# GoekeLab/m6anet

Measured on AMD Instinct MI355X. Metric: DRACH sites/sec at num_iterations=1000, higher is better.
Workload: dtype f32

## Files before the change

include/m6a.h:

```cpp
#ifndef M6A_H
#define M6A_H
#include <stddef.h>
#include <stdint.h>
#ifdef __cplusplus
extern "C" {
#endif

typedef struct m6a_ctx m6a_ctx;

enum {
    M6A_OK = 0,
    M6A_EINVAL = -1,
    M6A_ENOMEM = -2,
    M6A_EHIP = -3,
    M6A_ESTREAM = -4,
    M6A_ENODEV = -5,
    M6A_EUNSUPPORTED = -6,
    M6A_EFORMAT = -7,
    M6A_EIO = -8,
    M6A_EDECLINED = -9
};

enum { M6A_RNG_NUMPY = 0 };

#define M6A_N_WEIGHTS 7997
#define M6A_N_FEATURES 9
#define M6A_MAX_SAMPLES 64
#define M6A_N_KMERS 66

int m6a_create(m6a_ctx **out, const float *weights, size_t n_floats, int device_id);
void m6a_destroy(m6a_ctx *ctx);
const char *m6a_last_error(const m6a_ctx *ctx);

int m6a_set_stream(m6a_ctx *ctx, void *hip_stream);
int m6a_set_job_offset(m6a_ctx *ctx, int64_t first_site);
int m6a_sync(m6a_ctx *ctx);
int m6a_set_host_offsets(m6a_ctx *ctx, const int64_t *off_host);
int m6a_prepare_host_io(m6a_ctx *ctx);
int m6a_host_alloc(size_t bytes, void **out);
int m6a_host_free(void *p);
int m6a_host_is_pinned(const void *p, size_t bytes);

int m6a_encode_reads(m6a_ctx *ctx, const float *X, const uint8_t *site_kmers, const int64_t *off,
                     int64_t n_sites, float *read_prob);

int m6a_site_pool(m6a_ctx *ctx, const float *read_prob, const int64_t *off, int64_t n_sites,
                  int n_iters, int n_samples, float read_proba_threshold, uint32_t seed,
                  int rng_mode, int64_t batch_size, int64_t save_per_batch,
                  float *site_prob, double *mod_ratio);

int m6a_infer(m6a_ctx *ctx, const float *X, const uint8_t *site_kmers, const int64_t *off,
              int64_t n_sites, int n_iters, int n_samples, float read_proba_threshold,
              uint32_t seed, int rng_mode, int64_t batch_size, int64_t save_per_batch,
              float *read_prob, float *site_prob, double *mod_ratio);

int m6a_job_begin(m6a_ctx *ctx, int n_iters, int n_samples, float read_proba_threshold, uint32_t seed, int rng_mode,
                  int64_t batch_size, int64_t save_per_batch, int64_t expect_sites, int64_t expect_reads);
int m6a_job_feed(m6a_ctx *ctx, const float *X, const uint8_t *site_kmers, const int64_t *off, int64_t n_sites);
int m6a_job_feed_collated(m6a_ctx *ctx, const float *features, const int64_t *kmers, const int64_t *n_reads, int64_t n_sites);
int m6a_job_size(const m6a_ctx *ctx, int64_t *n_sites, int64_t *n_reads);
int m6a_job_end(m6a_ctx *ctx, float *read_prob, float *site_prob, double *mod_ratio);
int m6a_job_abort(m6a_ctx *ctx);

int m6a_bag_forward(m6a_ctx *ctx, const float *X, const uint8_t *site_kmers, int64_t n_bags,
                    int bag, float *site_prob);

int m6a_validate_pool(m6a_ctx *ctx, const float *read_prob, const int64_t *off, int64_t n_sites,
                      int n_iters, int n_samples, uint32_t seed, float *y_pred, float *y_pred_avg);
int m6a_validate(m6a_ctx *ctx, const float *X, const uint8_t *site_kmers, const int64_t *off,
                 int64_t n_sites, int n_iters, int n_samples, uint32_t seed, float *read_prob,
                 float *y_pred, float *y_pred_avg);


int64_t m6a_flush_groups(int64_t n_sites, int64_t batch_size, int64_t save_per_batch,
                         int64_t *group_off, int64_t cap);

int64_t m6a_reference_written_sites(int64_t n_sites, int64_t batch_size, int64_t save_per_batch);

int m6a_shard_plan(const int64_t *off, int64_t n_sites, int64_t batch_size, int64_t save_per_batch,
                   int n_shards, int64_t *shard_site_off);

#define M6A_COMM_ID_BYTES 128
int m6a_comm_unique_id(void *id_out);
int m6a_comm_init(m6a_ctx *ctx, const void *unique_id, int rank, int world_size);
int m6a_gather(m6a_ctx *ctx, const float *site_prob, const double *mod_ratio, const int64_t *shard_site_off,
               int dst, float *site_all, double *mod_all);
int m6a_gather_reads(m6a_ctx *ctx, const float *read_prob, const int64_t *shard_read_off, int dst, float *read_all);
int m6a_comm_destroy(m6a_ctx *ctx);
int m6a_comm_count(m6a_ctx *ctx, int *ranks_seen);
int m6a_comm_info(m6a_ctx *ctx, int *rank, int *device, int *rccl_version);
int m6a_device_link(int dev_a, int dev_b, int *link_type, int *hops, int *peer_access);
int m6a_device_count(void);

int m6a_random_stream(m6a_ctx *ctx, uint32_t seed, int64_t n_words, uint32_t *words);

int m6a_profile_enable(m6a_ctx *ctx, int on);
int m6a_profile_read(m6a_ctx *ctx, int kind, double *total_ms, int64_t *n_launches);
int m6a_profile_clock(m6a_ctx *ctx, int kind, double *ghz_median, double *ghz_min, double *ghz_max, double *span_ms, int *n_waves);
int m6a_set_encoder_variant(m6a_ctx *ctx, int mode);
const char *m6a_last_encoder_variant(const m6a_ctx *ctx);
const char *m6a_last_encoder_kernel(const m6a_ctx *ctx);
int m6a_set_scan_driver(m6a_ctx *ctx, int mode);
int m6a_set_table_variant(m6a_ctx *ctx, int mode);
const char *m6a_last_pool_variant(const m6a_ctx *ctx);

const char *m6a_version(void);

typedef struct m6a_prep m6a_prep;
struct m6a_io_prep_table;
int m6a_prep_eventalign(int device_id, const char *path, int n_neighbors, const char *index_path, m6a_prep **out);
const struct m6a_io_prep_table *m6a_prep_table(const m6a_prep *p);
int m6a_prep_times(const m6a_prep *p, double *ms6);
void m6a_prep_free(m6a_prep *p);
const char *m6a_prep_last_error(void);

typedef struct m6a_prep_sites m6a_prep_sites;
struct m6a_io_rows;
typedef struct m6a_prep_host_half {
    int (*rows)(const char *eventalign_path, int64_t n_runs, const int64_t *start, const int64_t *end, const int64_t *read,
                int n_neighbors, int n_threads, struct m6a_io_rows **out);
    const struct m6a_io_prep_table *(*table)(const struct m6a_io_rows *r);
    void (*free)(struct m6a_io_rows *r);
    const char *(*error)(void);
} m6a_prep_host_half;
typedef struct m6a_prep_sites_info {
    int64_t n_sites, n_reads, n_tx;
    const float *X;
    const uint8_t *site_kmers;
    const int64_t *off;
    float *read_prob, *site_prob;
    double *mod_ratio;
    const int64_t *off_host;
    const uint32_t *site_tx;
    const int64_t *site_pos;
    const char *site_kmer7;
    const char *tx_blob;
    const int64_t *tx_off;
    const double *read_ids;
    double ms[8];
    int64_t d2h_bytes;
    int n_rep;
    const int32_t *read_rep;
    int64_t peak_bytes;
    int64_t n_windows, window_bytes;
    int64_t n_bgzf_blocks, compressed_bytes;
    double ms_inflate;
    int64_t n_declined_sites;
} m6a_prep_sites_info;
int m6a_prep_sites_build(int device_id, const char *path, int readcount_min, int readcount_max, int min_segment_count,
                         const char *norm_kmers, const double *norm_mean, const double *norm_std, int n_norm,
                         const m6a_prep_host_half *host, int n_threads, m6a_prep_sites **out);
int m6a_prep_sites_build_multi(int device_id, const char *const *paths, int n_paths, int readcount_min, int readcount_max,
                               int min_segment_count, const char *norm_kmers, const double *norm_mean, const double *norm_std, int n_norm,
                               const m6a_prep_host_half *host, int n_threads, m6a_prep_sites **out);
int m6a_prep_sites_build_windows(int device_id, const char *const *paths, int n_paths, int readcount_min, int readcount_max,
                                 int min_segment_count, const char *norm_kmers, const double *norm_mean, const double *norm_std, int n_norm,
                                 const m6a_prep_host_half *host, int n_threads, int64_t window_bytes, m6a_prep_sites **out);
int m6a_prep_sites_build_names(int device_id, const char *const *paths, int n_paths, int readcount_min, int readcount_max,
                               int min_segment_count, const char *norm_kmers, const double *norm_mean, const double *norm_std, int n_norm,
                               const m6a_prep_host_half *host, int n_threads, int64_t window_bytes, int read_names, m6a_prep_sites **out);
int m6a_prep_sites_read_names(const m6a_prep_sites *p, const uint8_t **names16, const int64_t **name_off, int *n_rep);
double m6a_prep_sites_intern_ms(const m6a_prep_sites *p);
#define M6A_PREP_STREAM_WINDOW_BYTES ((int64_t)256 << 20)
int64_t m6a_prep_sites_stream_bytes(const m6a_prep_sites *p);
int64_t m6a_prep_sites_n_streams(const m6a_prep_sites *p);
const m6a_prep_sites_info *m6a_prep_sites_get(const m6a_prep_sites *p);
int m6a_prep_sites_fetch(m6a_prep_sites *p, float *read_prob, float *site_prob, double *mod_ratio);
int m6a_prep_sites_inputs(m6a_prep_sites *p, float *X, uint8_t *site_kmers, int64_t *off);
void m6a_prep_sites_free(m6a_prep_sites *p);

struct m6a_io_info;
struct m6a_io_info_table;
typedef struct m6a_json_host_half {
    int (*open)(const char *dir, int min_reads, struct m6a_io_info **out);
    const struct m6a_io_info_table *(*table)(const struct m6a_io_info *info);
    int (*rows)(struct m6a_io_info *info, const int64_t *sites, int64_t n, const char *norm_kmers, const double *norm_mean,
                const double *norm_std, int n_norm, int n_threads, float *X, double *read_ids, uint8_t *site_kmers, char *kmer7);
    void (*free)(struct m6a_io_info *info);
    const char *(*error)(void);
} m6a_json_host_half;
int m6a_json_sites_build(int device_id, const char *const *dirs, int n_dirs, int min_reads, const char *norm_kmers,
// ... 59 lines not shown
```

m6anet_amd/_lib.py:

```python
import ctypes as C
import os

_PKG = os.path.dirname(os.path.abspath(__file__))
LIB_PATH = os.environ.get("M6A_HIP_LIB") or os.path.join(_PKG, "libm6a_hip.so")

M6A_OK = 0
ERRORS = {-1: "M6A_EINVAL", -2: "M6A_ENOMEM", -3: "M6A_EHIP", -4: "M6A_ESTREAM", -5: "M6A_ENODEV",
          -6: "M6A_EUNSUPPORTED", -7: "M6A_EFORMAT", -8: "M6A_EIO", -9: "M6A_EDECLINED"}
M6A_EDECLINED = -9
RNG_NUMPY = 0

SYMBOLS = ["m6a_create", "m6a_destroy", "m6a_last_error", "m6a_set_stream", "m6a_set_job_offset", "m6a_set_scan_driver", "m6a_set_table_variant", "m6a_set_encoder_variant", "m6a_last_encoder_variant", "m6a_last_encoder_kernel", "m6a_sync", "m6a_set_host_offsets", "m6a_prepare_host_io", "m6a_host_alloc", "m6a_host_free", "m6a_host_is_pinned",
           "m6a_encode_reads", "m6a_site_pool", "m6a_infer", "m6a_job_begin", "m6a_job_feed", "m6a_job_feed_collated", "m6a_job_size", "m6a_job_end", "m6a_job_abort", "m6a_bag_forward", "m6a_validate_pool", "m6a_validate", "m6a_flush_groups",
           "m6a_reference_written_sites",
           "m6a_shard_plan", "m6a_comm_unique_id", "m6a_comm_init", "m6a_gather", "m6a_gather_reads", "m6a_device_count", "m6a_random_stream", "m6a_comm_destroy", "m6a_comm_count", "m6a_comm_info", "m6a_device_link", "m6a_profile_enable", "m6a_profile_read", "m6a_profile_clock", "m6a_last_pool_variant",
           "m6a_version", "m6a_prep_eventalign", "m6a_prep_table", "m6a_prep_times", "m6a_prep_free", "m6a_prep_last_error",
           "m6a_prep_sites_build", "m6a_prep_sites_build_multi", "m6a_prep_sites_build_windows", "m6a_prep_sites_build_names", "m6a_prep_sites_read_names", "m6a_prep_sites_intern_ms", "m6a_prep_sites_stream_bytes", "m6a_prep_sites_n_streams", "m6a_prep_sites_get", "m6a_prep_sites_fetch", "m6a_prep_sites_inputs", "m6a_prep_sites_free",
           "m6a_csv_format", "m6a_prep_sites_write_csv", "m6a_bgzf_inflate", "m6a_bgzf_deflate", "m6a_prep_sites_write_csv_bgzf",
           "m6a_bgzf_deflate_level", "m6a_prep_sites_write_csv_bgzf_level", "m6a_json_sites_build"]

_lib = None


class HostHalf(C.Structure):
    _fields_ = [("rows", C.c_void_p), ("table", C.c_void_p), ("free", C.c_void_p), ("error", C.c_void_p)]


class JsonHostHalf(C.Structure):
    _fields_ = [("open", C.c_void_p), ("table", C.c_void_p), ("rows", C.c_void_p), ("free", C.c_void_p), ("error", C.c_void_p)]


class PrepSitesInfo(C.Structure):
    _fields_ = [("n_sites", C.c_int64), ("n_reads", C.c_int64), ("n_tx", C.c_int64), ("X", C.c_void_p), ("site_kmers", C.c_void_p),
                ("off", C.c_void_p), ("read_prob", C.c_void_p), ("site_prob", C.c_void_p), ("mod_ratio", C.c_void_p),
                ("off_host", C.c_void_p), ("site_tx", C.c_void_p), ("site_pos", C.c_void_p), ("site_kmer7", C.c_void_p),
                ("tx_blob", C.c_void_p), ("tx_off", C.c_void_p), ("read_ids", C.c_void_p), ("ms", C.c_double * 8),
                ("d2h_bytes", C.c_int64), ("n_rep", C.c_int), ("read_rep", C.c_void_p), ("peak_bytes", C.c_int64),
                ("n_windows", C.c_int64), ("window_bytes", C.c_int64),
                ("n_bgzf_blocks", C.c_int64), ("compressed_bytes", C.c_int64), ("ms_inflate", C.c_double),
                ("n_declined_sites", C.c_int64)]


class BgzfStats(C.Structure):
    _fields_ = [("n_blocks", C.c_int64), ("compressed_bytes", C.c_int64), ("ms_upload", C.c_double), ("ms_inflate", C.c_double),
                ("ms_crc", C.c_double), ("ms_copy", C.c_double), ("d2h_bytes", C.c_int64)]


class DeflateStats(C.Structure):
    _fields_ = [("n_blocks", C.c_int64), ("n_stored", C.c_int64), ("ms_deflate", C.c_double), ("ms_copy", C.c_double), ("d2h_bytes", C.c_int64)]


class CsvBgzfStats(C.Structure):
    _fields_ = [("ms_format", C.c_double), ("ms_deflate", C.c_double), ("ms_copy", C.c_double), ("ms_write", C.c_double),
                ("site_bytes", C.c_int64), ("indiv_bytes", C.c_int64), ("site_compressed", C.c_int64), ("indiv_compressed", C.c_int64),
                ("n_blocks", C.c_int64), ("n_stored", C.c_int64), ("n_declined", C.c_int64), ("d2h_bytes", C.c_int64), ("n_rounds", C.c_int64)]


class CsvArrays(C.Structure):
    _fields_ = [("n_sites", C.c_int64), ("n_tx", C.c_int64), ("off", C.c_void_p), ("site_tx", C.c_void_p), ("site_pos", C.c_void_p),
                ("kmer5", C.c_void_p), ("tx_blob", C.c_char_p), ("tx_off", C.c_void_p), ("read_ids", C.c_void_p), ("read_rep", C.c_void_p),
                ("n_rep", C.c_int), ("read_prob", C.c_void_p), ("site_prob", C.c_void_p), ("mod_ratio", C.c_void_p)]


class CsvStats(C.Structure):
    _fields_ = [("ms_format", C.c_double), ("ms_copy", C.c_double), ("ms_write", C.c_double), ("site_bytes", C.c_int64),
                ("indiv_bytes", C.c_int64), ("n_declined", C.c_int64), ("d2h_bytes", C.c_int64), ("n_rounds", C.c_int64)]


class M6AError(RuntimeError):
    def __init__(self, code, msg):
        super().__init__("%s (%d): %s" % (ERRORS.get(code, "M6A_E?"), code, msg))
        self.code = code


def _preload_hip_runtime():
    import importlib.util
    try:
        spec = importlib.util.find_spec("torch")
    except (ImportError, ValueError):
        spec = None
    if spec and spec.submodule_search_locations:
        libdir = os.path.join(list(spec.submodule_search_locations)[0], "lib")
        rt = os.path.join(libdir, "libamdhip64.so")
        if os.path.exists(rt):
            C.CDLL(rt, mode=C.RTLD_GLOBAL)
        rccl = os.path.join(libdir, "librccl.so")
        if os.path.exists(rccl):
            os.environ.setdefault("M6A_RCCL_LIB", rccl)


def load():
    global _lib
    if _lib is not None:
        return _lib
    if not os.path.exists(LIB_PATH):
        raise ImportError("libm6a_hip.so is not built: run `python -m m6anet_amd.build` "
                          "(or __graft_entry__.build()); there is no CPU fallback")
    _preload_hip_runtime()
    L = C.CDLL(LIB_PATH)
    vp, i64, i32, u32, f32, sz = C.c_void_p, C.c_int64, C.c_int, C.c_uint32, C.c_float, C.c_size_t
    L.m6a_create.argtypes = [C.POINTER(vp), vp, sz, i32]
    L.m6a_destroy.argtypes = [vp]
    L.m6a_destroy.restype = None
    L.m6a_last_error.argtypes = [vp]
    L.m6a_last_error.restype = C.c_char_p
    L.m6a_set_stream.argtypes = [vp, vp]
    L.m6a_sync.argtypes = [vp]
    L.m6a_set_host_offsets.argtypes = [vp, vp]
    L.m6a_prepare_host_io.argtypes = [vp]
    L.m6a_set_job_offset.argtypes = [vp, i64]
    L.m6a_set_scan_driver.argtypes = [vp, i32]
    L.m6a_set_table_variant.argtypes = [vp, i32]
    L.m6a_set_encoder_variant.argtypes = [vp, i32]
    L.m6a_last_encoder_variant.argtypes = [vp]
    L.m6a_last_encoder_variant.restype = C.c_char_p
    L.m6a_host_alloc.argtypes = [C.c_size_t, C.POINTER(vp)]
    L.m6a_host_free.argtypes = [vp]
    L.m6a_host_is_pinned.argtypes = [vp, C.c_size_t]
    L.m6a_last_encoder_kernel.argtypes = [vp]
    L.m6a_last_encoder_kernel.restype = C.c_char_p
    L.m6a_encode_reads.argtypes = [vp, vp, vp, vp, i64, vp]
    L.m6a_site_pool.argtypes = [vp, vp, vp, i64, i32, i32, f32, u32, i32, i64, i64, vp, vp]
    L.m6a_infer.argtypes = [vp, vp, vp, vp, i64, i32, i32, f32, u32, i32, i64, i64, vp, vp, vp]
    L.m6a_job_begin.argtypes = [vp, i32, i32, f32, u32, i32, i64, i64, i64, i64]
    L.m6a_job_feed.argtypes = [vp, vp, vp, vp, i64]
    L.m6a_job_feed_collated.argtypes = [vp, vp, vp, vp, i64]
    L.m6a_job_size.argtypes = [vp, C.POINTER(i64), C.POINTER(i64)]
    L.m6a_job_end.argtypes = [vp, vp, vp, vp]
    L.m6a_job_abort.argtypes = [vp]
    L.m6a_bag_forward.argtypes = [vp, vp, vp, i64, i32, vp]
    L.m6a_validate_pool.argtypes = [vp, vp, vp, i64, i32, i32, C.c_uint32, vp, vp]
    L.m6a_validate.argtypes = [vp, vp, vp, vp, i64, i32, i32, C.c_uint32, vp, vp, vp]
    L.m6a_flush_groups.argtypes = [i64, i64, i64, vp, i64]
    L.m6a_flush_groups.restype = i64
    L.m6a_reference_written_sites.argtypes = [i64, i64, i64]
    L.m6a_reference_written_sites.restype = i64
    L.m6a_shard_plan.argtypes = [vp, i64, i64, i64, i32, vp]
    L.m6a_comm_unique_id.argtypes = [vp]
    L.m6a_comm_init.argtypes = [vp, vp, i32, i32]
    L.m6a_gather.argtypes = [vp, vp, vp, vp, i32, vp, vp]
    L.m6a_gather_reads.argtypes = [vp, vp, vp, i32, vp]
    L.m6a_device_count.argtypes = []
    L.m6a_random_stream.argtypes = [vp, u32, i64, vp]
    L.m6a_comm_destroy.argtypes = [vp]
    pi = C.POINTER(i32)
    L.m6a_comm_count.argtypes = [vp, pi]
    L.m6a_comm_info.argtypes = [vp, pi, pi, pi]
    L.m6a_device_link.argtypes = [i32, i32, pi, pi, pi]
    L.m6a_profile_enable.argtypes = [vp, i32]
    L.m6a_profile_read.argtypes = [vp, i32, C.POINTER(C.c_double), C.POINTER(i64)]
    L.m6a_profile_clock.argtypes = [vp, i32] + [C.POINTER(C.c_double)] * 4 + [C.POINTER(i32)]
    L.m6a_last_pool_variant.argtypes = [vp]
    L.m6a_last_pool_variant.restype = C.c_char_p
    L.m6a_version.restype = C.c_char_p
    L.m6a_prep_eventalign.argtypes = [i32, C.c_char_p, i32, C.c_char_p, C.POINTER(vp)]
    L.m6a_prep_table.argtypes = [vp]
    L.m6a_prep_table.restype = vp
    L.m6a_prep_times.argtypes = [vp, C.POINTER(C.c_double)]
    L.m6a_prep_free.argtypes = [vp]
    L.m6a_prep_free.restype = None
    L.m6a_prep_sites_build.argtypes = [i32, C.c_char_p, i32, i32, i32, C.c_char_p, vp, vp, i32, C.POINTER(HostHalf), i32, C.POINTER(vp)]
    L.m6a_prep_sites_build_multi.argtypes = [i32, C.POINTER(C.c_char_p), i32, i32, i32, i32, C.c_char_p, vp, vp, i32, C.POINTER(HostHalf), i32,
                                             C.POINTER(vp)]
    L.m6a_prep_sites_build_windows.argtypes = [i32, C.POINTER(C.c_char_p), i32, i32, i32, i32, C.c_char_p, vp, vp, i32, C.POINTER(HostHalf), i32,
                                               i64, C.POINTER(vp)]
    L.m6a_prep_sites_build_names.argtypes = [i32, C.POINTER(C.c_char_p), i32, i32, i32, i32, C.c_char_p, vp, vp, i32, C.POINTER(HostHalf), i32,
                                             i64, i32, C.POINTER(vp)]
    L.m6a_prep_sites_read_names.argtypes = [vp, C.POINTER(vp), C.POINTER(vp), C.POINTER(i32)]
    L.m6a_prep_sites_intern_ms.argtypes = [vp]
    L.m6a_prep_sites_intern_ms.restype = C.c_double
    for f in (L.m6a_prep_sites_stream_bytes, L.m6a_prep_sites_n_streams):
        f.argtypes = [vp]
        f.restype = C.c_int64
    L.m6a_json_sites_build.argtypes = [i32, C.POINTER(C.c_char_p), i32, i32, C.c_char_p, vp, vp, i32, C.POINTER(JsonHostHalf), i32, C.POINTER(vp)]
    L.m6a_prep_sites_get.argtypes = [vp]
    L.m6a_prep_sites_get.restype = C.POINTER(PrepSitesInfo)
    L.m6a_prep_sites_fetch.argtypes = [vp, vp, vp, vp]
    L.m6a_prep_sites_inputs.argtypes = [vp, vp, vp, vp]
    L.m6a_prep_sites_free.argtypes = [vp]
    L.m6a_prep_sites_free.restype = None
    pl = C.POINTER(i64)
    L.m6a_csv_format.argtypes = [i32, C.POINTER(CsvArrays), i64, i64, vp, i64, vp, i64, pl, pl, pl]
    L.m6a_prep_sites_write_csv.argtypes = [vp, C.c_char_p, i32, i64, i32, C.POINTER(CsvStats)]
    L.m6a_bgzf_inflate.argtypes = [i32, C.c_char_p, vp, i64, pl, C.POINTER(BgzfStats)]
    L.m6a_bgzf_deflate.argtypes = [i32, C.c_char_p, i64, vp, i64, pl, C.POINTER(DeflateStats)]
    L.m6a_prep_sites_write_csv_bgzf.argtypes = [vp, C.c_char_p, i32, i64, i32, C.POINTER(CsvBgzfStats)]
    L.m6a_bgzf_deflate_level.argtypes = [i32, C.c_char_p, i64, i32, vp, i64, pl, C.POINTER(DeflateStats), pl]
    L.m6a_prep_sites_write_csv_bgzf_level.argtypes = [vp, C.c_char_p, i32, i64, i32, i32, C.POINTER(CsvBgzfStats), pl]
    L.m6a_prep_last_error.argtypes = []
    L.m6a_prep_last_error.restype = C.c_char_p
    for name in SYMBOLS:
        fn = getattr(L, name)
        if fn.restype is C.c_int and name not in ("m6a_flush_groups", "m6a_reference_written_sites"):
            fn.restype = C.c_int
    _lib = L
    return L
```

m6anet_amd/csrc/m6a_api.hip:

```cpp
#include "m6a_ctx.h"

#if !defined(__HIP_DEVICE_COMPILE__)
#ifndef M6A_MT_JUMP_PATH
#error "build with -DM6A_MT_JUMP_PATH=\"<repo>/m6anet_amd/assets/mt19937_jump.bin\" (m6anet_amd/build.py does)"
#endif
asm(".section .rodata\n"
    ".global m6a_mt_jump_blob\n.global m6a_mt_jump_blob_end\n.hidden m6a_mt_jump_blob\n.hidden m6a_mt_jump_blob_end\n.balign 64\n"
    "m6a_mt_jump_blob:\n.incbin \"" M6A_MT_JUMP_PATH "\"\n"
    "m6a_mt_jump_blob_end:\n.byte 0\n.previous\n");
#endif

namespace {

thread_local std::string g_create_error;

std::mutex g_live_mu;
std::vector<m6a_ctx *> g_live;
void join_background_setups()
{
    std::lock_guard<std::mutex> g(g_live_mu);
    for (m6a_ctx *c : g_live)
        if (c->warm.joinable()) c->warm.join();
    g_live.clear();
}
// ... 50 lines not shown
    for (float &v : alpha) v *= bn_scale;
    for (float &v : beta) v *= bn_scale;
    for (float &v : w2) v *= 0x1p+64f;
    const float w3_scale = 0.5f;
    auto unit_of_row = [](int m, int i) { return 32 * m + 2 * ((i & 3) + 4 * (i >> 3)) + ((i >> 2) & 1); };
    auto out_unit = [](int q, int half) {
        if (half == 0) return q < 8 ? 2 * q + 1 : 2 * (q - 8) + 17;
        return q < 8 ? 2 * q + 2 : (q < 15 ? 2 * (q - 8) + 18 : 0);
    };
    auto out_unit_of_row = [&](int i) { return out_unit((i & 3) + 4 * (i >> 3), (i >> 2) & 1); };
    frag.assign(M6A_WFRAG_FLOATS, 0.f);
    for (int lane = 0; lane < 64; lane++) {
        const int col = lane & 31, half = lane >> 5;
        for (int m = 0; m < 5; m++) {
            for (int st = 0; st < 8; st++)
                frag[(m * 8 + st) * 64 + lane] = w1[unit_of_row(m, col) * 16 + 2 * st + half];
            for (int q = 0; q < 16; q++)
                frag[(40 + m * 16 + q) * 64 + lane] = w2[out_unit_of_row(col) * 160 + 32 * m + 2 * q + half];
        }
        for (int q = 0; q < 16; q++)
            frag[(120 + q) * 64 + lane] = w3_scale * w[O_W3 + out_unit(q, half)];
    }
    frag2.assign(M6A_WFRAG2_FLOATS, 0.f);
    w1e.assign(M6A_W1E_FLOATS + M6A_BN_FLOATS, 0.f);
    for (int lane = 0; lane < 64; lane++) {
        const int col = lane & 31, half = lane >> 5;
        for (int m = 0; m < 5; m++) {
            for (int st = 0; st < 4; st++) frag2[(m * 4 + st) * 64 + lane] = w1[unit_of_row(m, col) * 16 + 2 * st + half];
            frag2[(20 + m) * 64 + lane] = w1[unit_of_row(m, col) * 16 + 8];
        }
    }
    for (int m = 0; m < 5; m++)
        for (int col = 0; col < 32; col++) {
            for (int e = 0; e < 6; e++) w1e[(m * 7 + e) * 32 + col] = w1[unit_of_row(m, col) * 16 + 9 + e];
            w1e[(m * 7 + 6) * 32 + col] = w1[unit_of_row(m, col) * 16 + 15];
        }
    for (int m = 0; m < 5; m++)
        for (int half = 0; half < 2; half++)
            for (int q = 0; q < 16; q++) {
                const int u = 32 * m + 2 * q + half;
                w1e[M6A_W1E_FLOATS + ((m * 2 + half) * 16 + q) * 2] = alpha[u];
                w1e[M6A_W1E_FLOATS + ((m * 2 + half) * 16 + q) * 2 + 1] = beta[u];
            }
}

int64_t flush_groups(int64_t S, int64_t bs, int64_t spb, int64_t base, std::vector<int64_t> &goff)
{
    goff.clear();
    goff.push_back(0);
    if (S <= 0) return 0;
    const int64_t it0 = base / bs;
    const int64_t nb = (S + bs - 1) / bs;
    int64_t start_b = 0;
    for (int64_t b = 0; b < nb; b++) {
        if ((it0 + b + 1) % spb) {
            goff.push_back(std::min((b + 1) * bs, S));
            start_b = b + 1;
        }
    }
    if (start_b < nb) goff.push_back(S);
    return (int64_t)goff.size() - 1;
}

bool base_is_group_start(int64_t base, int64_t bs, int64_t spb)
{
    if (base < 0 || base % bs) return false;
    const int64_t it0 = base / bs;
    return it0 == 0 || (it0 % spb) != 0;
}

int ensure_groups(m6a_ctx *c, int64_t S, int64_t bs, int64_t spb)
{
    const int64_t base = c->job_offset;
    if (c->goff_key.valid && c->goff_key.S == S && c->goff_key.bs == bs && c->goff_key.spb == spb &&
        c->goff_key.base == base) return M6A_OK;
    if (!base_is_group_start(base, bs, spb))
        return fail(c, M6A_EINVAL, "job offset %lld does not start a flush group for batch_size=%lld save_per_batch=%lld",
                    (long long)base, (long long)bs, (long long)spb);
    std::vector<int64_t> g;
    const int64_t G = flush_groups(S, bs, spb, base, g);
    int64_t gmax = 0;
    for (int64_t i = 0; i < G; i++) gmax = std::max(gmax, g[i + 1] - g[i]);
    HIPCHK(c, c->goff.ensure(g.size() * sizeof(int64_t)));
    HIPCHK(c, hipMemcpyAsync(c->goff.p, g.data(), g.size() * sizeof(int64_t), hipMemcpyHostToDevice, c->stream));
    HIPCHK(c, hipStreamSynchronize(c->stream));
    c->goff_key = {S, bs, spb, base, G, gmax, true};
    return M6A_OK;
}

constexpr int kJumpPerRegime = 31, kJumpPolyWords = 312;
constexpr int64_t kXheadWords = 22016;

extern "C" const unsigned char m6a_mt_jump_blob[];
extern "C" const unsigned char m6a_mt_jump_blob_end[];

struct JumpRegime { int64_t G; const uint64_t *polys; };

const JumpRegime *jump_regimes(int *n_out)
{
    static JumpRegime reg[8];
    static int n = 0;
    static std::once_flag once;
    std::call_once(once, [] {
        const unsigned char *b = m6a_mt_jump_blob;
        const size_t len = (size_t)(m6a_mt_jump_blob_end - m6a_mt_jump_blob);
        uint32_t hdr[4];
        if (len >= 24 && std::memcmp(b, "M6AMTJP1", 8) == 0) {
            std::memcpy(hdr, b + 8, 16);
            const size_t per = 8 + (size_t)hdr[1] * hdr[2] * 8;
            if (hdr[0] <= 8 && hdr[1] == (uint32_t)kJumpPerRegime && hdr[2] == (uint32_t)kJumpPolyWords && hdr[3] == 512 &&
                len == 24 + hdr[0] * per)
                for (uint32_t r = 0; r < hdr[0]; r++) {
                    const unsigned char *q = b + 24 + r * per;
                    int64_t G;
                    std::memcpy(&G, q, 8);
                    reg[n++] = {G, (const uint64_t *)(q + 8)};
                }
        }
    });
    *n_out = n;
    return reg;
}

int launch_stream(m6a_ctx *c, uint32_t seed, int64_t len, uint32_t *raw)
{
    int n_reg = 0;
    const JumpRegime *reg = jump_regimes(&n_reg);
    const JumpRegime *use = nullptr;
    static const bool allowed = !(getenv("M6A_MT_SEGMENTS") && getenv("M6A_MT_SEGMENTS")[0] == '0');
    if (allowed && n_reg > 0 && len > reg[0].G + kXheadWords) {
        use = &reg[n_reg - 1];
        for (int r = 0; r < n_reg; r++) if (len <= (int64_t)(kJumpPerRegime + 1) * reg[r].G) { use = &reg[r]; break; }
    }
    if (!use) {
        hipLaunchKernelGGL(mt19937_kernel, dim3(1), dim3(640), 0, c->stream, seed, len, raw, (const uint32_t *)nullptr, len,
                           (uint32_t *)nullptr, (int64_t)0);
        HIPCHK(c, hipGetLastError());
        return M6A_OK;
    }
    const int n_seg = (int)std::min<int64_t>((len + use->G - 1) / use->G, kJumpPerRegime + 1);
    const size_t poly_bytes = (size_t)kJumpPerRegime * kJumpPolyWords * 8;
    HIPCHK(c, c->mt_scratch.ensure((size_t)kXheadWords * 4 + (size_t)kJumpPerRegime * 1078 * 4 + poly_bytes));
    uint32_t *xhead = (uint32_t *)c->mt_scratch.p, *hist = xhead + kXheadWords;
    uint64_t *d_polys = (uint64_t *)(hist + (size_t)kJumpPerRegime * 1078);
    if (c->mt_polys_G != use->G) {
        HIPCHK(c, hipMemcpyAsync(d_polys, use->polys, poly_bytes, hipMemcpyHostToDevice, c->stream));
        c->mt_polys_G = use->G;
    }
    hipLaunchKernelGGL(mt19937_kernel, dim3(1), dim3(640), 0, c->stream, seed, kXheadWords - 624, raw, (const uint32_t *)nullptr,
                       kXheadWords, xhead, kXheadWords);
    hipLaunchKernelGGL(mt_jump_kernel, dim3(17, (unsigned)(n_seg - 1)), dim3(256), 0, c->stream, (const uint32_t *)xhead,
                       (const uint64_t *)d_polys, hist);
    hipLaunchKernelGGL(mt19937_kernel, dim3((unsigned)n_seg), dim3(640), 0, c->stream, seed, len, raw, (const uint32_t *)hist, use->G,
                       (uint32_t *)nullptr, (int64_t)0);
    HIPCHK(c, hipGetLastError());
    return M6A_OK;
}

int ensure_raw(m6a_ctx *c, uint32_t seed, int64_t len)
{
    if (c->raw_len >= len && c->raw_seed == seed) return M6A_OK;
    if (len > ((int64_t)1 << 31) - 512)
        return fail(c, M6A_ESTREAM, "a flush group would need %lld MT19937 words (cap 2^31); "
                    "reduce batch_size*save_per_batch or num_iterations", (long long)len);
    len = (len + 1023) / 1024 * 1024;
    c->raw_len = 0;
    c->rt.valid = false;
    HIPCHK(c, c->raw.ensure((size_t)len * 4));
    int rc = launch_stream(c, seed, len, (uint32_t *)c->raw.p);
    if (rc) return rc;
    c->raw_seed = seed; c->raw_len = len;
    return M6A_OK;
}

void pairwise_rec(int lo, int n, MeanPlan &p)
{
    if (n <= 128) {
        p.leaf_start.push_back(lo);
        p.merge_after.push_back(0);
        return;
    }
    int n2 = n / 2;
    n2 -= n2 % 8;
    pairwise_rec(lo, n2, p);
    pairwise_rec(lo + n2, n - n2, p);
    p.merge_after.back()++;
}

int plan_iteration(const MeanPlan &p, int row, int lane)
{
    const int L = (int)p.merge_after.size();
    const int ps = p.row_pass[row], i = p.row_round[row];
    if (ps < 0) return lane < p.n_rem ? p.T - p.n_rem + lane : -1;
    const int b = 8 * ps + (lane >> 3);
    if (b >= L) return -1;
    const int len = p.leaf_start[b + 1] - p.leaf_start[b];
    return i < len / 8 ? p.leaf_start[b] + 8 * i + (lane & 7) : -1;
}

void build_mean_plan(int T, MeanPlan &p)
{
    p = MeanPlan();
    p.T = T;
    pairwise_rec(0, T, p);
    p.leaf_start.push_back(T);
    const int L = (int)p.merge_after.size();
    const int last_len = p.leaf_start[L] - p.leaf_start[L - 1];
    p.n_rem = last_len % 8;
    if (p.n_rem) { p.row_pass.push_back(-1); p.row_round.push_back(0); }
    const int P = (L + 7) / 8;
    for (int ps = 0; ps < P; ps++) {
        int rounds = 0;
        for (int b = 8 * ps; b < std::min(L, 8 * ps + 8); b++)
            rounds = std::max(rounds, (p.leaf_start[b + 1] - p.leaf_start[b]) / 8);
        rounds = std::max(rounds, 1);
        for (int i = 0; i < rounds; i++) { p.row_pass.push_back(ps); p.row_round.push_back(i); }
    }
    int d = 0;
    for (int b = 0; b < L; b++) {
        d++; p.depth = std::max(p.depth, d); d -= p.merge_after[b];
        p.max_merge = std::max<int>(p.max_merge, p.merge_after[b]);
    }
    p.reg_ctl.assign((size_t)std::max(1, (T - p.n_rem) / 8), 0u);
    for (int b = 0; b + 1 < L; b++) p.reg_ctl[(size_t)p.leaf_start[b + 1] / 8 - 1] = 1u | ((uint32_t)p.merge_after[b] << 8);
    const int rows = (int)p.row_pass.size();
    p.row_meta.assign((size_t)rows * 4, 0u);
    for (int r = 0; r < rows; r++) {
        uint32_t *m = &p.row_meta[(size_t)r * 4];
        uint64_t live = 0;
        for (int l = 0; l < 64; l++) live |= (uint64_t)(plan_iteration(p, r, l) >= 0) << l;
        m[1] = (uint32_t)live; m[2] = (uint32_t)(live >> 32);
        const int ps = p.row_pass[r];
        if (ps < 0) { m[0] = 1u << 25; continue; }
        if (r + 1 == rows || p.row_pass[r + 1] != ps) {
            const int nl = std::min(8, L - 8 * ps);
            m[0] = (1u << 24) | ((uint32_t)nl << 26) | (ps == P - 1 ? 1u << 30 : 0u);
            for (int bl = 0; bl < nl; bl++) m[3] |= (uint32_t)(p.merge_after[8 * ps + bl] & 15) << (4 * bl);
        }
    }
}

int ensure_mean_plan(m6a_ctx *c, int T)
{
    if (c->plan.T == T && c->plan_dev.p) return M6A_OK;
    build_mean_plan(T, c->plan);
    const MeanPlan &p = c->plan;
    if (p.depth > M6A_MEAN_STACK) return fail(c, M6A_EUNSUPPORTED, "n_iters %d: pairwise-sum tree deeper than %d", T, M6A_MEAN_STACK);
    const size_t b0 = p.leaf_start.size() * 4, b1 = (p.merge_after.size() + 3) / 4 * 4, b2 = std::max<size_t>(p.row_meta.size(), 1) * 4;
    const size_t b3 = p.reg_ctl.size() * 4;
    HIPCHK(c, c->plan_dev.ensure(b0 + b1 + b2 + b3));
    char *d = (char *)c->plan_dev.p;
    HIPCHK(c, hipMemcpyAsync(d, p.leaf_start.data(), b0, hipMemcpyHostToDevice, c->stream));
    HIPCHK(c, hipMemcpyAsync(d + b0, p.merge_after.data(), p.merge_after.size(), hipMemcpyHostToDevice, c->stream));
    if (!p.row_meta.empty())
        HIPCHK(c, hipMemcpyAsync(d + b0 + b1, p.row_meta.data(), p.row_meta.size() * 4, hipMemcpyHostToDevice, c->stream));
    HIPCHK(c, hipMemcpyAsync(d + b0 + b1 + b2, p.reg_ctl.data(), b3, hipMemcpyHostToDevice, c->stream));
    HIPCHK(c, hipStreamSynchronize(c->stream));
    c->plan_off[0] = 0; c->plan_off[1] = b0; c->plan_off[2] = b0 + b1; c->plan_off[3] = b0 + b1 + b2;
    c->tab_key.valid = false;
    return M6A_OK;
}

void plan_args(m6a_ctx *c, PoolArgs &a)
{
    const char *d = (const char *)c->plan_dev.p;
    a.leaf_start = (const int *)(d + c->plan_off[0]);
    a.merge_after = (const uint8_t *)(d + c->plan_off[1]);
    a.row_meta = (const uint32_t *)(d + c->plan_off[2]);
    a.n_leaves = (int)c->plan.merge_after.size();
    a.n_rows = (int)c->plan.row_pass.size();
    a.n_rem = c->plan.n_rem;
    a.stack_depth = c->plan.depth;
    a.reg_ctl = (const uint32_t *)(d + c->plan_off[3]);
    a.reg_rounds = (a.T - c->plan.n_rem) / 8;
    a.reg_final_merges = c->plan.merge_after.back();
}

int64_t stream_need(int64_t gmax, int T, int K)
{
    const int64_t A = (int64_t)T * K;
    return gmax * (2 * A + A / 16) + 8192;
}

uint32_t *ctl_cursor(m6a_ctx *c) { return c->h_ctl; }
int32_t *ctl_slot(m6a_ctx *c) { return (int32_t *)(c->h_ctl + M6A_HIST_BINS); }
int32_t *ctl_build_n(m6a_ctx *c) { return ctl_slot(c) + M6A_RTAB_MAX_N + 1; }
int32_t *ctl_build_slot(m6a_ctx *c) { return ctl_build_n(c) + M6A_RTAB_MAX_N; }
constexpr size_t kCtlWords = M6A_HIST_BINS + (M6A_RTAB_MAX_N + 1) + 2 * M6A_RTAB_MAX_N;

int rtab_missing(const m6a_ctx *c, uint32_t seed, int T, int K, int64_t need, const uint32_t *hist, int *n_distinct)
{
    const bool valid = c->rt.valid && c->rt.seed == seed && c->rt.A == (int64_t)T * K && c->raw_seed == seed &&
                       c->rt.n_blk * 64 >= need && c->rt.n_blk == c->raw_len / 64;
    int missing = 0, distinct = 0;
    for (int n = 2; n <= M6A_RTAB_MAX_N; n++)
        if (hist[n]) { distinct++; if (!valid || c->rt.slot_of_n[n] < 0) missing++; }
    if (n_distinct) *n_distinct = distinct;
    return missing;
}

int ensure_rtab(m6a_ctx *c, uint32_t seed, int T, int K, int64_t gmax, const uint32_t *hist, bool *usable)
{
    *usable = false;
    const int64_t need = stream_need(gmax, T, K);
    int rc = ensure_raw(c, seed, need);
    if (rc) return rc;
    auto &rt = c->rt;
    const int64_t n_blk = c->raw_len / 64;
    if (!(rt.valid && rt.seed == seed && rt.A == (int64_t)T * K && rt.n_blk == n_blk)) {
        rt.valid = false; rt.used = 0;
        for (int n = 0; n <= M6A_RTAB_MAX_N; n++) rt.slot_of_n[n] = -1;
    }
    std::vector<int> todo;
    for (int n = 2; n <= M6A_RTAB_MAX_N; n++)
        if (hist[n] && rt.slot_of_n[n] < 0) todo.push_back(n);
    const int64_t c_stride = n_blk * 64;
    const size_t slot_bytes = (size_t)c_stride * 2 + (size_t)(n_blk + 1) * 4;
    const bool fresh = !rt.valid || rt.n_blk != n_blk;
    const int want = (fresh ? 1 : rt.used) + (int)todo.size();
    if (fresh || want > rt.cap) {
        int new_cap = std::max(want, fresh ? 0 : rt.cap * 2);
        new_cap = std::min(std::max(new_cap, std::max(32, c->rt_presize)), M6A_RTAB_MAX_N + 1);
        size_t free_b = 0, total_b = 0;
        HIPCHK(c, hipMemGetInfo(&free_b, &total_b));
        const size_t held = fresh ? 0 : (size_t)rt.cap * slot_bytes;
        const size_t budget = std::min<size_t>((size_t)16 << 30, (free_b + held) / 2);
        if ((size_t)new_cap * slot_bytes > budget) new_cap = want;
        if ((size_t)new_cap * slot_bytes > budget) return M6A_OK;
        uint16_t *nC = nullptr; uint32_t *nRS = nullptr;
        if (fresh) {
            if (rt.C) (void)hipFree(rt.C);
            if (rt.RS) (void)hipFree(rt.RS);
            rt.C = nullptr; rt.RS = nullptr; rt.cap = 0;
        }
        if (hipMalloc((void **)&nC, (size_t)new_cap * c_stride * 2 + 64) != hipSuccess) { (void)hipGetLastError(); return M6A_OK; }
        if (hipMalloc((void **)&nRS, (size_t)new_cap * (n_blk + 1) * 4) != hipSuccess) { (void)hipGetLastError(); (void)hipFree(nC); return M6A_OK; }
        if (!fresh && rt.used) {
            HIPCHK(c, hipMemcpyAsync(nC, rt.C, (size_t)rt.used * c_stride * 2, hipMemcpyDeviceToDevice, c->stream));
            HIPCHK(c, hipMemcpyAsync(nRS, rt.RS, (size_t)rt.used * (n_blk + 1) * 4, hipMemcpyDeviceToDevice, c->stream));
            HIPCHK(c, hipStreamSynchronize(c->stream));
            c->graveyard.push_back(rt.C); c->graveyard.push_back(rt.RS);
        }
        rt.C = nC; rt.RS = nRS; rt.cap = new_cap;
        if (fresh) {
            HIPCHK(c, hipMemsetAsync(rt.C, 0, (size_t)c_stride * 2, c->stream));
            HIPCHK(c, hipMemsetAsync(rt.RS, 0, (size_t)(n_blk + 1) * 4, c->stream));
            rt.used = 1;
        }
        rt.valid = true; rt.seed = seed; rt.A = (int64_t)T * K; rt.n_blk = n_blk;
    }
    if (!todo.empty()) {
        int32_t *bn = ctl_build_n(c), *bs = ctl_build_slot(c);
        for (size_t i = 0; i < todo.size(); i++) { bn[i] = todo[i]; bs[i] = rt.used; rt.slot_of_n[todo[i]] = rt.used++; }
        HIPCHK(c, c->ctl_dev.ensure(kCtlWords * 4));
        int32_t *d_bn = (int32_t *)c->ctl_dev.p + (ctl_build_n(c) - (int32_t *)c->h_ctl);
        HIPCHK(c, hipMemcpyAsync(d_bn, bn, (size_t)2 * M6A_RTAB_MAX_N * 4, hipMemcpyHostToDevice, c->stream));
        RtabBuild b;
        b.raw = (const uint32_t *)c->raw.p; b.n_blk = (uint32_t)n_blk; b.build_n = d_bn; b.build_slot = d_bn + M6A_RTAB_MAX_N;
        b.C = rt.C; b.RS = rt.RS; b.c_stride = c_stride; b.n_build = (int)todo.size();
        const unsigned gx = (unsigned)std::min<int64_t>((n_blk + 63) / 64, 65535);
        const unsigned gn = (unsigned)((todo.size() + 7) / 8);
        hipLaunchKernelGGL(rtab_count_kernel, dim3(gn, gx), dim3(256), 0, c->stream, b);
        hipLaunchKernelGGL(rtab_scan_kernel, dim3((unsigned)todo.size()), dim3(256), 0, c->stream, b);
        hipLaunchKernelGGL(rtab_fill_kernel, dim3(gn, gx), dim3(256), 0, c->stream, b);
        HIPCHK(c, hipGetLastError());
        HIPCHK(c, hipStreamSynchronize(c->stream));
    }
    *usable = true;
    return M6A_OK;
}

int uniform_slice(m6a_ctx *c, uint32_t seed, int n, int T, int K, int jmax, const uint16_t **C)
{
    *C = nullptr;
    if (n < 2) return M6A_OK;
    std::vector<uint32_t> hist(M6A_HIST_BINS, 0u);
    hist[n] = 1;
    bool usable = false;
    int rc = ensure_rtab(c, seed, T, K, jmax, hist.data(), &usable);
    if (rc) return rc;
    if (!usable) return fail(c, M6A_ENOMEM, "no device memory for the index table of bag size %d", n);
    const int64_t slot = c->rt.slot_of_n[n], A = (int64_t)T * K;
    uint32_t total = 0;
    HIPCHK(c, hipMemcpyAsync(&total, c->rt.RS + slot * (c->rt.n_blk + 1) + c->rt.n_blk, 4, hipMemcpyDeviceToHost, c->stream));
    HIPCHK(c, hipStreamSynchronize(c->stream));
    if ((int64_t)total < A * jmax) return fail(c, M6A_ESTREAM, "MT19937 stream too short for a flush group");
    *C = c->rt.C + slot * c->rt.n_blk * 64;
    return M6A_OK;
}

int ensure_table_reg(m6a_ctx *c, uint32_t seed, int n, int T, int K, int jmax)
{
    auto &k = c->tab_reg_key;
    if (k.valid && k.seed == seed && k.n == n && k.T == T && k.K == K && k.jmax >= jmax) return M6A_OK;
    k.valid = false;
    const size_t per_j = (size_t)(T + 8) * K;
    const size_t bytes = (size_t)jmax * per_j * 2 + 4096;
    HIPCHK(c, c->tab_reg.ensure(bytes));
    HIPCHK(c, hipMemsetAsync(c->tab_reg.p, 0, bytes, c->stream));
    const uint16_t *C = nullptr;
    int rc = uniform_slice(c, seed, n, T, K, jmax, &C);
    if (rc) return rc;
    if (C) {
        const int64_t A = (int64_t)T * K;
        hipLaunchKernelGGL(rtab_to_reg_table_kernel, dim3((unsigned)((A * jmax + 255) / 256)), dim3(256), 0, c->stream,
                           C, A, (int64_t)per_j, jmax, (uint16_t *)c->tab_reg.p);
        HIPCHK(c, hipGetLastError());
    }
    k = {seed, n, T, K, jmax, true};
    return M6A_OK;
}

int ensure_table(m6a_ctx *c, uint32_t seed, int n, int T, int K, int jmax)
{
    int rc = ensure_mean_plan(c, T);
    if (rc) return rc;
    auto &k = c->tab_key;
    if (k.valid && k.seed == seed && k.n == n && k.T == T && k.K == K && k.jmax >= jmax) return M6A_OK;
    k.valid = false;
    const MeanPlan &p = c->plan;
    const int rows = (int)p.row_pass.size();
    c->iter_of.resize((size_t)rows * 64);
    for (int r = 0; r < rows; r++)
        for (int l = 0; l < 64; l++) c->iter_of[(size_t)r * 64 + l] = plan_iteration(p, r, l);
    const size_t words = (size_t)jmax * rows * 5 * 64;
    HIPCHK(c, c->tab.ensure(words * 4 + c->iter_of.size() * 4));
    int *d_iter = (int *)((uint32_t *)c->tab.p + words);
    HIPCHK(c, hipMemcpyAsync(d_iter, c->iter_of.data(), c->iter_of.size() * 4, hipMemcpyHostToDevice, c->stream));
    const uint16_t *C = nullptr;
    rc = uniform_slice(c, seed, n, T, K, jmax, &C);
    if (rc) return rc;
    if (C) {
        hipLaunchKernelGGL(rtab_to_lds_table_kernel, dim3((unsigned)((words + 255) / 256)), dim3(256), 0, c->stream,
                           C, (int64_t)T * K, K, rows, jmax, (const int *)d_iter, (uint32_t *)c->tab.p);
        HIPCHK(c, hipGetLastError());
    } else {
        HIPCHK(c, hipMemsetAsync(c->tab.p, 0, words * 4, c->stream));
    }
    k = {seed, n, T, K, jmax, true};
    return M6A_OK;
}

void prof_begin(m6a_ctx *c, int kind)
{
    Profiler &p = c->prof;
    if (!p.on || !(p.mask >> kind & 1)) return;
    if (p.used[kind] >= kMaxProfiled) { p.dropped[kind]++; return; }
    if ((int)p.start[kind].size() <= p.used[kind]) {
        hipEvent_t a, b;
        (void)hipEventCreate(&a); (void)hipEventCreate(&b);
        p.start[kind].push_back(a); p.stop[kind].push_back(b);
    }
    (void)hipEventRecord(p.start[kind][p.used[kind]], c->stream);
}
void prof_end(m6a_ctx *c, int kind)
{
    Profiler &p = c->prof;
    if (!p.on || !(p.mask >> kind & 1) || p.used[kind] >= kMaxProfiled) return;
    (void)hipEventRecord(p.stop[kind][p.used[kind]], c->stream);
    p.used[kind]++;
}

void host_bag_range(m6a_ctx *c, const int64_t *off, int64_t S);
int sync_and_check(m6a_ctx *c);

int query_bags(m6a_ctx *c, const int64_t *d_off, int64_t S)
{
    if (c->side_work) { HIPCHK(c, hipStreamSynchronize(c->s_prep)); c->side_work = false; }
    c->h_minmax[0] = ~0ull; c->h_minmax[1] = 0ull; c->h_minmax[2] = 0ull;
    HIPCHK(c, hipMemcpyAsync(c->d_minmax, c->h_minmax, 24, hipMemcpyHostToDevice, c->stream));
    HIPCHK(c, hipMemsetAsync(c->d_hist, 0, M6A_HIST_BINS * 4, c->stream));
    hipLaunchKernelGGL(bag_minmax_kernel, dim3((unsigned)std::min<int64_t>((S + 255) / 256, 512)), dim3(256), 0,
                       c->stream, d_off, S, c->d_minmax, c->d_hist);
    HIPCHK(c, hipGetLastError());
    HIPCHK(c, hipMemcpyAsync(c->h_minmax, c->d_minmax, 24, hipMemcpyDeviceToHost, c->stream));
    HIPCHK(c, hipMemcpyAsync(c->h_hist, c->d_hist, M6A_HIST_BINS * 4, hipMemcpyDeviceToHost, c->stream));
    HIPCHK(c, hipStreamSynchronize(c->stream));
    c->bag_min = (int64_t)c->h_minmax[0];
    c->bag_max = (int64_t)c->h_minmax[1];
    c->n_reads = (int64_t)c->h_minmax[2];
    return M6A_OK;
}

int bag_stats(m6a_ctx *c, const int64_t *d_off, int64_t S)
{
    const int64_t *h = c->hint_off;
    c->hint_off = nullptr;
    if (!h) return query_bags(c, d_off, S);
    if (h[0] != 0) return fail(c, M6A_EINVAL, "off[0] must be 0");
    host_bag_range(c, h, S);
    if (c->bag_min < 0) return fail(c, M6A_EINVAL, "off[] must be non-decreasing");
    unsigned long long hash = 0;
    for (int i = 0; i < M6A_HIST_BINS; i++) hash += (unsigned long long)c->h_hist[i] * m6a_bin_weight(i);
    hipStream_t st = c->s_prep ? c->s_prep : c->stream;
    if (st != c->stream) {
        HIPCHK(c, hipEventRecord(c->ev_main, c->stream));
        HIPCHK(c, hipStreamWaitEvent(st, c->ev_main, 0));
    }
    HIPCHK(c, hipMemsetAsync(c->d_minmax, 0xff, 8, st));
    HIPCHK(c, hipMemsetAsync(c->d_minmax + 1, 0, 16, st));
    HIPCHK(c, hipMemsetAsync(c->d_hist, 0, M6A_HIST_BINS * 4, st));
    hipLaunchKernelGGL(bag_minmax_kernel, dim3((unsigned)std::min<int64_t>((S + 255) / 256, 512)), dim3(256), 0,
                       st, d_off, S, c->d_minmax, c->d_hist);
    hipLaunchKernelGGL(bag_verify_kernel, dim3(1), dim3(256), 0, st, c->d_minmax, c->d_hist, (unsigned long long)c->bag_min,
                       (unsigned long long)c->bag_max, (unsigned long long)c->n_reads, hash, c->d_err);
    HIPCHK(c, hipGetLastError());
    c->side_work = true;
    return M6A_OK;
}

int launch_encode(m6a_ctx *c, const float *X, const uint8_t *km, const int64_t *off, int64_t S,
                  int64_t R, float *rp)
{
    if (R <= 0 || S <= 0) return M6A_OK;
    EncArgs a;
    a.X = X; a.site_kmers = km; a.off = off; a.wfrag = c->d_wfrag; a.emb = c->d_emb; a.read_prob = rp;
    a.wfrag2 = c->d_wfrag2; a.w1e_tab = c->d_w1e; a.bn = c->d_w1e + M6A_W1E_FLOATS; a.err = c->d_err;
    a.n_sites = S; a.n_reads = R; a.n_tiles = (R + 31) / 32; a.b3 = c->b3;
    a.clk = c->prof.clk_for(0);
#ifdef M6A_AB_W3
    const int64_t max_waves = (int64_t)c->n_cu * 12;
#else
    const int64_t max_waves = (int64_t)c->n_cu * 8;
#endif
    a.tiles_per_wave = (a.n_tiles + max_waves - 1) / max_waves;
    const int64_t waves = (a.n_tiles + a.tiles_per_wave - 1) / a.tiles_per_wave;
    const unsigned blocks = (unsigned)((waves + 3) / 4);
    const bool fits32 = S < 0x7ffffff0LL && a.n_tiles < 0x7ffffff0LL;
    if (c->enc_variant == 2 && !fits32) return fail(c, M6A_EUNSUPPORTED, "12-slot encoder: more than 2^31 sites or tiles");
    const bool scalar_chain = c->bag_min >= M6A_CSITE_MIN_BAG && fits32;
    const bool csite = c->enc_variant == 2 || (c->enc_variant == 4 && scalar_chain);
    const bool site16 = !csite && c->enc_variant != 3 && scalar_chain;
    c->enc_variant_used = csite ? "csite12" : "general16";
    c->enc_kernel_used = csite ? "enc_csite_kernel" : site16 ? "enc_site16_kernel" : "enc_kernel";
    prof_begin(c, 0);
    if (csite) hipLaunchKernelGGL(enc_csite_kernel, dim3(blocks), dim3(256), 0, c->stream, a);
    else if (site16) hipLaunchKernelGGL(enc_site16_kernel, dim3(blocks), dim3(256), 0, c->stream, a);
    else hipLaunchKernelGGL(enc_kernel, dim3(blocks), dim3(256), 0, c->stream, a);
    prof_end(c, 0);
    HIPCHK(c, hipGetLastError());
    return M6A_OK;
}

RtabUse rtab_use(m6a_ctx *c, int64_t nmax, uint32_t si_base = 0, uint32_t si_count = 0)
{
    RtabUse u;
    u.C = c->rt.C; u.RS = c->rt.RS; u.slot_of_n = (const int32_t *)c->ctl_dev.p + M6A_HIST_BINS;
    u.rank = (uint32_t *)c->rt_rank.p; u.order = (const uint32_t *)c->rt_order.p;
    u.c_stride = c->rt.n_blk * 64; u.n_blk = (uint32_t)c->rt.n_blk;
    u.bag_cap = (int)std::max<int64_t>(64, (nmax + 63) / 64 * 64);
    u.si_base = si_base; u.si_count = si_count;
    return u;
}

int rtab_prepare(m6a_ctx *c, PoolArgs a, int64_t nmax, int64_t gmax, uint32_t seed, bool *use)
{
    *use = false;
    const int T = a.T, K = a.K;
    const int64_t S = a.n_sites;
    const int64_t need = stream_need(gmax, T, K);
    if (nmax > M6A_RTAB_MAX_N || c->scan_driver == 1 || c->scan_driver == 2) {
        if (c->scan_driver == 3)
            return fail(c, M6A_EUNSUPPORTED, "index-table pooling needs every bag <= %d reads (largest: %lld)", M6A_RTAB_MAX_N, (long long)nmax);
        return M6A_OK;
    }
    int distinct = 0;
    const int missing = rtab_missing(c, seed, T, K, need, c->h_hist, &distinct);
    if (c->rt_credit_seed != seed || c->rt_credit_A != (int64_t)T * K) { c->rt_credit_seed = seed; c->rt_credit_A = (int64_t)T * K; c->rt_credit = 0; }
    bool use_rtab = c->scan_driver == 3 || missing == 0 || c->rt_credit + S >= (int64_t)16 * missing;
    if (use_rtab) c->rt_credit = 0; else c->rt_credit += S;
    if (!use_rtab) return M6A_OK;
    int rc = ensure_rtab(c, seed, T, K, gmax, c->h_hist, &use_rtab);
    if (rc) return rc;
    if (!use_rtab) return M6A_OK;
    a.raw = (const uint32_t *)c->raw.p; a.raw_len = c->raw_len;
    HIPCHK(c, c->rt_rank.ensure((size_t)S * 4));
    HIPCHK(c, c->rt_order.ensure((size_t)S * 4));
    HIPCHK(c, c->ctl_dev.ensure(kCtlWords * 4));
    HIPCHK(c, hipEventSynchronize(c->ev_ctl));
    uint32_t *cur = ctl_cursor(c);
    uint32_t run = 0;
    for (int n = M6A_HIST_BINS - 1; n > M6A_RTAB_SMALL_N; n--) { cur[n] = run; run += c->h_hist[n]; }
    for (int x = 0; x < 8; x++)
        for (int n = M6A_RTAB_SMALL_N - ((M6A_RTAB_SMALL_N - x) & 7); n >= 0; n -= 8) { cur[n] = run; run += c->h_hist[n]; }
    std::memcpy(ctl_slot(c), c->rt.slot_of_n, sizeof c->rt.slot_of_n);
    HIPCHK(c, hipMemcpyAsync(c->ctl_dev.p, c->h_ctl, (size_t)(M6A_HIST_BINS + M6A_RTAB_MAX_N + 1) * 4, hipMemcpyHostToDevice, c->stream));
    HIPCHK(c, hipEventRecord(c->ev_ctl, c->stream));
    const RtabUse u = rtab_use(c, nmax);
    const unsigned n_order_blocks = (unsigned)((S + 255) / 256);
    const unsigned n_chain_blocks = (unsigned)std::min<int64_t>((a.n_groups + 3) / 4, (int64_t)c->n_cu * 16);
    hipLaunchKernelGGL(rtab_prep_kernel, dim3(n_order_blocks + n_chain_blocks), dim3(256), 0, c->stream, a, u,
                       (uint32_t *)c->ctl_dev.p, (uint32_t *)c->rt_order.p, n_order_blocks);
    HIPCHK(c, hipGetLastError());
    *use = true;
    return M6A_OK;
}

int launch_pool(m6a_ctx *c, const float *rp, const int64_t *off, int64_t S, int T, int K, float thr,
                uint32_t seed, int64_t bs, int64_t spb, float *site, double *mod, bool dry)
{
    const bool prepared = c->prep.ready && c->prep.off == off && c->prep.S == S && c->prep.T == T && c->prep.K == K &&
                          c->prep.seed == seed && c->prep.bs == bs && c->prep.spb == spb;
    c->prep.ready = false;
    if (S <= 0) return M6A_OK;
    int rc = ensure_groups(c, S, bs, spb);
    if (rc) return rc;
    const int64_t nmin = c->bag_min, nmax = c->bag_max;
    if (nmin < 0 || nmax > 0x7fffffff) return fail(c, M6A_EINVAL, "off[] is not a non-decreasing CSR array");

    PoolArgs a;
    memset(&a, 0, sizeof a);
    a.read_prob = rp; a.off = off; a.goff = (const int64_t *)c->goff.p; a.site_prob = site; a.mod_ratio = mod;
    a.err = c->d_err; a.n_groups = c->goff_key.G; a.n_sites = S; a.T = T; a.K = K; a.thr = thr;
    a.clk = dry ? nullptr : c->prof.clk_for(1);
    const int64_t gmax = c->goff_key.gmax;

    rc = ensure_mean_plan(c, T);
    if (rc) return rc;
    const bool uniform = nmin == nmax && nmin >= 1 && nmin <= M6A_TABLE_MAX_N && K == 20 && gmax <= 4096;
    const bool reg_ok = uniform && c->plan.depth <= M6A_REG_STACK && c->n_reads < (int64_t)1 << 30 &&
                        (int64_t)gmax * (T + 8) * K * 2 <= (int64_t)256 << 20;
    if (uniform && reg_ok && c->table_variant != 1) {
        rc = ensure_table_reg(c, seed, (int)nmin, T, K, (int)gmax);
        if (rc) return rc;
        plan_args(c, a);
        a.tab = (const uint32_t *)c->tab_reg.p; a.uniform_n = (int)nmin; a.jmax = (int)gmax;
        if (dry) return M6A_OK;
        c->pool_variant = "table-reg";
        prof_begin(c, 1);
        const int64_t wpj = (a.n_groups + 255) / 256;
        a.reg_items = wpj * a.jmax;
        hipLaunchKernelGGL(pool_reg_kernel, dim3((unsigned)((a.reg_items + 7) / 8 * 8)), dim3(64), 0, c->stream, a);
        prof_end(c, 1);
    } else if (uniform && c->plan.max_merge <= 15) {
        rc = ensure_table(c, seed, (int)nmin, T, K, (int)gmax);
        if (rc) return rc;
        if (dry) return M6A_OK;
        plan_args(c, a);
        a.tab = (const uint32_t *)c->tab.p; a.uniform_n = (int)nmin; a.jmax = (int)gmax;
        const int64_t gblocks = (a.n_groups + 7) / 8;
        int64_t nbj = std::max<int64_t>(1, ((int64_t)c->n_cu * 5 + a.jmax - 1) / a.jmax);
        nbj = std::min<int64_t>(nbj, (gblocks + 3) / 4);
        const unsigned blocks = (unsigned)(nbj * a.jmax);
        c->pool_variant = "table";
        prof_begin(c, 1);
        const size_t mean_lds = (size_t)4 * (128 + 8 * a.stack_depth) * sizeof(float);
        hipLaunchKernelGGL(pool_table_kernel, dim3(blocks), dim3(256), mean_lds, c->stream, a);
        prof_end(c, 1);
    } else {
        const int64_t need = stream_need(gmax, T, K);
        bool use_rtab = false;
        if (prepared && !dry) {
            use_rtab = c->prep.use;
        } else {
            rc = rtab_prepare(c, a, nmax, gmax, seed, &use_rtab);
            if (rc) return rc;
        }
        if (dry) {
            c->prep.ready = true; c->prep.use = use_rtab;
            c->prep.off = off; c->prep.S = S; c->prep.bs = bs; c->prep.spb = spb; c->prep.T = T; c->prep.K = K; c->prep.seed = seed;
            if (!use_rtab) {
                rc = ensure_raw(c, seed, need);
                if (rc) return rc;
                HIPCHK(c, c->start_pos.ensure((size_t)S * sizeof(uint32_t)));
            }
            return M6A_OK;
        }
        if (use_rtab) {
            plan_args(c, a);
            a.raw = (const uint32_t *)c->raw.p; a.raw_len = c->raw_len;
            c->pool_variant = "ragged-table";
            int64_t n_big = 0;
            for (int n = M6A_RTAB_SMALL_N + 1; n < M6A_HIST_BINS; n++) n_big += c->h_hist[n];
            prof_begin(c, 1);
            auto launch = [&](int64_t base, int64_t count, int64_t cap_n) {
                if (count <= 0) return;
                const RtabUse u = rtab_use(c, cap_n, (uint32_t)base, (uint32_t)count);
                const size_t lds = (size_t)(u.bag_cap + 16 + M6A_MEAN_STACK) * sizeof(float);
                const unsigned blocks = (unsigned)((count + 7) / 8 * 8);
                if (K == 20) hipLaunchKernelGGL(pool_rtab_kernel<20>, dim3(blocks), dim3(64), lds, c->stream, a, u);
                else hipLaunchKernelGGL(pool_rtab_kernel<0>, dim3(blocks), dim3(64), lds, c->stream, a, u);
            };
            launch(0, n_big, nmax);
            launch(n_big, S - n_big, std::min<int64_t>(nmax, M6A_RTAB_SMALL_N));
            prof_end(c, 1);
            HIPCHK(c, hipGetLastError());
            return M6A_OK;
        }
        rc = ensure_raw(c, seed, need);
        if (rc) return rc;
        plan_args(c, a);
        a.raw = (const uint32_t *)c->raw.p; a.raw_len = c->raw_len;
        HIPCHK(c, c->start_pos.ensure((size_t)S * sizeof(uint32_t)));
        a.start_pos = (uint32_t *)c->start_pos.p;
        int64_t cap = 64;
        while (cap < nmax && cap < M6A_BAG_LDS) cap *= 2;
        a.bag_cap = (int)cap;
        const size_t lds = (size_t)4 * (a.bag_cap + (32 * K + 256) * 5 / 4 + 32 + M6A_MEAN_STACK) * sizeof(float);
        const int64_t wg_per_cu = std::max<int64_t>(1, std::min<int64_t>(a.bag_cap >= 256 ? 5 : 8, (160 * 1024) / (int64_t)lds));
        const int64_t wave_slots = (int64_t)c->n_cu * wg_per_cu * 4;
        const bool by_group = c->scan_driver ? c->scan_driver == 1 : a.n_groups * 5 >= wave_slots * 3;
        c->pool_variant = by_group ? "scan-group" : "scan-site";
        prof_begin(c, 1);
        if (by_group) {
            const unsigned blocks = (unsigned)std::min<int64_t>((a.n_groups + 3) / 4, wave_slots / 4);
            if (K == 20) hipLaunchKernelGGL(pool_scan_group_kernel<20>, dim3(blocks), dim3(256), lds, c->stream, a);
            else hipLaunchKernelGGL(pool_scan_group_kernel<0>, dim3(blocks), dim3(256), lds, c->stream, a);
        } else {
            hipLaunchKernelGGL(pool_scan_start_kernel, dim3((unsigned)std::min<int64_t>((a.n_groups + 3) / 4, (int64_t)c->n_cu * 8)),
                               dim3(256), 0, c->stream, a);
            const unsigned blocks = (unsigned)std::min<int64_t>((S + 3) / 4, wave_slots / 4);
            if (K == 20) hipLaunchKernelGGL(pool_scan_site_kernel<20>, dim3(blocks), dim3(256), lds, c->stream, a);
            else hipLaunchKernelGGL(pool_scan_site_kernel<0>, dim3(blocks), dim3(256), lds, c->stream, a);
        }
        prof_end(c, 1);
    }
    HIPCHK(c, hipGetLastError());
    return M6A_OK;
}

int pool_setup_aside(m6a_ctx *c, const int64_t *off, int64_t S, int T, int K, uint32_t seed, int64_t bs, int64_t spb)
{
    c->prep.ready = false;
    if (S <= 0 || !c->s_prep) return M6A_OK;
    HIPCHK(c, hipStreamWaitEvent(c->s_prep, c->ev_main, 0));
    hipStream_t main_stream = c->stream;
    c->stream = c->s_prep;
    const int rc = launch_pool(c, nullptr, off, S, T, K, 0.0f, seed, bs, spb, nullptr, nullptr, true);
    c->stream = main_stream;
    if (rc) { c->prep.ready = false; return rc; }
    HIPCHK(c, hipEventRecord(c->ev_prep, c->s_prep));
    HIPCHK(c, hipStreamWaitEvent(c->stream, c->ev_prep, 0));
    return M6A_OK;
}

template <int>
static inline void bag_range_loop(const int64_t *off, int64_t S, int64_t *mn_out, int64_t *mx_out)
{
    int64_t mn = INT64_MAX, mx = 0;
    for (int64_t s = 0; s < S; s++) {
        const int64_t n = off[s + 1] - off[s];
        mn = n < mn ? n : mn;
        mx = n > mx ? n : mx;
    }
    *mn_out = mn; *mx_out = mx;
}
__attribute__((target("avx2"))) static void bag_range_avx2(const int64_t *off, int64_t S, int64_t *mn, int64_t *mx) { bag_range_loop<1>(off, S, mn, mx); }
static void bag_range_base(const int64_t *off, int64_t S, int64_t *mn, int64_t *mx) { bag_range_loop<0>(off, S, mn, mx); }

void host_bag_range(m6a_ctx *c, const int64_t *off, int64_t S)
{
    int64_t mn = INT64_MAX, mx = 0;
    static const bool avx2 = __builtin_cpu_supports("avx2");
    (avx2 ? bag_range_avx2 : bag_range_base)(off, S, &mn, &mx);
    auto bin = [](int64_t n) { return n < 0 ? 0 : n > M6A_RTAB_MAX_N ? M6A_RTAB_MAX_N + 1 : n; };
    std::memset(c->h_hist, 0, M6A_HIST_BINS * 4);
    if (mn == mx || S == 0) {
        if (S > 0) c->h_hist[bin(mn)] = (uint32_t)S;
    } else {
        c->hist_part.assign((size_t)8 * M6A_HIST_BINS, 0u);
        uint32_t (*part)[M6A_HIST_BINS] = (uint32_t (*)[M6A_HIST_BINS])c->hist_part.data();
        int64_t s = 0;
        for (; s + 8 <= S; s += 8)
            for (int k = 0; k < 8; k++) part[k][bin(off[s + k + 1] - off[s + k])]++;
        for (; s < S; s++) part[0][bin(off[s + 1] - off[s])]++;
        for (int i = 0; i < M6A_HIST_BINS; i++) {
            uint32_t t = 0;
            for (int k = 0; k < 8; k++) t += part[k][i];
            c->h_hist[i] = t;
        }
    }
    c->bag_min = S > 0 ? mn : 0; c->bag_max = mx; c->n_reads = off[S];
}

int job_busy(m6a_ctx *c)
{
    if (c->job.open) return fail(c, M6A_EINVAL, "a streaming job is open on this context (m6a_job_end or m6a_job_abort first)");
    return M6A_OK;
}

int check_pool_args(m6a_ctx *c, int64_t S, int T, int K, int rng_mode, int64_t bs, int64_t spb)
{
    if (!c) return M6A_EINVAL;
    if (S < 0) return fail(c, M6A_EINVAL, "n_sites < 0");
    if (T < 1) return fail(c, M6A_EINVAL, "n_iters must be >= 1");
    if (K < 1 || K > M6A_MAX_SAMPLES) return fail(c, M6A_EINVAL, "n_samples must be in 1..%d", M6A_MAX_SAMPLES);
    if ((int64_t)T * K > 0x3fffffff) return fail(c, M6A_EINVAL, "n_iters*n_samples too large");
    if (rng_mode != M6A_RNG_NUMPY) return fail(c, M6A_EINVAL, "rng_mode %d: M6A_RNG_NUMPY (0) is the only value (include/m6a.h)", rng_mode);
    if (bs < 1 || spb < 1) return fail(c, M6A_EINVAL, "batch_size and save_per_batch must be >= 1");
    return M6A_OK;
}

int deferred_error(m6a_ctx *c)
{
    if (*c->h_err) {
        const int e = *c->h_err;
        *c->h_err = 0;
        if (e == 2) return fail(c, M6A_EINVAL, "encoder: a 32-read tile spans more than 3 sites (bag < 16 reads) in the 12-slot kernel");
        if (e == 4) return fail(c, M6A_EHIP, "pool_rtab_kernel: the dynamic LDS block does not start at offset 0");
        if (e == 3) return fail(c, M6A_EINVAL, "the host offsets given to m6a_set_host_offsets differ from the device off[] of the call");
        return fail(c, M6A_ESTREAM, "MT19937 stream too short for a flush group");
    }
    return M6A_OK;
}

int sync_and_check(m6a_ctx *c)
{
    if (c->side_work) { HIPCHK(c, hipStreamSynchronize(c->s_prep)); c->side_work = false; }
    HIPCHK(c, hipMemcpyAsync(c->h_err, c->d_err, sizeof(int), hipMemcpyDeviceToHost, c->stream));
    HIPCHK(c, hipStreamSynchronize(c->stream));
    for (void *p : c->graveyard) (void)hipFree(p);
    c->graveyard.clear();
    if (*c->h_err) {
        HIPCHK(c, hipMemsetAsync(c->d_err, 0, sizeof(int), c->stream));
        return deferred_error(c);
// ... 35 lines not shown
}


extern "C" {

const char *m6a_version(void) { return "m6a_hip 0.1 (gfx950)"; }

const char *m6a_last_error(const m6a_ctx *ctx)
{
    settle(const_cast<m6a_ctx *>(ctx));
    return ctx ? ctx->err.c_str() : g_create_error.c_str();
}

int m6a_create(m6a_ctx **out, const float *weights, size_t n_floats, int device_id)
{
    if (!out) return M6A_EINVAL;
    *out = nullptr;
    if (!weights || n_floats != M6A_N_WEIGHTS)
        return fail(nullptr, M6A_EINVAL, "weights must be %d floats (got %zu)", M6A_N_WEIGHTS, n_floats);
    for (int i = O_W2; i < O_W3; i++)
        if (std::isfinite(weights[i]) && std::fabs(weights[i]) >= 0x1p+63f)
            return fail(nullptr, M6A_EUNSUPPORTED, "layer-2 weight %d is %g: beyond 2^63 in magnitude", i - O_W2, (double)weights[i]);
    int env_enc = 0;
    if (const char *ev = getenv("M6A_ENCODER")) {
        if (!*ev || !strcmp(ev, "auto") || !strcmp(ev, "reference")) env_enc = 0;
        else if (!strcmp(ev, "general16")) env_enc = 1;
        else if (!strcmp(ev, "csite12")) env_enc = 2;
        else if (!strcmp(ev, "walk16")) env_enc = 3;
        else if (!strcmp(ev, "fast")) env_enc = 4;
        else return fail(nullptr, M6A_EINVAL, "M6A_ENCODER=%s: must be auto, reference, general16, csite12, walk16 or fast", ev);
    }
    int ndev = 0;
    if (hipGetDeviceCount(&ndev) != hipSuccess || ndev <= 0) {
        (void)hipGetLastError();
        return fail(nullptr, M6A_ENODEV, "no HIP device visible");
    }
    if (device_id < 0 || device_id >= ndev) return fail(nullptr, M6A_EINVAL, "device_id %d out of range (%d devices)", device_id, ndev);
    m6a_ctx *c = new (std::nothrow) m6a_ctx;
    if (!c) return fail(nullptr, M6A_ENOMEM, "out of host memory");
    c->device = device_id;
#define CRCHK(expr)                                                                                  \
    do {                                                                                             \
        hipError_t e_ = (expr);                                                                      \
        if (e_ != hipSuccess) {                                                                      \
            (void)hipGetLastError();                                                                 \
            fail(nullptr, M6A_EHIP, "%s: %s", #expr, hipGetErrorString(e_));                         \
            m6a_destroy(c);                                                                          \
            return M6A_EHIP;                                                                         \
        }                                                                                            \
    } while (0)
    CRCHK(hipSetDevice(device_id));
    hipDeviceProp_t prop;
    CRCHK(hipGetDeviceProperties(&prop, device_id));
    if (std::strncmp(prop.gcnArchName, "gfx950", 6) != 0) {
        fail(nullptr, M6A_ENODEV, "device %d is %s; this library is built for gfx950 only", device_id, prop.gcnArchName);
        m6a_destroy(c);
        return M6A_ENODEV;
    }
    c->n_cu = prop.multiProcessorCount > 0 ? prop.multiProcessorCount : 256;
    CRCHK(hipStreamCreate(&c->own_stream));
    CRCHK(hipStreamCreateWithFlags(&c->s_prep, hipStreamNonBlocking));
    CRCHK(hipEventCreateWithFlags(&c->ev_main, hipEventDisableTiming));
    CRCHK(hipEventCreateWithFlags(&c->ev_prep, hipEventDisableTiming));
    CRCHK(hipEventCreateWithFlags(&c->ev_ctl, hipEventDisableTiming));
    c->stream = c->own_stream;
    std::vector<float> frag, frag2, w1e;
    build_fragments(weights, frag, frag2, w1e);
    CRCHK(hipMalloc((void **)&c->d_wfrag, frag.size() * sizeof(float)));
    CRCHK(hipMalloc((void **)&c->d_wfrag2, frag2.size() * sizeof(float)));
    CRCHK(hipMalloc((void **)&c->d_w1e, w1e.size() * sizeof(float)));
    CRCHK(hipMemcpy(c->d_wfrag2, frag2.data(), frag2.size() * sizeof(float), hipMemcpyHostToDevice));
    CRCHK(hipMemcpy(c->d_w1e, w1e.data(), w1e.size() * sizeof(float), hipMemcpyHostToDevice));
    CRCHK(hipMalloc((void **)&c->d_emb, 132 * sizeof(float)));
    CRCHK(hipMemcpy(c->d_wfrag, frag.data(), frag.size() * sizeof(float), hipMemcpyHostToDevice));
    CRCHK(hipMemcpy(c->d_emb, weights + O_E, 132 * sizeof(float), hipMemcpyHostToDevice));
    c->b3 = weights[O_B3];
    CRCHK(hipMalloc((void **)&c->d_err, sizeof(int)));
    CRCHK(hipMemset(c->d_err, 0, sizeof(int)));
    CRCHK(hipMalloc((void **)&c->d_minmax, 24));
    CRCHK(hipHostMalloc((void **)&c->h_minmax, 24, hipHostMallocDefault));
    CRCHK(hipHostMalloc((void **)&c->h_err, sizeof(int), hipHostMallocDefault));
    *c->h_err = 0;
    CRCHK(hipMalloc((void **)&c->d_hist, M6A_HIST_BINS * 4));
    CRCHK(hipHostMalloc((void **)&c->h_hist, M6A_HIST_BINS * 4, hipHostMallocDefault));
    CRCHK(hipHostMalloc((void **)&c->h_ctl, kCtlWords * 4, hipHostMallocDefault));
    for (int n = 0; n <= M6A_RTAB_MAX_N; n++) c->rt.slot_of_n[n] = -1;
#undef CRCHK
    c->enc_variant = env_enc;
    const char *w = getenv("M6A_WARMUP");
    if (!(w && w[0] == '0')) {
        try { c->warm = std::thread(warm_default, c); } catch (...) {  }
        if (c->warm.joinable()) {
            static std::once_flag once;
            std::call_once(once, [] { atexit(join_background_setups); });
            std::lock_guard<std::mutex> g(g_live_mu);
            g_live.push_back(c);
        }
    }
    *out = c;
    return M6A_OK;
}

void m6a_destroy(m6a_ctx *c)
{
    if (!c) return;
    settle(c);
    {
        std::lock_guard<std::mutex> g(g_live_mu);
        g_live.erase(std::remove(g_live.begin(), g_live.end(), c), g_live.end());
    }
    (void)hipSetDevice(c->device);
    if (c->stream) (void)hipStreamSynchronize(c->stream);
    for (int k = 0; k < 2; k++) {
        for (auto e : c->prof.start[k]) (void)hipEventDestroy(e);
        for (auto e : c->prof.stop[k]) (void)hipEventDestroy(e);
    }
    for (DevBuf *b : {&c->raw, &c->tab, &c->goff, &c->rp_scratch, &c->off_scratch, &c->start_pos, &c->plan_dev, &c->tab_reg, &c->val_idx, &c->val_y, &c->val_avg, &c->sX, &c->sK, &c->sOff,
                      &c->sP, &c->sSite, &c->sMod}) b->release();
    if (c->prof.d_clk) (void)hipFree(c->prof.d_clk);
    if (c->d_wfrag) (void)hipFree(c->d_wfrag);
    if (c->d_wfrag2) (void)hipFree(c->d_wfrag2);
    if (c->d_w1e) (void)hipFree(c->d_w1e);
    if (c->d_emb) (void)hipFree(c->d_emb);
    if (c->d_err) (void)hipFree(c->d_err);
    if (c->d_minmax) (void)hipFree(c->d_minmax);
    if (c->h_minmax) (void)hipHostFree(c->h_minmax);
    if (c->h_err) (void)hipHostFree(c->h_err);
    if (c->d_hist) (void)hipFree(c->d_hist);
    if (c->h_hist) (void)hipHostFree(c->h_hist);
    if (c->h_ctl) (void)hipHostFree(c->h_ctl);
    for (void *p : c->graveyard) (void)hipFree(p);
    if (c->rt.C) (void)hipFree(c->rt.C);
    if (c->rt.RS) (void)hipFree(c->rt.RS);
    for (DevBuf *b : {&c->ctl_dev, &c->rt_rank, &c->rt_order, &c->sOffChunk, &c->jX, &c->jP, &c->jOff, &c->gSite, &c->gMod, &c->gP, &c->mt_scratch}) b->release();
    for (auto e : c->job.ev_h2d) (void)hipEventDestroy(e);
    for (auto e : c->job.ev_enc) (void)hipEventDestroy(e);
    release_staging(c);
    comm_release(c);
    if (c->s_prep) (void)hipStreamDestroy(c->s_prep);
    if (c->ev_main) (void)hipEventDestroy(c->ev_main);
    if (c->ev_prep) (void)hipEventDestroy(c->ev_prep);
    if (c->ev_ctl) (void)hipEventDestroy(c->ev_ctl);
    if (c->own_stream) (void)hipStreamDestroy(c->own_stream);
    delete c;
}

int m6a_set_stream(m6a_ctx *c, void *hip_stream)
{
    settle(c);
    if (!c) return M6A_EINVAL;
    if (c->job.open) return job_busy(c);
    c->stream = hip_stream ? (hipStream_t)hip_stream : c->own_stream;
    return M6A_OK;
}

int m6a_set_host_offsets(m6a_ctx *c, const int64_t *off_host)
{
    if (!c) return M6A_EINVAL;
    if (off_host && is_device_ptr(off_host)) return fail(c, M6A_EINVAL, "m6a_set_host_offsets takes a host pointer");
    c->hint_off = off_host;
    return M6A_OK;
}

int m6a_set_job_offset(m6a_ctx *c, int64_t first_site)
{
    if (!c) return M6A_EINVAL;
    if (c->job.open) return job_busy(c);
    if (first_site < 0) return fail(c, M6A_EINVAL, "job offset must be >= 0");
    c->job_offset = first_site;
    return M6A_OK;
}

int m6a_set_encoder_variant(m6a_ctx *c, int mode)
{
    if (!c) return M6A_EINVAL;
    if (mode < 0 || mode > 4)
        return fail(c, M6A_EINVAL, "encoder variant must be 0 (auto: 16-slot), 1 (16-slot), 2 (12-slot), 3 (16-slot, per-lane walk) or 4 (fast: 12-slot where every bag has >= 16 reads)");
    c->enc_variant = mode;
    return M6A_OK;
}

const char *m6a_last_encoder_variant(const m6a_ctx *c) { return c ? c->enc_variant_used : "none"; }
const char *m6a_last_encoder_kernel(const m6a_ctx *c) { return c ? c->enc_kernel_used : "none"; }

int m6a_set_scan_driver(m6a_ctx *c, int mode)
{
    if (!c) return M6A_EINVAL;
    if (mode < 0 || mode > 3) return fail(c, M6A_EINVAL, "scan driver must be 0 (auto), 1 (group), 2 (site) or 3 (index tables)");
    c->scan_driver = mode;
    return M6A_OK;
}

int m6a_set_table_variant(m6a_ctx *c, int mode)
{
    if (!c) return M6A_EINVAL;
    if (mode < 0 || mode > 2) return fail(c, M6A_EINVAL, "table variant must be 0 (auto), 1 (LDS) or 2 (registers)");
    c->table_variant = mode;
    return M6A_OK;
}

int m6a_sync(m6a_ctx *c)
{
    settle(c);
    if (!c) return M6A_EINVAL;
    HIPCHK(c, hipSetDevice(c->device));
    return sync_and_check(c);
}

int m6a_prepare_host_io(m6a_ctx *c)
{
    settle(c);
    if (!c) return M6A_EINVAL;
    HIPCHK(c, hipSetDevice(c->device));
    return ensure_staging(c);
}

int m6a_host_alloc(size_t bytes, void **out)
{
    if (!out) return M6A_EINVAL;
    *out = nullptr;
    if (bytes == 0) return M6A_OK;
    const hipError_t e = hipHostMalloc(out, bytes, hipHostMallocDefault);
    if (e != hipSuccess) { (void)hipGetLastError(); *out = nullptr; return e == hipErrorOutOfMemory ? M6A_ENOMEM : M6A_EHIP; }
    return M6A_OK;
}

int m6a_host_free(void *p)
{
    if (!p) return M6A_OK;
    if (hipHostFree(p) != hipSuccess) { (void)hipGetLastError(); return M6A_EHIP; }
    return M6A_OK;
}

int m6a_encode_reads(m6a_ctx *c, const float *X, const uint8_t *km, const int64_t *off, int64_t S, float *rp)
{
    settle(c);
    HintScope hint_scope(c);
    if (c && c->job.open) return job_busy(c);
    if (!c) return M6A_EINVAL;
    if (S < 0) return fail(c, M6A_EINVAL, "n_sites < 0");
    if (S == 0) return M6A_OK;
    if (!X || !km || !off || !rp) return fail(c, M6A_EINVAL, "null pointer argument");
    HIPCHK(c, hipSetDevice(c->device));
    const bool dev = is_device_ptr(X);
    if (dev != is_device_ptr(km) || dev != is_device_ptr(off) || dev != is_device_ptr(rp))
        return fail(c, M6A_EINVAL, "X, site_kmers, off, read_prob must be all host or all device pointers");
    if (!dev) {
        if (off[0] != 0) return fail(c, M6A_EINVAL, "off[0] must be 0");
        for (int64_t s = 0; s < S; s++) if (off[s + 1] < off[s]) return fail(c, M6A_EINVAL, "off[] must be non-decreasing");
        const int64_t R = off[S];
        if (R == 0) return M6A_OK;
        host_bag_range(c, off, S);
        Prefault pf_rp;
        pf_rp.start(rp, (size_t)R * 4, 2);
        int rc = staged_encode(c, X, km, off, S, R, rp);
        if (rc) return rc;
        return sync_and_check(c);
    }
    int rc = bag_stats(c, off, S);
    if (rc) return rc;
    return launch_encode(c, X, km, off, S, c->n_reads, rp);
}

int m6a_site_pool(m6a_ctx *c, const float *rp, const int64_t *off, int64_t S, int T, int K, float thr,
                  uint32_t seed, int rng_mode, int64_t bs, int64_t spb, float *site, double *mod)
{
    settle(c);
    HintScope hint_scope(c);
    if (c && c->job.open) return job_busy(c);
    int rc = check_pool_args(c, S, T, K, rng_mode, bs, spb);
    if (rc) return rc;
    if (S == 0) return M6A_OK;
    if (!rp || !off || !site || !mod) return fail(c, M6A_EINVAL, "null pointer argument");
    HIPCHK(c, hipSetDevice(c->device));
    const bool dev = is_device_ptr(rp);
    if (dev != is_device_ptr(off) || dev != is_device_ptr(site) || dev != is_device_ptr(mod))
        return fail(c, M6A_EINVAL, "read_prob, off, site_prob, mod_ratio must be all host or all device pointers");
    if (dev) {
        rc = bag_stats(c, off, S);
        if (rc) return rc;
        return launch_pool(c, rp, off, S, T, K, thr, seed, bs, spb, site, mod);
    }
    if (off[0] != 0) return fail(c, M6A_EINVAL, "off[0] must be 0");
    for (int64_t s = 0; s < S; s++) if (off[s + 1] < off[s]) return fail(c, M6A_EINVAL, "off[] must be non-decreasing");
    const int64_t R = off[S];
    HIPCHK(c, c->sP.ensure((size_t)std::max<int64_t>(R, 1) * 4));
    HIPCHK(c, c->sOff.ensure((size_t)(S + 1) * 8));
    HIPCHK(c, c->sSite.ensure((size_t)S * 4));
    HIPCHK(c, c->sMod.ensure((size_t)S * 8));
    HIPCHK(c, hipMemcpyAsync(c->sP.p, rp, (size_t)R * 4, hipMemcpyHostToDevice, c->stream));
    HIPCHK(c, hipMemcpyAsync(c->sOff.p, off, (size_t)(S + 1) * 8, hipMemcpyHostToDevice, c->stream));
    host_bag_range(c, off, S);
    rc = launch_pool(c, (const float *)c->sP.p, (const int64_t *)c->sOff.p, S, T, K, thr, seed, bs, spb,
                     (float *)c->sSite.p, (double *)c->sMod.p);
    if (rc) return rc;
    HIPCHK(c, hipMemcpyAsync(site, c->sSite.p, (size_t)S * 4, hipMemcpyDeviceToHost, c->stream));
    HIPCHK(c, hipMemcpyAsync(mod, c->sMod.p, (size_t)S * 8, hipMemcpyDeviceToHost, c->stream));
    return sync_and_check(c);
}

int m6a_infer(m6a_ctx *c, const float *X, const uint8_t *km, const int64_t *off, int64_t S, int T, int K,
              float thr, uint32_t seed, int rng_mode, int64_t bs, int64_t spb, float *rp, float *site, double *mod)
{
    settle(c);
    HintScope hint_scope(c);
    if (c && c->job.open) return job_busy(c);
    int rc = check_pool_args(c, S, T, K, rng_mode, bs, spb);
    if (rc) return rc;
    if (S == 0) return M6A_OK;
    if (!X || !km || !off || !site || !mod) return fail(c, M6A_EINVAL, "null pointer argument");
    HIPCHK(c, hipSetDevice(c->device));
    const bool dev = is_device_ptr(X);
    if (dev != is_device_ptr(km) || dev != is_device_ptr(off) || dev != is_device_ptr(site) ||
        dev != is_device_ptr(mod) || (rp && dev != is_device_ptr(rp)))
        return fail(c, M6A_EINVAL, "all data pointers must be host pointers or all device pointers");
    if (dev) {
        rc = bag_stats(c, off, S);
        if (rc) return rc;
        const int64_t R = c->n_reads;
        float *p = rp;
        if (!p) { HIPCHK(c, c->rp_scratch.ensure((size_t)std::max<int64_t>(R, 1) * 4)); p = (float *)c->rp_scratch.p; }
        HIPCHK(c, hipEventRecord(c->ev_main, c->stream));
        rc = launch_encode(c, X, km, off, S, R, p);
        if (rc) return rc;
        rc = pool_setup_aside(c, off, S, T, K, seed, bs, spb);
        if (rc) return rc;
        return launch_pool(c, p, off, S, T, K, thr, seed, bs, spb, site, mod);
    }
    if (off[0] != 0) return fail(c, M6A_EINVAL, "off[0] must be 0");
    for (int64_t s = 0; s < S; s++) if (off[s + 1] < off[s]) return fail(c, M6A_EINVAL, "off[] must be non-decreasing");
    const int64_t R = off[S];
    HIPCHK(c, c->sSite.ensure((size_t)S * 4));
    HIPCHK(c, c->sMod.ensure((size_t)S * 8));
    host_bag_range(c, off, S);
    Prefault pf_rp, pf_out;
    if (rp) pf_rp.start(rp, (size_t)R * 4, 2);
    pf_out.start(mod, (size_t)S * 8, 1);
    rc = staged_encode(c, X, km, off, S, R, rp);
    if (rc) return rc;
    rc = launch_pool(c, (const float *)c->sP.p, (const int64_t *)c->sOff.p, S, T, K, thr, seed, bs, spb,
                     (float *)c->sSite.p, (double *)c->sMod.p);
    if (rc) return rc;
    return staged_outputs(c, S, site, mod);
}

int m6a_bag_forward(m6a_ctx *c, const float *X, const uint8_t *km, int64_t B, int bag, float *site)
{
    settle(c);
    HintScope hint_scope(c);
    if (c && c->job.open) return job_busy(c);
    if (!c) return M6A_EINVAL;
    if (B < 0 || bag < 1) return fail(c, M6A_EINVAL, "n_bags must be >= 0 and bag >= 1");
    if (B == 0) return M6A_OK;
    if (!X || !km || !site) return fail(c, M6A_EINVAL, "null pointer argument");
    HIPCHK(c, hipSetDevice(c->device));
    const bool dev = is_device_ptr(X);
    if (dev != is_device_ptr(km) || dev != is_device_ptr(site))
        return fail(c, M6A_EINVAL, "X, site_kmers, site_prob must be all host or all device pointers");
    const int64_t R = B * bag;
    HIPCHK(c, c->off_scratch.ensure((size_t)(B + 1) * 8));
    HIPCHK(c, c->rp_scratch.ensure((size_t)R * 4));
    int64_t *d_off = (int64_t *)c->off_scratch.p;
    float *d_p = (float *)c->rp_scratch.p;
    hipLaunchKernelGGL(iota_off_kernel, dim3((unsigned)((B + 1 + 255) / 256)), dim3(256), 0, c->stream, d_off, B + 1, (int64_t)bag);
    HIPCHK(c, hipGetLastError());
    const float *dX = X; const uint8_t *dK = km; float *dS = site;
    if (!dev) {
        HIPCHK(c, c->sX.ensure((size_t)R * 9 * 4));
        HIPCHK(c, c->sK.ensure((size_t)B * 3));
        HIPCHK(c, c->sSite.ensure((size_t)B * 4));
        HIPCHK(c, hipMemcpyAsync(c->sX.p, X, (size_t)R * 9 * 4, hipMemcpyHostToDevice, c->stream));
        HIPCHK(c, hipMemcpyAsync(c->sK.p, km, (size_t)B * 3, hipMemcpyHostToDevice, c->stream));
        dX = (const float *)c->sX.p; dK = (const uint8_t *)c->sK.p; dS = (float *)c->sSite.p;
    }
    c->bag_min = c->bag_max = bag; c->n_reads = R;
    int rc = launch_encode(c, dX, dK, d_off, B, R, d_p);
    if (rc) return rc;
    hipLaunchKernelGGL(bag_noisy_or_kernel, dim3((unsigned)((B + 255) / 256)), dim3(256), 0, c->stream, d_p, B, bag, dS);
    HIPCHK(c, hipGetLastError());
    if (!dev) {
        HIPCHK(c, hipMemcpyAsync(site, dS, (size_t)B * 4, hipMemcpyDeviceToHost, c->stream));
        HIPCHK(c, hipStreamSynchronize(c->stream));
    }
    return M6A_OK;
}

int64_t m6a_flush_groups(int64_t S, int64_t bs, int64_t spb, int64_t *group_off, int64_t cap)
{
    if (S < 0 || bs < 1 || spb < 1 || !group_off) return M6A_EINVAL;
    std::vector<int64_t> g;
    const int64_t G = flush_groups(S, bs, spb, 0, g);
    if (cap < G + 1) return M6A_EINVAL;
    std::copy(g.begin(), g.end(), group_off);
    return G;
}

int64_t m6a_reference_written_sites(int64_t S, int64_t bs, int64_t spb)
{
    if (S < 0 || bs < 1 || spb < 1) return M6A_EINVAL;
    const int64_t nb = (S + bs - 1) / bs;
    for (int64_t b = nb - 1; b >= 0; b--)
        if ((b + 1) % spb) return std::min((b + 1) * bs, S);
    return 0;
}

int m6a_shard_plan(const int64_t *off, int64_t S, int64_t bs, int64_t spb, int n_shards, int64_t *shard_off)
{
    if (!off || !shard_off || S < 0 || n_shards < 1 || bs < 1 || spb < 1) return M6A_EINVAL;
    std::vector<int64_t> g;
    const int64_t G = flush_groups(S, bs, spb, 0, g);
    const int64_t R = S > 0 ? off[S] : 0;
    shard_off[0] = 0;
    int64_t gi = 0;
    for (int k = 1; k <= n_shards; k++) {
        if (k == n_shards) { shard_off[k] = S; break; }
        const double target = (double)R * k / n_shards;
        while (gi < G && (double)off[g[gi]] < target) gi++;
        if (gi > 0 && gi <= G) {
            const double hi = (double)off[g[std::min(gi, G)]], lo = (double)off[g[gi - 1]];
            if (target - lo < hi - target && g[gi - 1] >= shard_off[k - 1]) gi--;
        }
        shard_off[k] = std::max(g[std::min(gi, G)], shard_off[k - 1]);
    }
    return M6A_OK;
}

int m6a_random_stream(m6a_ctx *c, uint32_t seed, int64_t n_words, uint32_t *words)
{
    settle(c);
    if (!c) return M6A_EINVAL;
    if (n_words < 0 || n_words > ((int64_t)1 << 31) - 2048) return fail(c, M6A_EINVAL, "n_words out of range");
    if (n_words == 0) return M6A_OK;
    if (!words) return fail(c, M6A_EINVAL, "null pointer argument");
    HIPCHK(c, hipSetDevice(c->device));
    if (is_device_ptr(words)) return launch_stream(c, seed, n_words, words);
    HIPCHK(c, c->val_idx.ensure((size_t)n_words * 4));
    int rc = launch_stream(c, seed, n_words, (uint32_t *)c->val_idx.p);
    if (rc) return rc;
    rc = d2h_through_ring(c, words, c->val_idx.p, (size_t)n_words * 4);
    if (rc) return rc;
    return sync_and_check(c);
}

int m6a_device_count(void)
{
    int n = 0;
    if (hipGetDeviceCount(&n) != hipSuccess) { (void)hipGetLastError(); return 0; }
    return n;
}

int m6a_profile_enable(m6a_ctx *c, int on)
{
    if (!c) return M6A_EINVAL;
    if (on && !c->prof.d_clk) {
        HIPCHK(c, hipSetDevice(c->device));
        HIPCHK(c, hipMalloc((void **)&c->prof.d_clk, (size_t)2 * M6A_CLK_SLOTS * 4 * sizeof(unsigned long long)));
    }
    if (on) HIPCHK(c, hipMemsetAsync(c->prof.d_clk, 0, (size_t)2 * M6A_CLK_SLOTS * 4 * sizeof(unsigned long long), c->stream));
    c->prof.on = on != 0;
    c->prof.mask = on == 2 ? 1 : on == 3 ? 2 : 3;
    c->prof.used[0] = c->prof.used[1] = 0;
    c->prof.dropped[0] = c->prof.dropped[1] = 0;
    return M6A_OK;
}

int m6a_profile_read(m6a_ctx *c, int kind, double *total_ms, int64_t *n_launches)
{
    settle(c);
    if (!c || kind < 0 || kind > 1 || !total_ms || !n_launches) return M6A_EINVAL;
    HIPCHK(c, hipSetDevice(c->device));
    HIPCHK(c, hipStreamSynchronize(c->stream));
    double tot = 0;
    for (int i = 0; i < c->prof.used[kind]; i++) {
        float ms = 0;
        HIPCHK(c, hipEventElapsedTime(&ms, c->prof.start[kind][i], c->prof.stop[kind][i]));
        tot += ms;
    }
    *total_ms = tot;
    *n_launches = c->prof.used[kind];
    return M6A_OK;
}

int m6a_profile_clock(m6a_ctx *c, int kind, double *ghz_median, double *ghz_min, double *ghz_max, double *span_ms, int *n_waves)
{
    settle(c);
    if (!c || kind < 0 || kind > 1) return M6A_EINVAL;
    if (!c->prof.d_clk) return fail(c, M6A_EINVAL, "m6a_profile_clock: profiling was never enabled on this context");
    HIPCHK(c, hipSetDevice(c->device));
    HIPCHK(c, hipStreamSynchronize(c->stream));
    unsigned long long h[M6A_CLK_SLOTS * 4];
    HIPCHK(c, hipMemcpy(h, c->prof.d_clk + (size_t)kind * M6A_CLK_SLOTS * 4, sizeof h, hipMemcpyDeviceToHost));
    std::vector<double> ghz;
    unsigned long long r_first = ~0ull, r_last = 0;
    for (int i = 0; i < M6A_CLK_SLOTS; i++) {
        const unsigned long long c0 = h[4 * i], r0 = h[4 * i + 1], c1 = h[4 * i + 2], r1 = h[4 * i + 3];
        if (!r0 || r1 <= r0 || c1 <= c0) continue;
        ghz.push_back((double)(c1 - c0) / (double)(r1 - r0) * 0.1);
        r_first = std::min(r_first, r0);
        r_last = std::max(r_last, r1);
    }
    std::sort(ghz.begin(), ghz.end());
    const bool any = !ghz.empty();
    if (ghz_median) *ghz_median = any ? ghz[ghz.size() / 2] : 0.0;
    if (ghz_min) *ghz_min = any ? ghz.front() : 0.0;
    if (ghz_max) *ghz_max = any ? ghz.back() : 0.0;
    if (span_ms) *span_ms = any ? (double)(r_last - r_first) * 1e-5 : 0.0;
    if (n_waves) *n_waves = (int)ghz.size();
    return M6A_OK;
}

const char *m6a_last_pool_variant(const m6a_ctx *c) { return c ? c->pool_variant : "none"; }

}
```

m6anet_amd/csrc/m6a_ctx.h:

```cpp
#pragma once
#include <hip/hip_runtime.h>
#include <dlfcn.h>
#include <sys/mman.h>

#include <algorithm>
#include <atomic>
#include <cmath>
#include <cstdarg>
#include <cstdio>
#include <cstdlib>
#include <cstring>
#include <condition_variable>
#include <functional>
#include <memory>
#include <mutex>
#include <new>
#include <string>
#include <thread>
#include <vector>

#include "m6a.h"
#include "m6a_kernels.h"
#include "m6a_host_cpus.h"




struct DevBuf {
    void *p = nullptr;
    size_t cap = 0;
    hipError_t ensure(size_t bytes)
    {
        if (bytes <= cap) return hipSuccess;
        if (p) (void)hipFree(p);
        p = nullptr; cap = 0;
        size_t want = bytes + bytes / 8 + 256;
        hipError_t e = hipMalloc(&p, want);
        if (e == hipSuccess) cap = want;
        return e;
    }
    void release() { if (p) (void)hipFree(p); p = nullptr; cap = 0; }
};

constexpr int kMaxProfiled = 8192;

struct Profiler {
    unsigned long long *d_clk = nullptr;
    unsigned long long *clk_for(int kind) const { return on && (mask >> kind & 1) ? d_clk + (size_t)kind * M6A_CLK_SLOTS * 4 : nullptr; }
    bool on = false;
    int mask = 3;
    std::vector<hipEvent_t> start[2], stop[2];
    int used[2] = {0, 0};
    int64_t dropped[2] = {0, 0};
};


class CopyPool {
public:
    explicit CopyPool(int n_threads)
    {
        for (int i = 0; i < n_threads; i++) workers_.emplace_back([this] { loop(); });
    }
    ~CopyPool()
    {
        { std::lock_guard<std::mutex> g(mu_); stop_ = true; }
        cv_job_.notify_all();
        for (auto &t : workers_) t.join();
    }
    void copy(void *dst, const void *src, size_t n)
    {
        const size_t parts = std::max<size_t>(1, std::min<size_t>(workers_.size() + 1, n / ((size_t)256 << 10)));
        if (parts == 1) { std::memcpy(dst, src, n); return; }
        const size_t slice = ((n + parts - 1) / parts + 4095) & ~(size_t)4095;
        {
            std::lock_guard<std::mutex> g(mu_);
            dst_ = (char *)dst; src_ = (const char *)src; n_ = n; slice_ = slice; next_ = 0; pending_ = (n + slice - 1) / slice;
        }
        cv_job_.notify_all();
        work();
        std::unique_lock<std::mutex> g(mu_);
        cv_done_.wait(g, [this] { return pending_ == 0; });
    }

private:
    bool work()
    {
        bool any = false;
        for (;;) {
            size_t off;
            {
                std::lock_guard<std::mutex> g(mu_);
                if (next_ * slice_ >= n_) return any;
                off = next_++ * slice_;
            }
            std::memcpy(dst_ + off, src_ + off, std::min(slice_, n_ - off));
            any = true;
            std::lock_guard<std::mutex> g(mu_);
            if (--pending_ == 0) cv_done_.notify_all();
        }
    }
    void loop()
    {
        for (;;) {
            {
                std::unique_lock<std::mutex> g(mu_);
                cv_job_.wait(g, [this] { return stop_ || next_ * slice_ < n_; });
                if (stop_) return;
            }
            work();
        }
    }
    std::vector<std::thread> workers_;
    std::mutex mu_;
    std::condition_variable cv_job_, cv_done_;
    char *dst_ = nullptr; const char *src_ = nullptr;
    size_t n_ = 0, slice_ = 1, next_ = 0, pending_ = 0;
    bool stop_ = false;
};

class Prefault {
public:
    Prefault() = default;
    void start(void *p, size_t bytes, int n_threads)
    {
        if (!p || bytes < ((size_t)4 << 20)) return;
        char *b = (char *)p;
        const size_t page = 4096;
        const size_t first = (page - ((uintptr_t)b & (page - 1))) & (page - 1);
        if (first >= bytes) return;
        const size_t n_pages = (bytes - first) / page;
        for (int t = 0; t < n_threads; t++)
            th_.emplace_back([=] {
                const size_t p0 = n_pages * (size_t)t / (size_t)n_threads, p1 = n_pages * (size_t)(t + 1) / (size_t)n_threads;
                char *lo = b + first + p0 * page, *hi = b + first + p1 * page;
                bool populate = true;
                for (char *q = lo; q < hi;) {
                    const size_t len = std::min<size_t>((size_t)2 << 20, (size_t)(hi - q));
                    if (populate && madvise(q, len, 23 ) != 0) populate = false;
                    if (!populate)
                        for (size_t o = 0; o < len; o += page) __atomic_fetch_add(q + o, (char)0, __ATOMIC_RELAXED);
                    q += len;
                }
            });
    }
    void join() { for (auto &t : th_) t.join(); th_.clear(); }
    ~Prefault() { join(); }
private:
    std::vector<std::thread> th_;
};

constexpr int kStageSlots = 3;
struct Staging {
    hipStream_t s_h2d = nullptr, s_d2h = nullptr;
    char *pin_in[kStageSlots] = {nullptr, nullptr, nullptr};
    char *pin_out[kStageSlots] = {nullptr, nullptr, nullptr};
    hipEvent_t ev_h2d[kStageSlots] = {nullptr, nullptr, nullptr}, ev_enc[kStageSlots] = {nullptr, nullptr, nullptr},
               ev_d2h[kStageSlots] = {nullptr, nullptr, nullptr};
    int64_t chunk_reads = 0;
    std::unique_ptr<CopyPool> pool;
    bool ready = false;
};

struct MeanPlan {
    int T = 0;
    std::vector<int> leaf_start;
    std::vector<uint8_t> merge_after;
    std::vector<uint32_t> row_meta;
    std::vector<int> row_pass, row_round;
    std::vector<uint32_t> reg_ctl;
    int n_rem = 0;
    int depth = 1;
    int max_merge = 0;
};

struct m6a_ctx {
    int device = 0;
    int n_cu = 256;
    hipStream_t own_stream = nullptr;
    hipStream_t stream = nullptr;
    std::string err;
    float *d_wfrag = nullptr, *d_wfrag2 = nullptr, *d_w1e = nullptr, *d_emb = nullptr;
    float b3 = 0.f;
    DevBuf raw, tab, tab_reg, goff, rp_scratch, off_scratch, start_pos, plan_dev;
    MeanPlan plan; size_t plan_off[4] = {0, 0, 0, 0};
    uint32_t raw_seed = 0; int64_t raw_len = 0;
    struct { uint32_t seed; int n, T, K, jmax; bool valid; } tab_key = {0, 0, 0, 0, 0, false}, tab_reg_key = {0, 0, 0, 0, 0, false};
    int table_variant = 0;
    struct { int64_t S, bs, spb, base, G, gmax; bool valid; } goff_key = {0, 0, 0, 0, 0, 0, false};
    int64_t job_offset = 0;
    int64_t bag_min = 0, bag_max = 0, n_reads = 0;
    int enc_variant = 0;
    const char *enc_variant_used = "none";
    const char *enc_kernel_used = "none";
    int scan_driver = 0;
    int *d_err = nullptr;
    unsigned long long *d_minmax = nullptr;
    unsigned long long *h_minmax = nullptr;
    int *h_err = nullptr;
    uint32_t *h_hist = nullptr, *d_hist = nullptr;
    std::vector<uint32_t> hist_part;
    uint32_t *h_ctl = nullptr;
    DevBuf ctl_dev, rt_rank, rt_order;
    bool side_work = false;
    const int64_t *hint_off = nullptr;
    hipEvent_t ev_ctl = nullptr;
    hipStream_t s_prep = nullptr;
    hipEvent_t ev_main = nullptr, ev_prep = nullptr;
    struct { bool ready = false, use = false; const int64_t *off = nullptr; int64_t S = 0, bs = 0, spb = 0; int T = 0, K = 0; uint32_t seed = 0; } prep;
    struct {
        bool valid = false; uint32_t seed = 0; int64_t A = 0, n_blk = 0;
        int cap = 0, used = 0;
        uint16_t *C = nullptr; uint32_t *RS = nullptr;
        int32_t slot_of_n[M6A_RTAB_MAX_N + 1];
    } rt;
    DevBuf sX, sK, sOff, sP, sSite, sMod, val_idx, val_y, val_avg, sOffChunk;
    Staging stg;
    std::vector<void *> graveyard;
    int rt_presize = 0;
    uint32_t rt_credit_seed = 0; int64_t rt_credit_A = 0, rt_credit = 0;
    struct Job {
        bool open = false;
        int failed = 0;
        std::string failed_msg;
        int T = 0, K = 0; float thr = 0.f; uint32_t seed = 0; int64_t bs = 1, spb = 1;
        std::vector<int64_t> off;
        int64_t S = 0, R = 0;
        int n_sub = 0; size_t sub_bytes = 0, o_goff = 0, o_km = 0, o_x = 0;
        int64_t cap_sites = 0, cap_reads = 0;
        std::vector<char *> pin;
        std::vector<hipEvent_t> ev_h2d, ev_enc;
        std::vector<char> used;
        int64_t item = 0;
        int64_t fill_sites = 0, fill_reads = 0, fill_min = INT64_MAX;
        bool cur_ready = false;
        int64_t chunks = 0;
    } job;
    DevBuf gSite, gMod, gP;
    DevBuf jX, jP, jOff;
    DevBuf mt_scratch; int64_t mt_polys_G = 0;
    std::vector<int> iter_of;
    std::thread warm;
    void *comm = nullptr;
    int comm_rank = 0, comm_world = 0;
    Profiler prof;
    const char *pool_variant = "none";
};

namespace m6a_detail {

int fail(m6a_ctx *c, int code, const char *fmt, ...);

#define HIPCHK(c, expr)                                                                    \
    do {                                                                                   \
        hipError_t e_ = (expr);                                                            \
        if (e_ != hipSuccess) {                                                            \
            (void)hipGetLastError();                                                       \
            return fail((c), e_ == hipErrorOutOfMemory ? M6A_ENOMEM : M6A_EHIP, "%s: %s (%s:%d)", \
                        #expr, hipGetErrorString(e_), __FILE__, __LINE__);                 \
        }                                                                                  \
    } while (0)

bool is_device_ptr(const void *p);
inline void settle(m6a_ctx *c) { if (c && c->warm.joinable()) c->warm.join(); }
int job_busy(m6a_ctx *c);
int check_pool_args(m6a_ctx *c, int64_t S, int T, int K, int rng_mode, int64_t bs, int64_t spb);
int deferred_error(m6a_ctx *c);
int sync_and_check(m6a_ctx *c);
struct HintScope {
    m6a_ctx *c;
    explicit HintScope(m6a_ctx *ctx) : c(ctx) {}
    ~HintScope() { if (c) c->hint_off = nullptr; }
};
int ensure_raw(m6a_ctx *c, uint32_t seed, int64_t len);
int launch_stream(m6a_ctx *c, uint32_t seed, int64_t len, uint32_t *raw);
int launch_encode(m6a_ctx *c, const float *X, const uint8_t *km, const int64_t *off, int64_t S, int64_t R, float *rp);
int launch_pool(m6a_ctx *c, const float *rp, const int64_t *off, int64_t S, int T, int K, float thr, uint32_t seed, int64_t bs, int64_t spb,
                float *site, double *mod, bool dry = false);
int bag_stats(m6a_ctx *c, const int64_t *d_off, int64_t S);
void host_bag_range(m6a_ctx *c, const int64_t *off, int64_t S);
void prof_begin(m6a_ctx *c, int kind);
void prof_end(m6a_ctx *c, int kind);
int ensure_staging(m6a_ctx *c);
void release_staging(m6a_ctx *c);
int staged_encode(m6a_ctx *c, const float *X, const uint8_t *km, const int64_t *off, int64_t S, int64_t R, float *rp_host);
int staged_outputs(m6a_ctx *c, int64_t S, float *site, double *mod);
int d2h_through_ring(m6a_ctx *c, void *host, const void *dev, size_t bytes);
bool base_is_group_start(int64_t base, int64_t bs, int64_t spb);
void comm_release(m6a_ctx *c);

}
```

m6anet_amd/csrc/m6a_kernels.h:

```cpp
#ifndef M6A_KERNELS_H
#define M6A_KERNELS_H
#include <hip/hip_runtime.h>
#include <stdint.h>

#define M6A_BAG_LDS 1024
#define M6A_WFRAG_FLOATS (136 * 64)
#define M6A_WFRAG2_FLOATS (25 * 64)
#define M6A_W1E_FLOATS (35 * 32)
#define M6A_BN_FLOATS (5 * 2 * 16 * 2)
#define M6A_MEAN_STACK 32
#define M6A_CSITE_MIN_BAG 16
#define M6A_TABLE_MAX_N 32
#define M6A_REG_STACK 8
#define M6A_RTAB_MAX_N 4096
#define M6A_RTAB_SMALL_N 1024
#define M6A_RTAB_U8_MAX_N 256
#define M6A_HIST_BINS (M6A_RTAB_MAX_N + 2)

__host__ __device__ inline unsigned long long m6a_bin_weight(int i)
{
    unsigned long long z = (unsigned long long)(i + 1) * 0x9E3779B97F4A7C15ull;
    z = (z ^ (z >> 30)) * 0xBF58476D1CE4E5B9ull;
    z = (z ^ (z >> 27)) * 0x94D049BB133111EBull;
    return z ^ (z >> 31);
}

#define M6A_CLK_SLOTS 64
__device__ __forceinline__ void m6a_clk_stamp(unsigned long long *clk, int which)
{
    if (!clk) return;
    const unsigned stride = (gridDim.x >> 6) | 1u, b = blockIdx.x;
    if (threadIdx.x == 0 && b % stride == 0 && b / stride < M6A_CLK_SLOTS) {
        unsigned long long *p = clk + (size_t)(b / stride) * 4 + which * 2;
        p[0] = __builtin_amdgcn_s_memtime();
        p[1] = __builtin_amdgcn_s_memrealtime();
    }
}

struct EncArgs {
    const float *X;
    const uint8_t *site_kmers;
    const int64_t *off;
    const float *wfrag;
    const float *wfrag2;
    const float *w1e_tab;
    const float *bn;
    const float *emb;
    float *read_prob;
    int *err;
    int64_t n_sites, n_reads, n_tiles, tiles_per_wave;
    float b3;
    unsigned long long *clk;
};

struct PoolArgs {
    const float *read_prob;
    const int64_t *off;
    const int64_t *goff;
    const uint32_t *raw;
    const uint32_t *tab;
    float *site_prob;
    double *mod_ratio;
    uint32_t *start_pos;
    const int *leaf_start;
    const uint8_t *merge_after;
    const uint32_t *row_meta;
    int n_leaves, n_rows, n_rem;
    int stack_depth;
    const uint32_t *reg_ctl;
    int reg_rounds, reg_final_merges;
    int64_t reg_items;
    int *err;
    int64_t n_groups, n_sites, raw_len;
    int T, K, uniform_n, jmax, bag_cap;
    float thr;
    unsigned long long *clk;
};

struct RtabBuild {
    const uint32_t *raw;
    uint32_t n_blk;
    const int32_t *build_n;
    const int32_t *build_slot;
    int n_build;
    uint16_t *C;
    uint32_t *RS;
    int64_t c_stride;
};
struct RtabUse {
    const uint16_t *C;
    const uint32_t *RS;
    const int32_t *slot_of_n;
    uint32_t *rank;
    const uint32_t *order;
    int64_t c_stride;
    uint32_t n_blk;
    int bag_cap;
    uint32_t si_base, si_count;
};

__global__ void enc_kernel(EncArgs a);
__global__ void enc_site16_kernel(EncArgs a);
__global__ void enc_csite_kernel(EncArgs a);
__global__ void pool_scan_start_kernel(PoolArgs a);
template <int KT> __global__ void pool_scan_group_kernel(PoolArgs a);
template <int KT> __global__ void pool_scan_site_kernel(PoolArgs a);
__global__ void pool_table_kernel(PoolArgs a);
__global__ void pool_reg_kernel(PoolArgs a);
__global__ void bag_noisy_or_kernel(const float *read_prob, int64_t n_bags, int bag, float *site_prob);
__global__ void iota_off_kernel(int64_t *off, int64_t n_plus_1, int64_t step);
__global__ void rebase_off_kernel(const int64_t *off, int64_t count, int64_t *out);
__global__ void sampled_noisy_or_kernel(const float *read_prob, const int32_t *gidx, int64_t n_bags, int k, float *y);
__global__ void mean_over_passes_kernel(const float *y, int n_iters, int64_t n_sites, float *avg);
__global__ void pairwise_mean_kernel(const float *y, int n_iters, float *avg);
__global__ void bag_minmax_kernel(const int64_t *off, int64_t n_sites, unsigned long long *out, uint32_t *hist);
__global__ void bag_verify_kernel(const unsigned long long *got, const uint32_t *hist, unsigned long long mn, unsigned long long mx,
                                  unsigned long long reads, unsigned long long hash, int *err);
__global__ void mt19937_kernel(uint32_t seed, int64_t n_words, uint32_t *raw, const uint32_t *hist, int64_t seg_words, uint32_t *xhead, int64_t xhead_n);
__global__ void mt_jump_kernel(const uint32_t *xhead, const uint64_t *polys, uint32_t *hist);
__global__ void rtab_count_kernel(RtabBuild a);
__global__ void rtab_scan_kernel(RtabBuild a);
__global__ void rtab_fill_kernel(RtabBuild a);
__global__ void rtab_to_reg_table_kernel(const uint16_t *C, int64_t A, int64_t row_words, int jmax, uint16_t *tab);
__global__ void rtab_to_lds_table_kernel(const uint16_t *C, int64_t A, int K, int rows, int jmax, const int *iter_of, uint32_t *tab);
__global__ void rtab_prep_kernel(PoolArgs a, RtabUse u, uint32_t *cursor, uint32_t *order, unsigned n_order_blocks);
template <int KT> __global__ void pool_rtab_kernel(PoolArgs a, RtabUse u);

__global__ void m6a_touch_kernels();
__global__ void m6a_touch_pool_reg();
__global__ void m6a_touch_pool_rtab();

#endif
```

m6anet_amd/csrc/m6a_kernels.hip:

```cpp
#include <hip/hip_runtime.h>
#include <stdint.h>

#include "m6a_kernels.h"

typedef float f32x16 __attribute__((ext_vector_type(16)));
typedef float f32x2 __attribute__((ext_vector_type(2)));

__device__ __forceinline__ float chain8_sum(float r)
{
    r += __builtin_bit_cast(float, __builtin_amdgcn_update_dpp(0, __builtin_bit_cast(int, r), 0xB1, 0xf, 0xf, false));
    r += __builtin_bit_cast(float, __builtin_amdgcn_update_dpp(0, __builtin_bit_cast(int, r), 0x4E, 0xf, 0xf, false));
    r += __builtin_bit_cast(float, __builtin_amdgcn_update_dpp(0, __builtin_bit_cast(int, r), 0x141, 0xf, 0xf, false));
    return r;
}

__device__ __forceinline__ int wave_sum_i32(int v)
{
#pragma unroll
    for (int m = 1; m < 64; m <<= 1) v += __shfl_xor(v, m, 64);
    return v;
}

#define L2_REGS(m) ((m) == 4 ? 12 : 16)

// ... 141 lines not shown
    const int q = (int)qf;
    float s = __builtin_fmaf(qf, -0.693145751953125f, d);
    s = __builtin_fmaf(qf, -1.428606765330187045e-06f, s);
    float u = 0.000198527617612853646278381f;
    u = __builtin_fmaf(u, s, 0.00139304355252534151077271f);
    u = __builtin_fmaf(u, s, 0.00833336077630519866943359f);
    u = __builtin_fmaf(u, s, 0.0416664853692054748535156f);
    u = __builtin_fmaf(u, s, 0.166666671633720397949219f);
    u = __builtin_fmaf(u, s, 0.5f);
    u = 1.0f + __builtin_fmaf(s * s, u, s);
    const int q1 = q >> 1;
    u = u * ldexpf(1.0f, q1) * ldexpf(1.0f, q - q1);
    u = d < -104.0f ? 0.0f : u;
    return d > 104.0f ? __builtin_inff() : u;
}

__device__ __forceinline__ float gemv32_as_mkl(const f32x16 &acc2, const float (&w)[16], int half)
{
    float r[16];
#pragma unroll
    for (int q = 0; q < 16; q++) r[q] = relu2(acc2[q]);
    const float k0 = r[15] * w[15];
    float k0_other = __shfl_xor(k0, 32, 64);
    asm volatile("" : "+v"(k0_other));
    const float s0 = half ? 0.0f : k0_other;
    float v[8];
    v[0] = __builtin_fmaf(r[0], w[0], s0);
#pragma unroll
    for (int q = 1; q < 8; q++) v[q] = r[q] * w[q];
    float c = ((v[0] + v[4]) + (v[2] + v[6])) + ((v[1] + v[5]) + (v[3] + v[7]));
    float c_other = __shfl_xor(c, 32, 64);
    asm volatile("" : "+v"(c_other));
    const float t1 = c + c_other;
    v[0] = __builtin_fmaf(r[8], w[8], half ? 0.0f : t1);
#pragma unroll
    for (int q = 1; q < 7; q++) v[q] = r[8 + q] * w[8 + q];
    v[7] = half ? 0.0f : k0;
    c = ((v[0] + v[4]) + (v[2] + v[6])) + ((v[1] + v[5]) + (v[3] + v[7]));
    c_other = __shfl_xor(c, 32, 64);
    asm volatile("" : "+v"(c_other));
    return c + c_other;
}

__device__ __forceinline__ int64_t uniform_i64(int64_t v)
{
    return ((int64_t)__builtin_amdgcn_readfirstlane((int)(v >> 32)) << 32) |
           (uint32_t)__builtin_amdgcn_readfirstlane((int)v);
}

__device__ __forceinline__ void wave_lds_fence()
{
    __builtin_amdgcn_fence(__ATOMIC_ACQ_REL, "wavefront");
    __builtin_amdgcn_wave_barrier();
}

struct EncTile {
    float f[8];
    int64_t s_last;
};

__global__ __launch_bounds__(256, 2) void enc_kernel(EncArgs a)
{
    clamp_keeps_nan();
    m6a_clk_stamp(a.clk, 0);
    __shared__ float s_emb[132];
    __shared__ __attribute__((aligned(16))) float s_bn[M6A_BN_FLOATS];
    for (int i = threadIdx.x; i < 132; i += 256) s_emb[i] = a.emb[i];
#ifdef M6A_AB_BN_PK
    for (int i = threadIdx.x; i < M6A_BN_FLOATS; i += 256) s_bn[i] = a.bn[(i & ~3) | ((i & 1) << 1) | ((i & 2) >> 1)];
#else
    for (int i = threadIdx.x; i < M6A_BN_FLOATS; i += 256) s_bn[i] = a.bn[i];
#endif
    __syncthreads();

    const int lane = threadIdx.x & 63;
    const int col = lane & 31;
    const int half = lane >> 5;
    const float *bn_half = s_bn + half * 32;
    const int64_t wave = (int64_t)blockIdx.x * 4 + __builtin_amdgcn_readfirstlane((int)(threadIdx.x >> 6));
    const int64_t tile0 = wave * a.tiles_per_wave;
    if (tile0 >= a.n_tiles) return;
    const int64_t tile1 = (tile0 + a.tiles_per_wave < a.n_tiles) ? tile0 + a.tiles_per_wave : a.n_tiles;

    float w1[40], w2[80], w3[16];
#pragma unroll
    for (int i = 0; i < 40; i++) w1[i] = a.wfrag[i * 64 + lane];
#pragma unroll
    for (int i = 0; i < 80; i++) w2[i] = a.wfrag[(40 + i) * 64 + lane];
#pragma unroll
    for (int i = 0; i < 16; i++) w3[i] = a.wfrag[(120 + i) * 64 + lane];

    int64_t s_base;
    {
        const int64_t r = tile0 * 32;
        int64_t lo = 0, hi = a.n_sites;
        while (hi - lo > 1) {
            int64_t mid = (lo + hi) >> 1;
            if (a.off[mid] <= r) lo = mid; else hi = mid;
        }
        s_base = lo;
    }
    const int64_t last_site = a.n_sites - 1;

    auto link0 = [&](int64_t base, int64_t (&o)[3]) {
#pragma unroll
        for (int i = 0; i < 3; i++) {
            const int64_t si = base + 1 + i;
            o[i] = a.off[si <= a.n_sites ? si : a.n_sites];
        }
    };
    auto link1 = [&](int64_t tile, int64_t base, const int64_t (&o)[3], int64_t &s, int (&km)[3], float (&x)[8]) {
        const int64_t r = tile * 32 + col;
        const int64_t rc = r < a.n_reads ? r : a.n_reads - 1;
        s = base + (rc >= o[0] ? 1 : 0) + (rc >= o[1] ? 1 : 0);
        if (__any(rc >= o[2])) {
            s = base;
            while (a.off[s + 1] <= rc) ++s;
        }
        s = s < last_site ? s : last_site;
        const uint8_t *kp = a.site_kmers + s * 3;
        km[0] = kp[0]; km[1] = kp[1]; km[2] = kp[2];
        const float *xp = a.X + rc * 9 + half;
#pragma unroll
        for (int i = 0; i < 4; i++) x[i] = xp[2 * i];
        x[4] = xp[half ? 6 : 8];
    };
    auto link2 = [&](const int (&km)[3], float (&x)[8]) {
        const float e0 = s_emb[2 * km[0] + 1 - half], e1 = s_emb[2 * km[1] + 1 - half], e2 = s_emb[2 * km[2] + 1 - half];
        x[4] = half ? e0 : x[4];
        x[5] = half ? e1 : e0;
        x[6] = half ? e2 : e1;
        x[7] = half ? 1.0f : e2;
    };

    float f[8];
    s_base = uniform_i64(s_base);
    {
        int64_t o[3], s;
        int km[3];
        link0(s_base, o);
        link1(tile0, s_base, o, s, km, f);
        link2(km, f);
        s_base = uniform_i64(__shfl(s, 31, 64));
    }

    BnPairs bnq;
    bn_pairs_load(bnq, bn_half);
    for (int64_t tile = tile0; tile < tile1; ++tile) {
        const int64_t tn = tile + 1 < tile1 ? tile + 1 : tile;
        float fn[8];
        int64_t o[3], sn;
        int km[3];
        link0(s_base, o);
        tile_body_priority();

        f32x16 acc2, h1a, h1b;
#pragma unroll
        for (int q = 0; q < 16; q++) { acc2[q] = 0.0f; h1a[q] = 0.0f; }
#pragma unroll
        for (int st = 0; st < 8; st++)
            h1a = __builtin_amdgcn_mfma_f32_32x32x2f32(w1[st], f[st], h1a, 0, 0, 0);
#pragma unroll
        for (int m = 0; m < 5; m++) {
            f32x16 &cur = (m & 1) ? h1b : h1a;
            f32x16 &nxt = (m & 1) ? h1a : h1b;
            if (m < 4) {
#pragma unroll
                for (int q = 0; q < 16; q++) nxt[q] = 0.0f;
#pragma unroll
                for (int st = 0; st < 8; st++)
                    nxt = __builtin_amdgcn_mfma_f32_32x32x2f32(w1[(m + 1) * 8 + st], f[st], nxt, 0, 0, 0);
            }
            __builtin_amdgcn_sched_barrier(0);
            if (m == 0) link1(tn, s_base, o, sn, km, fn);
            if (m == 2) link2(km, fn);
            if (m == 0) layer2_with_bn<0>(acc2, cur, w2, bnq, bn_half);
            if (m == 1) layer2_with_bn<1>(acc2, cur, w2, bnq, bn_half);
            if (m == 2) layer2_with_bn<2>(acc2, cur, w2, bnq, bn_half);
            if (m == 3) layer2_with_bn<3>(acc2, cur, w2, bnq, bn_half);
            if (m == 4) layer2_with_bn<4>(acc2, cur, w2, bnq, bn_half);
        }
        tile_epilogue_priority();
        const float z = gemv32_as_mkl(acc2, w3, half) + a.b3;
        const float p = 1.0f / (1.0f + sleef_expf_u10(-z));
        const int64_t r = tile * 32 + col;
        if (half == 0 && r < a.n_reads) a.read_prob[r] = p;
        if (tn != tile) s_base = uniform_i64(__shfl(sn, 31, 64));
#pragma unroll
        for (int i = 0; i < 8; i++) f[i] = fn[i];
    }
    m6a_clk_stamp(a.clk, 1);
}

#ifdef M6A_AB_STAMPS
#define M6A_AB_STAMP_TILES 16
#define M6A_AB_STAMP_FIRST 100
#define M6A_AB_STAMP_POINTS 10
__device__ unsigned long long m6a_ab_stamp_buf[4096][M6A_AB_STAMP_TILES][M6A_AB_STAMP_POINTS];
__device__ unsigned m6a_ab_stamp_hw[4096][2];
extern "C" int m6a_ab_read_stamps(unsigned long long *stamps, unsigned *hw)
{
    if (hipMemcpyFromSymbol(stamps, HIP_SYMBOL(m6a_ab_stamp_buf), sizeof(m6a_ab_stamp_buf)) != hipSuccess) return -1;
    if (hipMemcpyFromSymbol(hw, HIP_SYMBOL(m6a_ab_stamp_hw), sizeof(m6a_ab_stamp_hw)) != hipSuccess) return -1;
    return 0;
}
#define M6A_STAMP(k) do { __builtin_amdgcn_sched_barrier(0); ts[k] = __builtin_amdgcn_s_memtime(); __builtin_amdgcn_sched_barrier(0); } while (0)
#else
#define M6A_STAMP(k) do { } while (0)
#endif
__global__ __launch_bounds__(256, M6A_SITE16_WAVES_PER_SIMD) void enc_site16_kernel(EncArgs a)
{
    clamp_keeps_nan();
    m6a_clk_stamp(a.clk, 0);
    __shared__ float s_emb[132];
    __shared__ __attribute__((aligned(16))) float s_bn[M6A_BN_FLOATS];
    for (int i = threadIdx.x; i < 132; i += 256) s_emb[i] = a.emb[i];
#ifdef M6A_AB_BN_PK
    for (int i = threadIdx.x; i < M6A_BN_FLOATS; i += 256) s_bn[i] = a.bn[(i & ~3) | ((i & 1) << 1) | ((i & 2) >> 1)];
#else
    for (int i = threadIdx.x; i < M6A_BN_FLOATS; i += 256) s_bn[i] = a.bn[i];
#endif
#ifdef M6A_AB_W3
    __shared__ float4 s_w2q[19 * 64];
    for (int idx = threadIdx.x; idx < 19 * 64; idx += 256) {
        const int g = idx >> 6, ln = idx & 63, u = (g >> 2) * 16 + (g & 3) * 4;
        s_w2q[idx] = make_float4(a.wfrag[(40 + u) * 64 + ln], a.wfrag[(41 + u) * 64 + ln], a.wfrag[(42 + u) * 64 + ln], a.wfrag[(43 + u) * 64 + ln]);
    }
#endif
    __syncthreads();

    const int lane = threadIdx.x & 63;
    const int col = lane & 31;
    const int half = lane >> 5;
    const float *bn_half = s_bn + half * 32;
    const int wave = (int)blockIdx.x * 4 + __builtin_amdgcn_readfirstlane((int)(threadIdx.x >> 6));
    const int n_tiles = (int)a.n_tiles, tpw = (int)a.tiles_per_wave;
    const int tile0 = wave * tpw;
    if (tile0 >= n_tiles) return;
    const int tile1 = (tile0 + tpw < n_tiles) ? tile0 + tpw : n_tiles;
    const int n_sites = (int)a.n_sites;
    const int last_lim = (int)(a.n_reads - 1 - (int64_t)(n_tiles - 1) * 32);

#ifdef M6A_AB_W3
    float w1[40], w3[16];
    float4 wq[2];
    const float4 *w2lane = s_w2q + lane;
    wq[0] = w2lane[0];
#pragma unroll
    for (int i = 0; i < 40; i++) w1[i] = a.wfrag[i * 64 + lane];
#else
    float w1[40], w2[80], w3[16];
#pragma unroll
    for (int i = 0; i < 40; i++) w1[i] = a.wfrag[i * 64 + lane];
#pragma unroll
    for (int i = 0; i < 80; i++) w2[i] = a.wfrag[(40 + i) * 64 + lane];
#endif
#pragma unroll
    for (int i = 0; i < 16; i++) w3[i] = a.wfrag[(120 + i) * 64 + lane];

    int s_base;
    {
        const int64_t r = (int64_t)tile0 * 32;
        int lo = 0, hi = n_sites;
        while (hi - lo > 1) {
            const int mid = (int)(((int64_t)lo + hi) >> 1);
            if (a.off[mid] <= r) lo = mid; else hi = mid;
        }
        s_base = lo;
    }
    const int last_site = n_sites - 1;

    const __attribute__((address_space(4))) int64_t *off_c = (const __attribute__((address_space(4))) int64_t *)a.off;
    auto link0 = [&](int base, int64_t (&o)[3]) {
#pragma unroll
        for (int i = 0; i < 3; i++) {
            const int si = base + 1 + i;
            o[i] = off_c[si <= n_sites ? si : n_sites];
        }
    };
    const int kq = lane < 18 ? lane : 17;
    const int kq_site = kq / 6, kq_byte = (kq % 6) / 2;
    int too_small = 0;
    auto link1 = [&](int tile, int base, const int64_t (&o)[3], int &rel, int &kid, float (&x)[8]) {
        const int64_t rbase = (int64_t)tile * 32;
        const int lim = tile == n_tiles - 1 ? last_lim : 31;
        const int crel = col < lim ? col : lim;
        const int d0 = (int)o[0] - (int)rbase, d1 = (int)o[1] - (int)rbase, d2 = (int)o[2] - (int)rbase;
        rel = (crel >= d0 ? 1 : 0) + (crel >= d1 ? 1 : 0);
        too_small |= lim >= d2 ? 1 : 0;
        const int room = last_site - base;
        const int ksr = kq_site < room ? kq_site : room;
#ifdef M6A_AB_ADDR64
        kid = (int)(a.site_kmers + (int64_t)base * 3)[ksr * 3 + kq_byte];
#else
        kid = (int)(a.site_kmers + (int64_t)base * 3)[__umul24((unsigned)ksr, 3u) + (unsigned)kq_byte];
#endif
#ifdef M6A_AB_ADDR64
        const float *xp = a.X + rbase * 9 + (crel * 9 + half);
#pragma unroll
        for (int i = 0; i < 4; i++) x[i] = xp[2 * i];
        x[4] = xp[half ? 6 : 8];
#else
        const float *xt = a.X + rbase * 9;
        const float *xp = (const float *)((const char *)xt + (unsigned)(4 * (crel * 9 + half)));
#pragma unroll
        for (int i = 0; i < 4; i++) x[i] = xp[2 * i];
        x[4] = *(const float *)((const char *)xt + (unsigned)(4 * (crel * 9 + (half ? 7 : 8))));
#endif
    };
    auto link2 = [&](int kid, float &ev) { ev = s_emb[2 * kid + (lane & 1)]; };
    auto link3 = [&](float ev, int rel, float (&x)[8]) {
        const int ebits = __builtin_bit_cast(int, ev);
        const int addr = 4 * (rel * 6 + 1 - half);
        const float e0 = __builtin_bit_cast(float, __builtin_amdgcn_ds_bpermute(addr, ebits));
        const float e1 = __builtin_bit_cast(float, __builtin_amdgcn_ds_bpermute(addr + 8, ebits));
        const float e2 = __builtin_bit_cast(float, __builtin_amdgcn_ds_bpermute(addr + 16, ebits));
        x[4] = half ? e0 : x[4];
        x[5] = half ? e1 : e0;
        x[6] = half ? e2 : e1;
        x[7] = half ? 1.0f : e2;
    };

    float f[8];
    s_base = __builtin_amdgcn_readfirstlane(s_base);
    {
        int64_t o[3];
        int rel, kid;
        float ev;
        link0(s_base, o);
        link1(tile0, s_base, o, rel, kid, f);
        link2(kid, ev);
        link3(ev, rel, f);
        s_base += __builtin_amdgcn_readfirstlane(__shfl(rel, 31, 64));
    }

    phase_shift_second_workgroup();
    BnPairs bnq;
    bn_pairs_load(bnq, bn_half);
    for (int tile = tile0; tile < tile1; ++tile) {
        const int tn = tile + 1 < tile1 ? tile + 1 : tile;
        float fn[8], evn;
        int64_t o[3];
        int reln, kidn;
#ifdef M6A_AB_STAMPS
        unsigned long long ts[M6A_AB_STAMP_POINTS];
#endif
        M6A_STAMP(0);
        link0(s_base, o);
        tile_body_priority();

        f32x16 acc2, h1a, h1b;
#pragma unroll
        for (int q = 0; q < 16; q++) { acc2[q] = 0.0f; h1a[q] = 0.0f; }
#pragma unroll
        for (int st = 0; st < 8; st++)
            h1a = __builtin_amdgcn_mfma_f32_32x32x2f32(w1[st], f[st], h1a, 0, 0, 0);
        M6A_STAMP(1);
#pragma unroll
        for (int m = 0; m < 5; m++) {
            f32x16 &cur = (m & 1) ? h1b : h1a;
            f32x16 &nxt = (m & 1) ? h1a : h1b;
#ifndef M6A_AB_L2_FIRST
            if (m < 4) {
#pragma unroll
                for (int q = 0; q < 16; q++) nxt[q] = 0.0f;
#pragma unroll
                for (int st = 0; st < 8; st++)
                    nxt = __builtin_amdgcn_mfma_f32_32x32x2f32(w1[(m + 1) * 8 + st], f[st], nxt, 0, 0, 0);
            }
            __builtin_amdgcn_sched_barrier(0);
#endif
#ifndef M6A_AB_LINK1_AT
#define M6A_AB_LINK1_AT 1
#define M6A_AB_LINK2_AT 2
#define M6A_AB_LINK3_AT 3
#endif
#ifdef M6A_AB_NO_LINKS
            if (m == 0) {
#pragma unroll
                for (int i = 0; i < 8; i++) fn[i] = f[i];
                reln = 0; kidn = 0; evn = 0.0f;
            }
#else
            if (m == M6A_AB_LINK1_AT) link1(tn, s_base, o, reln, kidn, fn);
            if (m == M6A_AB_LINK2_AT) link2(kidn, evn);
            if (m == M6A_AB_LINK3_AT) link3(evn, reln, fn);
#endif
#ifdef M6A_AB_W3
            if (m == 0) layer2_with_bn_lds<0>(acc2, cur, wq, w2lane, bnq, bn_half);
            if (m == 1) layer2_with_bn_lds<1>(acc2, cur, wq, w2lane, bnq, bn_half);
            if (m == 2) layer2_with_bn_lds<2>(acc2, cur, wq, w2lane, bnq, bn_half);
            if (m == 3) layer2_with_bn_lds<3>(acc2, cur, wq, w2lane, bnq, bn_half);
            if (m == 4) layer2_with_bn_lds<4>(acc2, cur, wq, w2lane, bnq, bn_half);
#else
            if (m == 0) layer2_with_bn<0>(acc2, cur, w2, bnq, bn_half);
            if (m == 1) layer2_with_bn<1>(acc2, cur, w2, bnq, bn_half);
            if (m == 2) layer2_with_bn<2>(acc2, cur, w2, bnq, bn_half);
            if (m == 3) layer2_with_bn<3>(acc2, cur, w2, bnq, bn_half);
            if (m == 4) layer2_with_bn<4>(acc2, cur, w2, bnq, bn_half);
#endif
#ifdef M6A_AB_L2_FIRST
            if (m < 4) {
#pragma unroll
                for (int q = 0; q < 16; q++) nxt[q] = 0.0f;
#pragma unroll
                for (int st = 0; st < 8; st++)
                    nxt = __builtin_amdgcn_mfma_f32_32x32x2f32(w1[(m + 1) * 8 + st], f[st], nxt, 0, 0, 0);
            }
            __builtin_amdgcn_sched_barrier(0);
#endif
            M6A_STAMP(2 + m);
        }
        tile_epilogue_priority();
#ifdef M6A_AB_NO_EPILOGUE
        const float p = (acc2[0] + acc2[5]) + w3[0];
#else
        const float z = gemv32_as_mkl(acc2, w3, half) + a.b3;
        M6A_STAMP(7);
        const float p = 1.0f / (1.0f + sleef_expf_u10(-z));
#endif
        if (half == 0 && col <= (tile == n_tiles - 1 ? last_lim : 31)) (a.read_prob + (int64_t)tile * 32)[col] = p;
        M6A_STAMP(8);
        if (tn != tile) s_base += __builtin_amdgcn_readfirstlane(__shfl(reln, 31, 64));
#pragma unroll
        for (int i = 0; i < 8; i++) f[i] = fn[i];
#ifdef M6A_AB_STAMPS
        M6A_STAMP(9);
        {
            const int k = tile - tile0 - M6A_AB_STAMP_FIRST;
            if (k >= 0 && k < M6A_AB_STAMP_TILES && wave < 4096 && lane == 0) {
#pragma unroll
                for (int i = 0; i < M6A_AB_STAMP_POINTS; i++) m6a_ab_stamp_buf[wave][k][i] = ts[i];
                if (k == 0) {
                    m6a_ab_stamp_hw[wave][0] = __builtin_amdgcn_s_getreg(4 | (0 << 6) | (31 << 11));
                    m6a_ab_stamp_hw[wave][1] = __builtin_amdgcn_s_getreg(20 | (0 << 6) | (31 << 11));
                }
            }
        }
#endif
    }
    if (too_small && lane == 0) atomicExch(a.err, 2);
    m6a_clk_stamp(a.clk, 1);
}

__global__ __launch_bounds__(256, 2) void enc_csite_kernel(EncArgs a)
{
    clamp_keeps_nan();
    m6a_clk_stamp(a.clk, 0);
    __shared__ float s_emb[132];
    __shared__ float s_w1e[35 * 32];
    for (int i = threadIdx.x; i < 132; i += 256) s_emb[i] = a.emb[i];
    for (int i = threadIdx.x; i < 35 * 32; i += 256) s_w1e[i] = a.w1e_tab[i];
    __shared__ __attribute__((aligned(16))) float s_bn[M6A_BN_FLOATS];
#ifdef M6A_AB_BN_PK
    for (int i = threadIdx.x; i < M6A_BN_FLOATS; i += 256) s_bn[i] = a.bn[(i & ~3) | ((i & 1) << 1) | ((i & 2) >> 1)];
#else
    for (int i = threadIdx.x; i < M6A_BN_FLOATS; i += 256) s_bn[i] = a.bn[i];
#endif
    __shared__ float s_w3[32];
    if (threadIdx.x < 64) s_w3[(threadIdx.x >> 5) * 16 + (threadIdx.x & 15)] = a.wfrag[(120 + (threadIdx.x & 15)) * 64 + (threadIdx.x & 32)];
    __syncthreads();

    const int lane = threadIdx.x & 63;
    const int col = lane & 31;
    const int half = lane >> 5;
    const float *bn_half = s_bn + half * 32;
    const int wave = (int)blockIdx.x * 4 + __builtin_amdgcn_readfirstlane((int)(threadIdx.x >> 6));
    const int n_tiles = (int)a.n_tiles, tpw = (int)a.tiles_per_wave;
    const int tile0 = wave * tpw;
    if (tile0 >= n_tiles) return;
    const int tile1 = (tile0 + tpw < n_tiles) ? tile0 + tpw : n_tiles;
    const int n_sites = (int)a.n_sites;
    const int last_lim = (int)(a.n_reads - 1 - (int64_t)(n_tiles - 1) * 32);

    float w1x[20], w8[5], w2[80];
#pragma unroll
    for (int i = 0; i < 20; i++) w1x[i] = a.wfrag2[i * 64 + lane];
#pragma unroll
    for (int i = 0; i < 5; i++) w8[i] = a.wfrag2[(20 + i) * 64 + lane];
#pragma unroll
    for (int i = 0; i < 80; i++) w2[i] = a.wfrag[(40 + i) * 64 + lane];

    int s_base;
    {
        const int64_t r = (int64_t)tile0 * 32;
        int lo = 0, hi = n_sites;
        while (hi - lo > 1) {
            const int mid = (int)(((int64_t)lo + hi) >> 1);
            if (a.off[mid] <= r) lo = mid; else hi = mid;
        }
        s_base = lo;
    }
    const int last_site = n_sites - 1;

    const __attribute__((address_space(4))) int64_t *off_c = (const __attribute__((address_space(4))) int64_t *)a.off;
    auto link0 = [&](int base, int64_t (&o)[3]) {
#pragma unroll
        for (int i = 0; i < 3; i++) {
            const int si = base + 1 + i;
            o[i] = off_c[si <= n_sites ? si : n_sites];
        }
    };
    const int kq = lane < 18 ? lane : 17;
    const int kq_site = kq / 6, kq_byte = (kq % 6) / 2;
    int too_small = 0;
    auto link1 = [&](int tile, int base, const int64_t (&o)[3], int &rel, int &kid, float (&x)[5]) {
        const int64_t rbase = (int64_t)tile * 32;
        const int lim = tile == n_tiles - 1 ? last_lim : 31;
        const int crel = col < lim ? col : lim;
        const int d0 = (int)o[0] - (int)rbase, d1 = (int)o[1] - (int)rbase, d2 = (int)o[2] - (int)rbase;
        rel = (crel >= d0 ? 1 : 0) + (crel >= d1 ? 1 : 0);
        too_small |= lim >= d2 ? 1 : 0;
        const int room = last_site - base;
        const int ksr = kq_site < room ? kq_site : room;
#ifdef M6A_AB_ADDR64
        kid = (int)(a.site_kmers + (int64_t)base * 3)[ksr * 3 + kq_byte];
#else
        kid = (int)(a.site_kmers + (int64_t)base * 3)[__umul24((unsigned)ksr, 3u) + (unsigned)kq_byte];
#endif
#ifdef M6A_AB_ADDR64
        const float *xp = a.X + rbase * 9 + (crel * 9 + half);
#pragma unroll
        for (int i = 0; i < 4; i++) x[i] = xp[2 * i];
        x[4] = xp[half ? 6 : 8];
#else
        const float *xt = a.X + rbase * 9;
        const float *xp = (const float *)((const char *)xt + (unsigned)(4 * (crel * 9 + half)));
#pragma unroll
        for (int i = 0; i < 4; i++) x[i] = xp[2 * i];
        x[4] = *(const float *)((const char *)xt + (unsigned)(4 * (crel * 9 + (half ? 7 : 8))));
#endif
    };
    auto link2 = [&](int kid, float &ev) { ev = s_emb[2 * kid + (lane & 1)]; };
    auto link3 = [&](float ev, int rel, float x8, float (&x)[6], float (&a4)[5], float (&a5)[5]) {
        const int ebits = __builtin_bit_cast(int, ev);
        const int lane_b = half ? 48 : 24;
        int lane_a;
        asm("v_mov_b32 %0, 0" : "=v"(lane_a));
        f32x2 e2[6];
#pragma unroll
        for (int q = 0; q < 6; q++) {
            e2[q].x = __builtin_bit_cast(float, __builtin_amdgcn_ds_bpermute(lane_a + 4 * q, ebits));
            e2[q].y = __builtin_bit_cast(float, __builtin_amdgcn_ds_bpermute(lane_b + 4 * q, ebits));
        }
#pragma unroll
        for (int m = 0; m < 5; m++) {
            const float *wr = s_w1e + (m * 7) * 32 + col;
#ifdef M6A_AB_CSITE_SCALAR_FMA
            float cx = wr[6 * 32], cy = cx;
#pragma unroll
            for (int q = 0; q < 6; q++) {
                const float wq = wr[q * 32];
                asm("v_fma_f32 %0, %1, %2, %0" : "+v"(cx) : "v"(wq), "v"(e2[q].x));
                asm("v_fma_f32 %0, %1, %2, %0" : "+v"(cy) : "v"(wq), "v"(e2[q].y));
            }
            const f32x2 c = {cx, cy};
#else
            f32x2 c = {wr[6 * 32], wr[6 * 32]};
#pragma unroll
            for (int q = 0; q < 6; q++) {
                const float wq = wr[q * 32];
                const f32x2 w2v = {wq, wq};
                c = __builtin_elementwise_fma(w2v, e2[q], c);
            }
#endif
            a4[m] = half ? c.x : w8[m];
            a5[m] = c.y;
#ifdef M6A_AB_CSITE_PIN
            asm volatile("" : "+v"(a4[m]), "+v"(a5[m]));
#endif
        }
        x[4] = half ? (rel == 0 ? 1.0f : 0.0f) : x8;
        x[5] = (rel == (half ? 2 : 1)) ? 1.0f : 0.0f;
    };

    float f[6], a4[5], a5[5];
    s_base = __builtin_amdgcn_readfirstlane(s_base);
    {
        int64_t o[3];
        int rel, kid;
        float ev, x5[5];
        link0(s_base, o);
        link1(tile0, s_base, o, rel, kid, x5);
#pragma unroll
        for (int i = 0; i < 4; i++) f[i] = x5[i];
        link2(kid, ev);
        link3(ev, rel, x5[4], f, a4, a5);
        s_base += __builtin_amdgcn_readfirstlane(__shfl(rel, 31, 64));
    }

    BnPairs bnq;
    bn_pairs_load(bnq, bn_half);
    for (int tile = tile0; tile < tile1; ++tile) {
        const int tn = tile + 1 < tile1 ? tile + 1 : tile;
        float fn[5], evn;
        int64_t o[3];
        int reln, kidn;
        link0(s_base, o);
        tile_body_priority();

        auto layer1 = [&](int m, f32x16 &acc) {
#pragma unroll
            for (int q = 0; q < 16; q++) acc[q] = 0.0f;
#pragma unroll
            for (int st = 0; st < 4; st++)
                acc = __builtin_amdgcn_mfma_f32_32x32x2f32(w1x[m * 4 + st], f[st], acc, 0, 0, 0);
            acc = __builtin_amdgcn_mfma_f32_32x32x2f32(a4[m], f[4], acc, 0, 0, 0);
            acc = __builtin_amdgcn_mfma_f32_32x32x2f32(a5[m], f[5], acc, 0, 0, 0);
        };

        f32x16 acc2, h1a, h1b;
#pragma unroll
        for (int q = 0; q < 16; q++) acc2[q] = 0.0f;
        layer1(0, h1a);
#pragma unroll
        for (int m = 0; m < 5; m++) {
            f32x16 &cur = (m & 1) ? h1b : h1a;
            f32x16 &nxt = (m & 1) ? h1a : h1b;
            if (m < 4) layer1(m + 1, nxt);
            __builtin_amdgcn_sched_barrier(0);
            if (m == 0) link1(tn, s_base, o, reln, kidn, fn);
            if (m == 1) link2(kidn, evn);
            if (m == 3) link3(evn, reln, fn[4], f, a4, a5);
            if (m == 0) layer2_with_bn<0>(acc2, cur, w2, bnq, bn_half);
            if (m == 1) layer2_with_bn<1>(acc2, cur, w2, bnq, bn_half);
            if (m == 2) layer2_with_bn<2>(acc2, cur, w2, bnq, bn_half);
            if (m == 3) layer2_with_bn<3>(acc2, cur, w2, bnq, bn_half);
            if (m == 4) layer2_with_bn<4>(acc2, cur, w2, bnq, bn_half);
        }
        tile_epilogue_priority();
        float z = 0.0f;
#pragma unroll
        for (int q = 0; q < 16; q++) z = fmaf(relu2(acc2[q]), s_w3[half * 16 + q], z);
        z += __shfl_xor(z, 32, 64);
        z += a.b3;
        const float p = 1.0f / (1.0f + expf(-z));
        if (half == 0 && col <= (tile == n_tiles - 1 ? last_lim : 31)) (a.read_prob + (int64_t)tile * 32)[col] = p;
        if (tn != tile) s_base += __builtin_amdgcn_readfirstlane(__shfl(reln, 31, 64));
#pragma unroll
        for (int i = 0; i < 4; i++) f[i] = fn[i];
    }
    if (too_small && lane == 0) atomicExch(a.err, 2);
    m6a_clk_stamp(a.clk, 1);
}

__device__ __forceinline__ uint32_t pow2_mask(uint32_t rng)
{
    uint32_t mask = rng;
    mask |= mask >> 1; mask |= mask >> 2; mask |= mask >> 4; mask |= mask >> 8; mask |= mask >> 16;
    return mask;
}

__device__ __forceinline__ int ring_addr(int s) { return s + (s >> 2); }

template <int KT>
__device__ __forceinline__ float window_product(const float *ring, int wbase, int lane, int K)
{
    float prod = 1.0f;
    if (KT && (KT % 4 == 0)) {
        const float *row = ring + (wbase + lane * KT) * 5 / 4;
#pragma unroll
        for (int k = 0; k < KT; k++) prod *= row[k + (k >> 2)];
    } else {
        const int base = wbase + lane * K;
        for (int k = 0; k < K; k++) prod *= ring[ring_addr(base + k)];
    }
    return prod;
}

template <int KT>
__device__ __forceinline__ bool scan_site(const PoolArgs &a, int64_t s, uint32_t &pos, float *bag, float *ring,
                                          int lane, int K)
{
    float *stack = ring + (32 * K + 256) * 5 / 4 + 32;
    pos = (uint32_t)__builtin_amdgcn_readfirstlane((int)pos);
// ... 531 lines not shown
    int64_t i = 8;
    for (; i < n - (n % 8); i += 8)
        for (int k = 0; k < 8; k++) r[k] += a[i + k];
    float res = ((r[0] + r[1]) + (r[2] + r[3])) + ((r[4] + r[5]) + (r[6] + r[7]));
    for (; i < n; i++) res += a[i];
    return res;
}

__global__ void pairwise_mean_kernel(const float *y, int n_iters, float *avg)
{
    if (blockIdx.x != 0 || threadIdx.x != 0) return;
    struct Frame { int64_t off, n; float left; bool right; };
    Frame st[32];
    int sp = 0;
    st[0] = {0, n_iters, 0.0f, false};
    float sum;
    for (;;) {
        Frame &f = st[sp];
        if (f.n > 128) {
            const int64_t n2 = (f.n / 2) - (f.n / 2) % 8;
            st[++sp] = {f.off, n2, 0.0f, false};
            continue;
        }
        sum = pairwise_leaf(y + f.off, f.n);
        for (;;) {
            if (sp == 0) { avg[0] = sum / (float)n_iters; return; }
            Frame &p = st[--sp];
            const int64_t n2 = (p.n / 2) - (p.n / 2) % 8;
            if (!p.right) {
                p.left = sum;
                p.right = true;
                st[++sp] = {p.off + n2, p.n - n2, 0.0f, false};
                break;
            }
            sum = p.left + sum;
        }
    }
}

__global__ void rebase_off_kernel(const int64_t *off, int64_t count, int64_t *out)
{
    const int64_t i = (int64_t)blockIdx.x * blockDim.x + threadIdx.x;
    if (i < count) out[i] = off[i] - off[0];
}

__global__ void iota_off_kernel(int64_t *off, int64_t n_plus_1, int64_t step)
{
    const int64_t i = (int64_t)blockIdx.x * blockDim.x + threadIdx.x;
    if (i < n_plus_1) off[i] = i * step;
}

__global__ __launch_bounds__(256) void bag_minmax_kernel(const int64_t *off, int64_t n_sites, unsigned long long *out, uint32_t *hist)
{
    __shared__ int64_t s_mn[4], s_mx[4];
    __shared__ uint32_t s_hist[M6A_HIST_BINS];
    for (int i = threadIdx.x; i < M6A_HIST_BINS; i += 256) s_hist[i] = 0;
    __syncthreads();
    int64_t mn = INT64_MAX, mx = 0;
    for (int64_t s = (int64_t)blockIdx.x * blockDim.x + threadIdx.x; s < n_sites;
         s += (int64_t)gridDim.x * blockDim.x) {
        const int64_t n = off[s + 1] - off[s];
        mn = n < mn ? n : mn;
        mx = n > mx ? n : mx;
        atomicAdd(&s_hist[n < 0 ? 0 : n > M6A_RTAB_MAX_N ? M6A_RTAB_MAX_N + 1 : n], 1u);
    }
#pragma unroll
    for (int m = 1; m < 64; m <<= 1) {
        const int64_t omn = __shfl_xor(mn, m, 64), omx = __shfl_xor(mx, m, 64);
        mn = omn < mn ? omn : mn;
        mx = omx > mx ? omx : mx;
    }
    if ((threadIdx.x & 63) == 0) { s_mn[threadIdx.x >> 6] = mn; s_mx[threadIdx.x >> 6] = mx; }
    __syncthreads();
    for (int i = threadIdx.x; i < M6A_HIST_BINS; i += 256)
        if (s_hist[i]) atomicAdd(&hist[i], s_hist[i]);
    if (threadIdx.x == 0) {
        for (int w = 1; w < 4; w++) { mn = s_mn[w] < mn ? s_mn[w] : mn; mx = s_mx[w] > mx ? s_mx[w] : mx; }
        atomicMin(&out[0], (unsigned long long)mn);
        atomicMax(&out[1], (unsigned long long)mx);
        if (blockIdx.x == 0) out[2] = (unsigned long long)off[n_sites];
    }
}

__global__ __launch_bounds__(256) void bag_verify_kernel(const unsigned long long *got, const uint32_t *hist, unsigned long long mn,
                                                         unsigned long long mx, unsigned long long reads, unsigned long long hash, int *err)
{
    __shared__ unsigned long long s_part[256];
    unsigned long long h = 0;
    for (int i = threadIdx.x; i < M6A_HIST_BINS; i += 256) h += (unsigned long long)hist[i] * m6a_bin_weight(i);
    s_part[threadIdx.x] = h;
    __syncthreads();
    if (threadIdx.x == 0) {
        for (int i = 1; i < 256; i++) h += s_part[i];
        if (got[0] != mn || got[1] != mx || got[2] != reads || h != hash) atomicExch(err, 3);
    }
}

__global__ void m6a_touch_kernels() {}
```

m6anet_amd/csrc/m6a_validate.hip:

```cpp
#include "m6a_ctx.h"

using namespace m6a_detail;

namespace m6a_detail {


struct MtBulk {
    uint32_t s[624], out[624];
    int pos = 624;
    explicit MtBulk(uint32_t seed)
    {
        uint32_t x = seed;
        s[0] = x;
        for (uint32_t i = 1; i < 624; i++) { x = 1812433253u * (x ^ (x >> 30)) + i; s[i] = x; }
    }
    static inline uint32_t tw(uint32_t a, uint32_t b)
    {
        const uint32_t y = (a & 0x80000000u) | (b & 0x7fffffffu);
        return (y >> 1) ^ ((0u - (y & 1u)) & 0x9908b0dfu);
    }
    __attribute__((always_inline)) inline void refill_body()
    {
        for (int k = 0; k < 227; k++) s[k] = s[k + 397] ^ tw(s[k], s[k + 1]);
        for (int k = 227; k < 623; k++) s[k] = s[k - 227] ^ tw(s[k], s[k + 1]);
// ... 231 lines not shown
        hipLaunchKernelGGL(mean_over_passes_kernel, dim3((unsigned)((S + 255) / 256)), dim3(256), 0, c->stream,
                           (const float *)d_y, T, S, d_avg);
    prof_end(c, 1);
    HIPCHK(c, hipGetLastError());
    HIPCHK(c, hipStreamSynchronize(c->stream));
    return M6A_OK;
}

int check_validate_args(m6a_ctx *c, int64_t S, int T, int K)
{
    if (!c) return M6A_EINVAL;
    if (S < 0) return fail(c, M6A_EINVAL, "n_sites < 0");
    if (T < 1) return fail(c, M6A_EINVAL, "n_iters must be >= 1");
    if (K < 1 || K > M6A_MAX_SAMPLES) return fail(c, M6A_EINVAL, "n_samples must be in 1..%d", M6A_MAX_SAMPLES);
    if ((double)T * (double)S * K > 2.0e9) return fail(c, M6A_EUNSUPPORTED, "n_iters * n_sites * n_samples too large for one call");
    return M6A_OK;
}


}

extern "C" {


int m6a_validate_pool(m6a_ctx *c, const float *rp, const int64_t *off, int64_t S, int T, int K, uint32_t seed,
                      float *y, float *avg)
{
    settle(c);
    HintScope hint_scope(c);
    if (c && c->job.open) return job_busy(c);
    int rc = check_validate_args(c, S, T, K);
    if (rc) return rc;
    if (S == 0) return M6A_OK;
    if (!rp || !off || !y) return fail(c, M6A_EINVAL, "null pointer argument");
    HIPCHK(c, hipSetDevice(c->device));
    const bool dev = is_device_ptr(rp);
    if (dev != is_device_ptr(off) || dev != is_device_ptr(y) || (avg && dev != is_device_ptr(avg)))
        return fail(c, M6A_EINVAL, "read_prob, off, y_pred, y_pred_avg must be all host or all device pointers");
    std::vector<int64_t> h_off;
    const int64_t *ho = off;
    if (dev) {
        h_off.resize((size_t)S + 1);
        HIPCHK(c, hipMemcpyAsync(h_off.data(), off, (size_t)(S + 1) * 8, hipMemcpyDeviceToHost, c->stream));
        HIPCHK(c, hipStreamSynchronize(c->stream));
        ho = h_off.data();
    }
    if (ho[0] != 0) return fail(c, M6A_EINVAL, "off[0] must be 0");
    for (int64_t s = 0; s < S; s++) if (ho[s + 1] < ho[s]) return fail(c, M6A_EINVAL, "off[] must be non-decreasing");
    if (dev) return launch_validate_pool(c, rp, ho, S, T, K, seed, y, avg);
    const int64_t R = ho[S];
    HIPCHK(c, c->sP.ensure((size_t)std::max<int64_t>(R, 1) * 4));
    HIPCHK(c, c->val_y.ensure((size_t)T * S * 4));
    HIPCHK(c, c->val_avg.ensure((size_t)S * 4));
    HIPCHK(c, hipMemcpyAsync(c->sP.p, rp, (size_t)R * 4, hipMemcpyHostToDevice, c->stream));
    rc = launch_validate_pool(c, (const float *)c->sP.p, ho, S, T, K, seed, (float *)c->val_y.p, avg ? (float *)c->val_avg.p : nullptr);
    if (rc) return rc;
    HIPCHK(c, hipMemcpyAsync(y, c->val_y.p, (size_t)T * S * 4, hipMemcpyDeviceToHost, c->stream));
    if (avg) HIPCHK(c, hipMemcpyAsync(avg, c->val_avg.p, (size_t)S * 4, hipMemcpyDeviceToHost, c->stream));
    return sync_and_check(c);
}

int m6a_validate(m6a_ctx *c, const float *X, const uint8_t *km, const int64_t *off, int64_t S, int T, int K,
                 uint32_t seed, float *rp, float *y, float *avg)
{
    settle(c);
    HintScope hint_scope(c);
    if (c && c->job.open) return job_busy(c);
    int rc = check_validate_args(c, S, T, K);
    if (rc) return rc;
    if (S == 0) return M6A_OK;
    if (!X || !km || !off || !y) return fail(c, M6A_EINVAL, "null pointer argument");
    HIPCHK(c, hipSetDevice(c->device));
    const bool dev = is_device_ptr(X);
    if (dev != is_device_ptr(km) || dev != is_device_ptr(off) || dev != is_device_ptr(y) || (rp && dev != is_device_ptr(rp)) ||
        (avg && dev != is_device_ptr(avg)))
        return fail(c, M6A_EINVAL, "X, site_kmers, off and the outputs must be all host or all device pointers");
    if (dev) {
        float *d_rp = rp;
        rc = bag_stats(c, off, S);
        if (rc) return rc;
        if (!d_rp) { HIPCHK(c, c->rp_scratch.ensure((size_t)std::max<int64_t>(c->n_reads, 1) * 4)); d_rp = (float *)c->rp_scratch.p; }
        rc = launch_encode(c, X, km, off, S, c->n_reads, d_rp);
        if (rc) return rc;
        return m6a_validate_pool(c, d_rp, off, S, T, K, seed, y, avg);
    }
    if (off[0] != 0) return fail(c, M6A_EINVAL, "off[0] must be 0");
    for (int64_t s = 0; s < S; s++) if (off[s + 1] < off[s]) return fail(c, M6A_EINVAL, "off[] must be non-decreasing");
    const int64_t R = off[S];
    if (R == 0) return fail(c, M6A_EINVAL, "no reads");
    HIPCHK(c, c->sX.ensure((size_t)R * 9 * 4));
    HIPCHK(c, c->sK.ensure((size_t)S * 3));
    HIPCHK(c, c->sOff.ensure((size_t)(S + 1) * 8));
    HIPCHK(c, c->sP.ensure((size_t)R * 4));
    HIPCHK(c, c->val_y.ensure((size_t)T * S * 4));
    HIPCHK(c, c->val_avg.ensure((size_t)S * 4));
    HIPCHK(c, hipMemcpyAsync(c->sX.p, X, (size_t)R * 9 * 4, hipMemcpyHostToDevice, c->stream));
    HIPCHK(c, hipMemcpyAsync(c->sK.p, km, (size_t)S * 3, hipMemcpyHostToDevice, c->stream));
    HIPCHK(c, hipMemcpyAsync(c->sOff.p, off, (size_t)(S + 1) * 8, hipMemcpyHostToDevice, c->stream));
    host_bag_range(c, off, S);
    rc = launch_encode(c, (const float *)c->sX.p, (const uint8_t *)c->sK.p, (const int64_t *)c->sOff.p, S, R, (float *)c->sP.p);
    if (rc) return rc;
    rc = launch_validate_pool(c, (const float *)c->sP.p, off, S, T, K, seed, (float *)c->val_y.p, avg ? (float *)c->val_avg.p : nullptr);
    if (rc) return rc;
    if (rp) HIPCHK(c, hipMemcpyAsync(rp, c->sP.p, (size_t)R * 4, hipMemcpyDeviceToHost, c->stream));
    HIPCHK(c, hipMemcpyAsync(y, c->val_y.p, (size_t)T * S * 4, hipMemcpyDeviceToHost, c->stream));
    if (avg) HIPCHK(c, hipMemcpyAsync(avg, c->val_avg.p, (size_t)S * 4, hipMemcpyDeviceToHost, c->stream));
    return sync_and_check(c);
}


}
```

m6anet_amd/engine.py:

```python
import ctypes as C

import numpy as np

from . import _lib
from .constants import (DEFAULT_PRETRAINED_MODEL, DEFAULT_READ_THRESHOLD, N_SAMPLES, N_WEIGHT_FLOATS,
                        PRETRAINED_CONFIGS, asset_path)


def load_weights(pretrained_model=DEFAULT_PRETRAINED_MODEL):
    if pretrained_model not in PRETRAINED_CONFIGS:
        raise ValueError("Invalid pretrained model {}, must be one of {}".format(
            pretrained_model, list(PRETRAINED_CONFIGS)))
    w = np.fromfile(asset_path(PRETRAINED_CONFIGS[pretrained_model][0]), np.float32)
    assert w.size == N_WEIGHT_FLOATS
    return w


def weights_from_state_dict(sd):
    order = ["read_level_encoder.1.embedding_layer.weight", "read_level_encoder.3.layers.0.weight",
             "read_level_encoder.3.layers.0.bias", "read_level_encoder.3.layers.1.weight",
             "read_level_encoder.3.layers.1.bias", "read_level_encoder.3.layers.1.running_mean",
             "read_level_encoder.3.layers.1.running_var", "read_level_encoder.4.layers.0.weight",
             "read_level_encoder.4.layers.0.bias", "pooling_filter.probability_layer.0.weight",
             "pooling_filter.probability_layer.0.bias"]
# ... 118 lines not shown
        return self._L.m6a_last_encoder_kernel(self._h).decode()

    def set_scan_driver(self, mode):
        self._chk(self._L.m6a_set_scan_driver(self._h, int(mode)))

    def set_table_variant(self, mode):
        self._chk(self._L.m6a_set_table_variant(self._h, int(mode)))

    def sync(self):
        self._chk(self._L.m6a_sync(self._h))

    def set_host_offsets(self, off_host):
        if off_host is None:
            self._chk(self._L.m6a_set_host_offsets(self._h, None))
            return
        a = np.ascontiguousarray(off_host, dtype=np.int64)
        self._host_off_keepalive = a
        self._chk(self._L.m6a_set_host_offsets(self._h, a.ctypes.data))

    def comm_init(self, unique_id, rank, world_size):
        buf = (C.c_char * 128).from_buffer_copy(bytes(unique_id))
        self._chk(self._L.m6a_comm_init(self._h, buf, int(rank), int(world_size)))
        self._comm = (int(rank), int(world_size))

    def comm_info(self):
        n, r, d, v = C.c_int(0), C.c_int(-1), C.c_int(-1), C.c_int(0)
        self._chk(self._L.m6a_comm_count(self._h, C.byref(n)))
        self._chk(self._L.m6a_comm_info(self._h, C.byref(r), C.byref(d), C.byref(v)))
        return {"ranks_seen": n.value, "rank": r.value, "device": d.value, "rccl_version": v.value}

    def comm_destroy(self):
        self._chk(self._L.m6a_comm_destroy(self._h))

    def gather(self, site, mod, cuts, dst=0, out=None):
        rank, world = self._comm
        cuts = np.ascontiguousarray(cuts, np.int64)
        assert cuts.size == world + 1
        aS, aM = _Arg(site, np.float32, "float32"), _Arg(mod, np.float64, "float64")
        total = int(cuts[-1] - cuts[0])
        sa = ma = None
        if rank == dst:
            sa, ma = out if out is not None else (self._out(aS.is_dev, total, np.float32, "float32"),
                                                  self._out(aS.is_dev, total, np.float64, "float64"))
        oS = _Arg(sa, np.float32, "float32") if sa is not None else None
        oM = _Arg(ma, np.float64, "float64") if ma is not None else None
        self._chk(self._L.m6a_gather(self._h, aS.ptr, aM.ptr, cuts.ctypes.data, int(dst),
                                     oS.ptr if oS else None, oM.ptr if oM else None))
        return sa, ma

    def gather_reads(self, read_prob, read_cuts, dst=0, out=None):
        rank, world = self._comm
        cuts = np.ascontiguousarray(read_cuts, np.int64)
        assert cuts.size == world + 1
        aP = _Arg(read_prob, np.float32, "float32")
        ra = None
        if rank == dst:
            ra = out if out is not None else self._out(aP.is_dev, int(cuts[-1] - cuts[0]), np.float32, "float32")
        oP = _Arg(ra, np.float32, "float32") if ra is not None else None
        self._chk(self._L.m6a_gather_reads(self._h, aP.ptr, cuts.ctypes.data, int(dst), oP.ptr if oP else None))
        return ra

    def random_stream(self, seed, n_words):
        out = np.empty(int(n_words), np.uint32)
        self._chk(self._L.m6a_random_stream(self._h, int(seed) & 0xffffffff, int(n_words), out.ctypes.data))
        return out

    def prepare_host_io(self):
        self._chk(self._L.m6a_prepare_host_io(self._h))

    def profile(self, on=True):
        self._chk(self._L.m6a_profile_enable(self._h, {False: 0, True: 1, 'encoder': 2, 'pooling': 3}[on]))

    def profile_read(self, kind):
        ms, n = C.c_double(), C.c_int64()
        self._chk(self._L.m6a_profile_read(self._h, kind, C.byref(ms), C.byref(n)))
        return ms.value, n.value

    def profile_clock(self, kind):
        g, lo, hi, span, n = C.c_double(), C.c_double(), C.c_double(), C.c_double(), C.c_int32()
        self._chk(self._L.m6a_profile_clock(self._h, kind, C.byref(g), C.byref(lo), C.byref(hi), C.byref(span), C.byref(n)))
        if n.value == 0:
            return None
        return {"ghz": g.value, "ghz_min": lo.value, "ghz_max": hi.value, "span_ms": span.value, "waves": n.value}

    @property
    def last_pool_variant(self):
        return self._L.m6a_last_pool_variant(self._h).decode()

    def _out(self, like_dev, n, np_dtype, torch_name):
        if like_dev:
            import torch
            return torch.empty(n, dtype=getattr(torch, torch_name), device="cuda:%d" % self.device)
        a = np.empty(n, np_dtype)
        _hint_huge_pages(a)
        return a

    def get_read_probability(self, X, site_kmers, off, out=None):
        aX, aK, aO = _Arg(X, np.float32, "float32"), _Arg(site_kmers, np.uint8, "uint8"), _Arg(off, np.int64, "int64")
        S = aO.size - 1
        R = aX.size // 9
        if aK.size != 3 * S:
            raise ValueError("site_kmers must be [n_sites, 3]")
        rp = out if out is not None else self._out(aX.is_dev, R, np.float32, "float32")
        aP = _Arg(rp, np.float32, "float32")
        if aP.size != R:
            raise ValueError("read_prob must have one float per read")
        self._chk(self._L.m6a_encode_reads(self._h, aX.ptr, aK.ptr, aO.ptr, S, aP.ptr))
        return rp

    def calculate_site_proba(self, read_probs, off, n_iters, n_samples=N_SAMPLES,
                             read_proba_threshold=DEFAULT_READ_THRESHOLD, seed=0, batch_size=16,
                             save_per_batch=2):
        aP, aO = _Arg(read_probs, np.float32, "float32"), _Arg(off, np.int64, "int64")
        S = aO.size - 1
        site = self._out(aP.is_dev, S, np.float32, "float32")
        mod = self._out(aP.is_dev, S, np.float64, "float64")
        aS, aM = _Arg(site, np.float32, "float32"), _Arg(mod, np.float64, "float64")
        self._chk(self._L.m6a_site_pool(self._h, aP.ptr, aO.ptr, S, int(n_iters), int(n_samples),
                                        float(np.float32(read_proba_threshold)), int(seed) & 0xffffffff,
                                        _lib.RNG_NUMPY, int(batch_size), int(save_per_batch), aS.ptr, aM.ptr))
        return site, mod

    def infer(self, X, site_kmers, off, n_iters, n_samples=N_SAMPLES,
              read_proba_threshold=DEFAULT_READ_THRESHOLD, seed=0, batch_size=16, save_per_batch=2,
              want_read_probs=True, out=None):
        aX, aK, aO = _Arg(X, np.float32, "float32"), _Arg(site_kmers, np.uint8, "uint8"), _Arg(off, np.int64, "int64")
        S = aO.size - 1
        R = aX.size // 9
        if out is not None:
            rp, site, mod = out
        else:
            rp = self._out(aX.is_dev, R, np.float32, "float32") if want_read_probs else None
            site = self._out(aX.is_dev, S, np.float32, "float32")
            mod = self._out(aX.is_dev, S, np.float64, "float64")
        aP = _Arg(rp, np.float32, "float32") if rp is not None else None
        aS, aM = _Arg(site, np.float32, "float32"), _Arg(mod, np.float64, "float64")
        self.infer_ptrs(aX.ptr, aK.ptr, aO.ptr, S, n_iters, n_samples, read_proba_threshold, seed, batch_size, save_per_batch,
                        aP.ptr if aP else None, aS.ptr, aM.ptr)
        return rp, site, mod

    def infer_ptrs(self, X, site_kmers, off, n_sites, n_iters, n_samples=N_SAMPLES, read_proba_threshold=DEFAULT_READ_THRESHOLD,
                   seed=0, batch_size=16, save_per_batch=2, read_prob=None, site_prob=None, mod_ratio=None):
        self._chk(self._L.m6a_infer(self._h, X, site_kmers, off, int(n_sites), int(n_iters), int(n_samples),
                                    float(np.float32(read_proba_threshold)), int(seed) & 0xffffffff,
                                    _lib.RNG_NUMPY, int(batch_size), int(save_per_batch), read_prob, site_prob, mod_ratio))

    def job_begin(self, n_iters, n_samples=N_SAMPLES, read_proba_threshold=DEFAULT_READ_THRESHOLD, seed=0, batch_size=16,
                  save_per_batch=2, expect_sites=0, expect_reads=0):
        self._chk(self._L.m6a_job_begin(self._h, int(n_iters), int(n_samples), float(np.float32(read_proba_threshold)),
                                        int(seed) & 0xffffffff, _lib.RNG_NUMPY, int(batch_size), int(save_per_batch),
                                        int(expect_sites), int(expect_reads)))
        self._job_dev = False
        self._job_keep = []

    def job_feed(self, X, site_kmers, off):
        aX, aK = _Arg(X, np.float32, "float32"), _Arg(site_kmers, np.uint8, "uint8")
        if aX.is_dev or aK.is_dev:
            import torch
            cur = torch.cuda.current_stream(self.device)
            if getattr(self, "_torch_stream", None) != cur.cuda_stream:
                cur.synchronize()
            self._job_keep.append((aX.keep, aK.keep))
        o = off if (isinstance(off, np.ndarray) and off.dtype == np.int64 and off.flags.c_contiguous) else \
            np.ascontiguousarray(off.cpu().numpy() if _is_torch(off) else off, dtype=np.int64)
        n = o.size - 1
        if aK.size != 3 * n or aX.size != 9 * int(o[-1]):
# ... 125 lines not shown
```

Measured before the change: 389.7 million.

## Defer bag validation, fuse check kernels, and overlap pool setup with encode

The two bag verification kernels and their three memsets are merged into one self-resetting kernel that uses a last-block pattern. Its launch is deferred until after the encoder, so the check no longer sits in front of the main work. Pool setup on the side stream is launched before the encode in steady state, and the main stream only waits on its event when side work was actually queued. The encoder's start-site binary search now uses bag min/max bounds and constant-address loads. The change also adds clock stamps and a stamps-readout API, and the reordered cross-stream ordering and in-kernel atomics add complexity.

```diff
diff --git a/include/m6a.h b/include/m6a.h
--- a/include/m6a.h
+++ b/include/m6a.h
@@ -97,6 +97,7 @@
 int m6a_profile_enable(m6a_ctx *ctx, int on);
 int m6a_profile_read(m6a_ctx *ctx, int kind, double *total_ms, int64_t *n_launches);
 int m6a_profile_clock(m6a_ctx *ctx, int kind, double *ghz_median, double *ghz_min, double *ghz_max, double *span_ms, int *n_waves);
+int m6a_profile_stamps(m6a_ctx *ctx, int kind, unsigned long long *stamps);
 int m6a_set_encoder_variant(m6a_ctx *ctx, int mode);
 const char *m6a_last_encoder_variant(const m6a_ctx *ctx);
 const char *m6a_last_encoder_kernel(const m6a_ctx *ctx);
diff --git a/m6anet_amd/_lib.py b/m6anet_amd/_lib.py
--- a/m6anet_amd/_lib.py
+++ b/m6anet_amd/_lib.py
@@ -13,7 +13,7 @@
 SYMBOLS = ["m6a_create", "m6a_destroy", "m6a_last_error", "m6a_set_stream", "m6a_set_job_offset", "m6a_set_scan_driver", "m6a_set_table_variant", "m6a_set_encoder_variant", "m6a_last_encoder_variant", "m6a_last_encoder_kernel", "m6a_sync", "m6a_set_host_offsets", "m6a_prepare_host_io", "m6a_host_alloc", "m6a_host_free", "m6a_host_is_pinned",
            "m6a_encode_reads", "m6a_site_pool", "m6a_infer", "m6a_job_begin", "m6a_job_feed", "m6a_job_feed_collated", "m6a_job_size", "m6a_job_end", "m6a_job_abort", "m6a_bag_forward", "m6a_validate_pool", "m6a_validate", "m6a_flush_groups",
            "m6a_reference_written_sites",
-           "m6a_shard_plan", "m6a_comm_unique_id", "m6a_comm_init", "m6a_gather", "m6a_gather_reads", "m6a_device_count", "m6a_random_stream", "m6a_comm_destroy", "m6a_comm_count", "m6a_comm_info", "m6a_device_link", "m6a_profile_enable", "m6a_profile_read", "m6a_profile_clock", "m6a_last_pool_variant",
+           "m6a_shard_plan", "m6a_comm_unique_id", "m6a_comm_init", "m6a_gather", "m6a_gather_reads", "m6a_device_count", "m6a_random_stream", "m6a_comm_destroy", "m6a_comm_count", "m6a_comm_info", "m6a_device_link", "m6a_profile_enable", "m6a_profile_read", "m6a_profile_clock", "m6a_profile_stamps", "m6a_last_pool_variant",
            "m6a_version", "m6a_prep_eventalign", "m6a_prep_table", "m6a_prep_times", "m6a_prep_free", "m6a_prep_last_error",
            "m6a_prep_sites_build", "m6a_prep_sites_build_multi", "m6a_prep_sites_build_windows", "m6a_prep_sites_build_names", "m6a_prep_sites_read_names", "m6a_prep_sites_intern_ms", "m6a_prep_sites_stream_bytes", "m6a_prep_sites_n_streams", "m6a_prep_sites_get", "m6a_prep_sites_fetch", "m6a_prep_sites_inputs", "m6a_prep_sites_free",
            "m6a_csv_format", "m6a_prep_sites_write_csv", "m6a_bgzf_inflate", "m6a_bgzf_deflate", "m6a_prep_sites_write_csv_bgzf",
@@ -150,6 +150,8 @@
     L.m6a_profile_enable.argtypes = [vp, i32]
     L.m6a_profile_read.argtypes = [vp, i32, C.POINTER(C.c_double), C.POINTER(i64)]
     L.m6a_profile_clock.argtypes = [vp, i32] + [C.POINTER(C.c_double)] * 4 + [C.POINTER(i32)]
+    if hasattr(L, "m6a_profile_stamps"):
+        L.m6a_profile_stamps.argtypes = [vp, i32, vp]
     L.m6a_last_pool_variant.argtypes = [vp]
     L.m6a_last_pool_variant.restype = C.c_char_p
     L.m6a_version.restype = C.c_char_p
@@ -190,7 +192,9 @@
     L.m6a_prep_last_error.argtypes = []
     L.m6a_prep_last_error.restype = C.c_char_p
     for name in SYMBOLS:
-        fn = getattr(L, name)
+        fn = getattr(L, name, None)
+        if fn is None:
+            continue
         if fn.restype is C.c_int and name not in ("m6a_flush_groups", "m6a_reference_written_sites"):
             fn.restype = C.c_int
     _lib = L
diff --git a/m6anet_amd/csrc/m6a_api.hip b/m6anet_amd/csrc/m6a_api.hip
--- a/m6anet_amd/csrc/m6a_api.hip
+++ b/m6anet_amd/csrc/m6a_api.hip
@@ -156,6 +156,7 @@
     int64_t gmax = 0;
     for (int64_t i = 0; i < G; i++) gmax = std::max(gmax, g[i + 1] - g[i]);
     HIPCHK(c, c->goff.ensure(g.size() * sizeof(int64_t)));
+    c->side_queued = true;
     HIPCHK(c, hipMemcpyAsync(c->goff.p, g.data(), g.size() * sizeof(int64_t), hipMemcpyHostToDevice, c->stream));
     HIPCHK(c, hipStreamSynchronize(c->stream));
     c->goff_key = {S, bs, spb, base, G, gmax, true};
@@ -199,6 +200,7 @@
 int launch_stream(m6a_ctx *c, uint32_t seed, int64_t len, uint32_t *raw)
 {
     int n_reg = 0;
+    c->side_queued = true;
     const JumpRegime *reg = jump_regimes(&n_reg);
     const JumpRegime *use = nullptr;
     static const bool allowed = !(getenv("M6A_MT_SEGMENTS") && getenv("M6A_MT_SEGMENTS")[0] == '0');
@@ -317,6 +319,7 @@
 int ensure_mean_plan(m6a_ctx *c, int T)
 {
     if (c->plan.T == T && c->plan_dev.p) return M6A_OK;
+    c->side_queued = true;
     build_mean_plan(T, c->plan);
     const MeanPlan &p = c->plan;
     if (p.depth > M6A_MEAN_STACK) return fail(c, M6A_EUNSUPPORTED, "n_iters %d: pairwise-sum tree deeper than %d", T, M6A_MEAN_STACK);
@@ -410,6 +413,7 @@
         if (hipMalloc((void **)&nC, (size_t)new_cap * c_stride * 2 + 64) != hipSuccess) { (void)hipGetLastError(); return M6A_OK; }
         if (hipMalloc((void **)&nRS, (size_t)new_cap * (n_blk + 1) * 4) != hipSuccess) { (void)hipGetLastError(); (void)hipFree(nC); return M6A_OK; }
         if (!fresh && rt.used) {
+            c->side_queued = true;
             HIPCHK(c, hipMemcpyAsync(nC, rt.C, (size_t)rt.used * c_stride * 2, hipMemcpyDeviceToDevice, c->stream));
             HIPCHK(c, hipMemcpyAsync(nRS, rt.RS, (size_t)rt.used * (n_blk + 1) * 4, hipMemcpyDeviceToDevice, c->stream));
             HIPCHK(c, hipStreamSynchronize(c->stream));
@@ -417,6 +421,7 @@
         }
         rt.C = nC; rt.RS = nRS; rt.cap = new_cap;
         if (fresh) {
+            c->side_queued = true;
             HIPCHK(c, hipMemsetAsync(rt.C, 0, (size_t)c_stride * 2, c->stream));
             HIPCHK(c, hipMemsetAsync(rt.RS, 0, (size_t)(n_blk + 1) * 4, c->stream));
             rt.used = 1;
@@ -428,6 +433,7 @@
         for (size_t i = 0; i < todo.size(); i++) { bn[i] = todo[i]; bs[i] = rt.used; rt.slot_of_n[todo[i]] = rt.used++; }
         HIPCHK(c, c->ctl_dev.ensure(kCtlWords * 4));
         int32_t *d_bn = (int32_t *)c->ctl_dev.p + (ctl_build_n(c) - (int32_t *)c->h_ctl);
+        c->side_queued = true;
         HIPCHK(c, hipMemcpyAsync(d_bn, bn, (size_t)2 * M6A_RTAB_MAX_N * 4, hipMemcpyHostToDevice, c->stream));
         RtabBuild b;
         b.raw = (const uint32_t *)c->raw.p; b.n_blk = (uint32_t)n_blk; b.build_n = d_bn; b.build_slot = d_bn + M6A_RTAB_MAX_N;
@@ -456,6 +462,7 @@
     if (!usable) return fail(c, M6A_ENOMEM, "no device memory for the index table of bag size %d", n);
     const int64_t slot = c->rt.slot_of_n[n], A = (int64_t)T * K;
     uint32_t total = 0;
+    c->side_queued = true;
     HIPCHK(c, hipMemcpyAsync(&total, c->rt.RS + slot * (c->rt.n_blk + 1) + c->rt.n_blk, 4, hipMemcpyDeviceToHost, c->stream));
     HIPCHK(c, hipStreamSynchronize(c->stream));
     if ((int64_t)total < A * jmax) return fail(c, M6A_ESTREAM, "MT19937 stream too short for a flush group");
@@ -471,6 +478,7 @@
     const size_t per_j = (size_t)(T + 8) * K;
     const size_t bytes = (size_t)jmax * per_j * 2 + 4096;
     HIPCHK(c, c->tab_reg.ensure(bytes));
+    c->side_queued = true;
     HIPCHK(c, hipMemsetAsync(c->tab_reg.p, 0, bytes, c->stream));
     const uint16_t *C = nullptr;
     int rc = uniform_slice(c, seed, n, T, K, jmax, &C);
@@ -500,6 +508,7 @@
     const size_t words = (size_t)jmax * rows * 5 * 64;
     HIPCHK(c, c->tab.ensure(words * 4 + c->iter_of.size() * 4));
     int *d_iter = (int *)((uint32_t *)c->tab.p + words);
+    c->side_queued = true;
     HIPCHK(c, hipMemcpyAsync(d_iter, c->iter_of.data(), c->iter_of.size() * 4, hipMemcpyHostToDevice, c->stream));
     const uint16_t *C = nullptr;
     rc = uniform_slice(c, seed, n, T, K, jmax, &C);
@@ -560,24 +569,30 @@
 {
     const int64_t *h = c->hint_off;
     c->hint_off = nullptr;
+    c->check_pending = false;
     if (!h) return query_bags(c, d_off, S);
     if (h[0] != 0) return fail(c, M6A_EINVAL, "off[0] must be 0");
     host_bag_range(c, h, S);
     if (c->bag_min < 0) return fail(c, M6A_EINVAL, "off[] must be non-decreasing");
     unsigned long long hash = 0;
     for (int i = 0; i < M6A_HIST_BINS; i++) hash += (unsigned long long)c->h_hist[i] * m6a_bin_weight(i);
+    c->check_hash = hash;
+    c->check_pending = true;
+    return M6A_OK;
+}
+
+int bag_check(m6a_ctx *c, const int64_t *d_off, int64_t S, bool ev_main_recorded)
+{
+    if (!c->check_pending) return M6A_OK;
+    c->check_pending = false;
     hipStream_t st = c->s_prep ? c->s_prep : c->stream;
-    if (st != c->stream) {
+    if (st != c->stream && !ev_main_recorded) {
         HIPCHK(c, hipEventRecord(c->ev_main, c->stream));
         HIPCHK(c, hipStreamWaitEvent(st, c->ev_main, 0));
     }
-    HIPCHK(c, hipMemsetAsync(c->d_minmax, 0xff, 8, st));
-    HIPCHK(c, hipMemsetAsync(c->d_minmax + 1, 0, 16, st));
-    HIPCHK(c, hipMemsetAsync(c->d_hist, 0, M6A_HIST_BINS * 4, st));
-    hipLaunchKernelGGL(bag_minmax_kernel, dim3((unsigned)std::min<int64_t>((S + 255) / 256, 512)), dim3(256), 0,
-                       st, d_off, S, c->d_minmax, c->d_hist);
-    hipLaunchKernelGGL(bag_verify_kernel, dim3(1), dim3(256), 0, st, c->d_minmax, c->d_hist, (unsigned long long)c->bag_min,
-                       (unsigned long long)c->bag_max, (unsigned long long)c->n_reads, hash, c->d_err);
+    hipLaunchKernelGGL(bag_check_kernel, dim3((unsigned)std::min<int64_t>((S + 255) / 256, 512)), dim3(256), 0, st, d_off, S,
+                       c->d_chk_state, c->d_chk_hist, (unsigned long long)c->bag_min, (unsigned long long)c->bag_max,
+                       (unsigned long long)c->n_reads, c->check_hash, c->d_err);
     HIPCHK(c, hipGetLastError());
     c->side_work = true;
     return M6A_OK;
@@ -591,6 +606,7 @@
     a.X = X; a.site_kmers = km; a.off = off; a.wfrag = c->d_wfrag; a.emb = c->d_emb; a.read_prob = rp;
     a.wfrag2 = c->d_wfrag2; a.w1e_tab = c->d_w1e; a.bn = c->d_w1e + M6A_W1E_FLOATS; a.err = c->d_err;
     a.n_sites = S; a.n_reads = R; a.n_tiles = (R + 31) / 32; a.b3 = c->b3;
+    a.bag_min = c->bag_min; a.bag_max = c->bag_max;
     a.clk = c->prof.clk_for(0);
 #ifdef M6A_AB_W3
     const int64_t max_waves = (int64_t)c->n_cu * 12;
@@ -658,6 +674,7 @@
     for (int x = 0; x < 8; x++)
         for (int n = M6A_RTAB_SMALL_N - ((M6A_RTAB_SMALL_N - x) & 7); n >= 0; n -= 8) { cur[n] = run; run += c->h_hist[n]; }
     std::memcpy(ctl_slot(c), c->rt.slot_of_n, sizeof c->rt.slot_of_n);
+    c->side_queued = true;
     HIPCHK(c, hipMemcpyAsync(c->ctl_dev.p, c->h_ctl, (size_t)(M6A_HIST_BINS + M6A_RTAB_MAX_N + 1) * 4, hipMemcpyHostToDevice, c->stream));
     HIPCHK(c, hipEventRecord(c->ev_ctl, c->stream));
     const RtabUse u = rtab_use(c, nmax);
@@ -796,15 +813,23 @@
 int pool_setup_aside(m6a_ctx *c, const int64_t *off, int64_t S, int T, int K, uint32_t seed, int64_t bs, int64_t spb)
 {
     c->prep.ready = false;
+    c->prep_wait = false;
     if (S <= 0 || !c->s_prep) return M6A_OK;
-    HIPCHK(c, hipStreamWaitEvent(c->s_prep, c->ev_main, 0));
     hipStream_t main_stream = c->stream;
     c->stream = c->s_prep;
+    c->side_queued = false;
     const int rc = launch_pool(c, nullptr, off, S, T, K, 0.0f, seed, bs, spb, nullptr, nullptr, true);
     c->stream = main_stream;
-    if (rc) { c->prep.ready = false; return rc; }
-    HIPCHK(c, hipEventRecord(c->ev_prep, c->s_prep));
-    HIPCHK(c, hipStreamWaitEvent(c->stream, c->ev_prep, 0));
+    const bool queued = c->side_queued;
+    c->side_queued = false;
+    if (rc) {
+        c->prep.ready = false; c->side_work = c->side_work || queued;
+        return rc;
+    }
+    if (queued) {
+        HIPCHK(c, hipEventRecord(c->ev_prep, c->s_prep));
+        c->prep_wait = true;
+    }
     return M6A_OK;
 }
 
@@ -1006,6 +1031,11 @@
     CRCHK(hipHostMalloc((void **)&c->h_err, sizeof(int), hipHostMallocDefault));
     *c->h_err = 0;
     CRCHK(hipMalloc((void **)&c->d_hist, M6A_HIST_BINS * 4));
+    CRCHK(hipMalloc((void **)&c->d_chk_state, 24));
+    CRCHK(hipMalloc((void **)&c->d_chk_hist, M6A_HIST_BINS * 4));
+    CRCHK(hipMemset(c->d_chk_state, 0xff, 8));
+    CRCHK(hipMemset(c->d_chk_state + 1, 0, 16));
+    CRCHK(hipMemset(c->d_chk_hist, 0, M6A_HIST_BINS * 4));
     CRCHK(hipHostMalloc((void **)&c->h_hist, M6A_HIST_BINS * 4, hipHostMallocDefault));
     CRCHK(hipHostMalloc((void **)&c->h_ctl, kCtlWords * 4, hipHostMallocDefault));
     for (int n = 0; n <= M6A_RTAB_MAX_N; n++) c->rt.slot_of_n[n] = -1;
@@ -1051,6 +1081,8 @@
     if (c->h_minmax) (void)hipHostFree(c->h_minmax);
     if (c->h_err) (void)hipHostFree(c->h_err);
     if (c->d_hist) (void)hipFree(c->d_hist);
+    if (c->d_chk_state) (void)hipFree(c->d_chk_state);
+    if (c->d_chk_hist) (void)hipFree(c->d_chk_hist);
     if (c->h_hist) (void)hipHostFree(c->h_hist);
     if (c->h_ctl) (void)hipHostFree(c->h_ctl);
     for (void *p : c->graveyard) (void)hipFree(p);
@@ -1183,7 +1215,9 @@
     }
     int rc = bag_stats(c, off, S);
     if (rc) return rc;
-    return launch_encode(c, X, km, off, S, c->n_reads, rp);
+    rc = launch_encode(c, X, km, off, S, c->n_reads, rp);
+    if (rc) return rc;
+    return bag_check(c, off, S);
 }
 
 int m6a_site_pool(m6a_ctx *c, const float *rp, const int64_t *off, int64_t S, int T, int K, float thr,
@@ -1203,7 +1237,9 @@
     if (dev) {
         rc = bag_stats(c, off, S);
         if (rc) return rc;
-        return launch_pool(c, rp, off, S, T, K, thr, seed, bs, spb, site, mod);
+        rc = launch_pool(c, rp, off, S, T, K, thr, seed, bs, spb, site, mod);
+        if (rc) return rc;
+        return bag_check(c, off, S);
     }
     if (off[0] != 0) return fail(c, M6A_EINVAL, "off[0] must be 0");
     for (int64_t s = 0; s < S; s++) if (off[s + 1] < off[s]) return fail(c, M6A_EINVAL, "off[] must be non-decreasing");
@@ -1244,11 +1280,27 @@
         const int64_t R = c->n_reads;
         float *p = rp;
         if (!p) { HIPCHK(c, c->rp_scratch.ensure((size_t)std::max<int64_t>(R, 1) * 4)); p = (float *)c->rp_scratch.p; }
-        HIPCHK(c, hipEventRecord(c->ev_main, c->stream));
+        if (c->s_prep) {
+            HIPCHK(c, hipEventRecord(c->ev_main, c->stream));
+            HIPCHK(c, hipStreamWaitEvent(c->s_prep, c->ev_main, 0));
+        }
+        rc = bag_check(c, off, S, c->s_prep != nullptr);
+        if (rc) return rc;
+        const bool steady = c->infer_key.valid && c->infer_key.T == T && c->infer_key.K == K && c->infer_key.seed == seed &&
+                            c->infer_key.bs == bs && c->infer_key.spb == spb;
+        c->infer_key.valid = false;
+        if (steady) {
+            rc = pool_setup_aside(c, off, S, T, K, seed, bs, spb);
+            if (rc) return rc;
+        }
         rc = launch_encode(c, X, km, off, S, R, p);
         if (rc) return rc;
-        rc = pool_setup_aside(c, off, S, T, K, seed, bs, spb);
-        if (rc) return rc;
+        if (!steady) {
+            rc = pool_setup_aside(c, off, S, T, K, seed, bs, spb);
+            if (rc) return rc;
+        }
+        c->infer_key = {T, K, seed, bs, spb, true};
+        if (c->prep_wait) { c->prep_wait = false; HIPCHK(c, hipStreamWaitEvent(c->stream, c->ev_prep, 0)); }
         return launch_pool(c, p, off, S, T, K, thr, seed, bs, spb, site, mod);
     }
     if (off[0] != 0) return fail(c, M6A_EINVAL, "off[0] must be 0");
@@ -1378,9 +1430,9 @@
     if (!c) return M6A_EINVAL;
     if (on && !c->prof.d_clk) {
         HIPCHK(c, hipSetDevice(c->device));
-        HIPCHK(c, hipMalloc((void **)&c->prof.d_clk, (size_t)2 * M6A_CLK_SLOTS * 4 * sizeof(unsigned long long)));
-    }
-    if (on) HIPCHK(c, hipMemsetAsync(c->prof.d_clk, 0, (size_t)2 * M6A_CLK_SLOTS * 4 * sizeof(unsigned long long), c->stream));
+        HIPCHK(c, hipMalloc((void **)&c->prof.d_clk, (size_t)2 * M6A_CLK_WORDS * sizeof(unsigned long long)));
+    }
+    if (on) HIPCHK(c, hipMemsetAsync(c->prof.d_clk, 0, (size_t)2 * M6A_CLK_WORDS * sizeof(unsigned long long), c->stream));
     c->prof.on = on != 0;
     c->prof.mask = on == 2 ? 1 : on == 3 ? 2 : 3;
     c->prof.used[0] = c->prof.used[1] = 0;
@@ -1413,7 +1465,7 @@
     HIPCHK(c, hipSetDevice(c->device));
     HIPCHK(c, hipStreamSynchronize(c->stream));
     unsigned long long h[M6A_CLK_SLOTS * 4];
-    HIPCHK(c, hipMemcpy(h, c->prof.d_clk + (size_t)kind * M6A_CLK_SLOTS * 4, sizeof h, hipMemcpyDeviceToHost));
+    HIPCHK(c, hipMemcpy(h, c->prof.d_clk + (size_t)kind * M6A_CLK_WORDS, sizeof h, hipMemcpyDeviceToHost));
     std::vector<double> ghz;
     unsigned long long r_first = ~0ull, r_last = 0;
     for (int i = 0; i < M6A_CLK_SLOTS; i++) {
@@ -1433,6 +1485,17 @@
     return M6A_OK;
 }
 
+int m6a_profile_stamps(m6a_ctx *c, int kind, unsigned long long *stamps)
+{
+    settle(c);
+    if (!c || kind < 0 || kind > 1 || !stamps) return M6A_EINVAL;
+    if (!c->prof.d_clk) return fail(c, M6A_EINVAL, "m6a_profile_stamps: profiling was never enabled on this context");
+    HIPCHK(c, hipSetDevice(c->device));
+    HIPCHK(c, hipStreamSynchronize(c->stream));
+    HIPCHK(c, hipMemcpy(stamps, c->prof.d_clk + (size_t)kind * M6A_CLK_WORDS, (size_t)M6A_CLK_WORDS * sizeof(unsigned long long), hipMemcpyDeviceToHost));
+    return M6A_OK;
+}
+
 const char *m6a_last_pool_variant(const m6a_ctx *c) { return c ? c->pool_variant : "none"; }
 
 }
diff --git a/m6anet_amd/csrc/m6a_ctx.h b/m6anet_amd/csrc/m6a_ctx.h
--- a/m6anet_amd/csrc/m6a_ctx.h
+++ b/m6anet_amd/csrc/m6a_ctx.h
@@ -46,7 +46,7 @@
 
 struct Profiler {
     unsigned long long *d_clk = nullptr;
-    unsigned long long *clk_for(int kind) const { return on && (mask >> kind & 1) ? d_clk + (size_t)kind * M6A_CLK_SLOTS * 4 : nullptr; }
+    unsigned long long *clk_for(int kind) const { return on && (mask >> kind & 1) ? d_clk + (size_t)kind * M6A_CLK_WORDS : nullptr; }
     bool on = false;
     int mask = 3;
     std::vector<hipEvent_t> start[2], stop[2];
@@ -202,6 +202,13 @@
     uint32_t *h_ctl = nullptr;
     DevBuf ctl_dev, rt_rank, rt_order;
     bool side_work = false;
+    bool side_queued = false;
+    struct { int T = 0, K = 0; uint32_t seed = 0; int64_t bs = 0, spb = 0; bool valid = false; } infer_key;
+    bool prep_wait = false;
+    unsigned long long *d_chk_state = nullptr;
+    uint32_t *d_chk_hist = nullptr;
+    bool check_pending = false;
+    unsigned long long check_hash = 0;
     const int64_t *hint_off = nullptr;
     hipEvent_t ev_ctl = nullptr;
     hipStream_t s_prep = nullptr;
@@ -277,6 +284,7 @@
 int launch_pool(m6a_ctx *c, const float *rp, const int64_t *off, int64_t S, int T, int K, float thr, uint32_t seed, int64_t bs, int64_t spb,
                 float *site, double *mod, bool dry = false);
 int bag_stats(m6a_ctx *c, const int64_t *d_off, int64_t S);
+int bag_check(m6a_ctx *c, const int64_t *d_off, int64_t S, bool ev_main_recorded = false);
 void host_bag_range(m6a_ctx *c, const int64_t *off, int64_t S);
 void prof_begin(m6a_ctx *c, int kind);
 void prof_end(m6a_ctx *c, int kind);
diff --git a/m6anet_amd/csrc/m6a_kernels.h b/m6anet_amd/csrc/m6a_kernels.h
--- a/m6anet_amd/csrc/m6a_kernels.h
+++ b/m6anet_amd/csrc/m6a_kernels.h
@@ -26,15 +26,32 @@
 }
 
 #define M6A_CLK_SLOTS 64
+#define M6A_CLK_WORDS (M6A_CLK_SLOTS * 6)
 __device__ __forceinline__ void m6a_clk_stamp(unsigned long long *clk, int which)
 {
     if (!clk) return;
     const unsigned stride = (gridDim.x >> 6) | 1u, b = blockIdx.x;
     if (threadIdx.x == 0 && b % stride == 0 && b / stride < M6A_CLK_SLOTS) {
-        unsigned long long *p = clk + (size_t)(b / stride) * 4 + which * 2;
+        unsigned long long *p = which == 2 ? clk + M6A_CLK_SLOTS * 4 + (size_t)(b / stride) * 2 : clk + (size_t)(b / stride) * 4 + which * 2;
+        if (which == 2) asm volatile("s_waitcnt vmcnt(0) lgkmcnt(0)" ::: "memory");
         p[0] = __builtin_amdgcn_s_memtime();
         p[1] = __builtin_amdgcn_s_memrealtime();
     }
+}
+
+__host__ __device__ inline void m6a_start_site_bounds(int64_t r, int64_t S, int64_t bag_min, int64_t bag_max, int64_t *lo, int64_t *hi)
+{
+    int64_t l = 0, h = S;
+    if (bag_max > 0) l = r / bag_max;
+    if (bag_min > 0) { const int64_t q = r / bag_min; h = q < S ? q + 1 : S; }
+    if (l < 0 || l >= h) { l = 0; h = S; }
+    *lo = l; *hi = h;
+}
+template <class OffPtr>
+__host__ __device__ inline void m6a_start_site_range(OffPtr off, int64_t r, int64_t S, int64_t bag_min, int64_t bag_max, int64_t *lo, int64_t *hi)
+{
+    m6a_start_site_bounds(r, S, bag_min, bag_max, lo, hi);
+    if (!(off[*lo] <= r && r < off[*hi])) { *lo = 0; *hi = S; }
 }
 
 struct EncArgs {
@@ -49,6 +66,7 @@
     float *read_prob;
     int *err;
     int64_t n_sites, n_reads, n_tiles, tiles_per_wave;
+    int64_t bag_min, bag_max;
     float b3;
     unsigned long long *clk;
 };
@@ -114,8 +132,8 @@
 __global__ void mean_over_passes_kernel(const float *y, int n_iters, int64_t n_sites, float *avg);
 __global__ void pairwise_mean_kernel(const float *y, int n_iters, float *avg);
 __global__ void bag_minmax_kernel(const int64_t *off, int64_t n_sites, unsigned long long *out, uint32_t *hist);
-__global__ void bag_verify_kernel(const unsigned long long *got, const uint32_t *hist, unsigned long long mn, unsigned long long mx,
-                                  unsigned long long reads, unsigned long long hash, int *err);
+__global__ void bag_check_kernel(const int64_t *off, int64_t n_sites, unsigned long long *state, uint32_t *hist, unsigned long long mn,
+                                 unsigned long long mx, unsigned long long reads, unsigned long long hash, int *err);
 __global__ void mt19937_kernel(uint32_t seed, int64_t n_words, uint32_t *raw, const uint32_t *hist, int64_t seg_words, uint32_t *xhead, int64_t xhead_n);
 __global__ void mt_jump_kernel(const uint32_t *xhead, const uint64_t *polys, uint32_t *hist);
 __global__ void rtab_count_kernel(RtabBuild a);
diff --git a/m6anet_amd/csrc/m6a_kernels.hip b/m6anet_amd/csrc/m6a_kernels.hip
--- a/m6anet_amd/csrc/m6a_kernels.hip
+++ b/m6anet_amd/csrc/m6a_kernels.hip
@@ -247,24 +247,27 @@
     if (tile0 >= a.n_tiles) return;
     const int64_t tile1 = (tile0 + a.tiles_per_wave < a.n_tiles) ? tile0 + a.tiles_per_wave : a.n_tiles;
 
-    float w1[40], w2[80], w3[16];
-#pragma unroll
-    for (int i = 0; i < 40; i++) w1[i] = a.wfrag[i * 64 + lane];
-#pragma unroll
-    for (int i = 0; i < 80; i++) w2[i] = a.wfrag[(40 + i) * 64 + lane];
-#pragma unroll
-    for (int i = 0; i < 16; i++) w3[i] = a.wfrag[(120 + i) * 64 + lane];
-
     int64_t s_base;
     {
+        const __attribute__((address_space(4))) int64_t *off_s = (const __attribute__((address_space(4))) int64_t *)a.off;
         const int64_t r = tile0 * 32;
-        int64_t lo = 0, hi = a.n_sites;
+        int64_t lo, hi;
+        m6a_start_site_range(off_s, r, a.n_sites, a.bag_min, a.bag_max, &lo, &hi);
         while (hi - lo > 1) {
             int64_t mid = (lo + hi) >> 1;
-            if (a.off[mid] <= r) lo = mid; else hi = mid;
+            if (off_s[mid] <= r) lo = mid; else hi = mid;
         }
         s_base = lo;
     }
+
+    float w1[40], w2[80], w3[16];
+#pragma unroll
+    for (int i = 0; i < 40; i++) w1[i] = a.wfrag[i * 64 + lane];
+#pragma unroll
+    for (int i = 0; i < 80; i++) w2[i] = a.wfrag[(40 + i) * 64 + lane];
+#pragma unroll
+    for (int i = 0; i < 16; i++) w3[i] = a.wfrag[(120 + i) * 64 + lane];
+
     const int64_t last_site = a.n_sites - 1;
 
     auto link0 = [&](int64_t base, int64_t (&o)[3]) {
@@ -311,6 +314,7 @@
 
     BnPairs bnq;
     bn_pairs_load(bnq, bn_half);
+    m6a_clk_stamp(a.clk, 2);
     for (int64_t tile = tile0; tile < tile1; ++tile) {
         const int64_t tn = tile + 1 < tile1 ? tile + 1 : tile;
         float fn[8];
@@ -406,6 +410,20 @@
     const int n_sites = (int)a.n_sites;
     const int last_lim = (int)(a.n_reads - 1 - (int64_t)(n_tiles - 1) * 32);
 
+    const __attribute__((address_space(4))) int64_t *off_c = (const __attribute__((address_space(4))) int64_t *)a.off;
+    int s_base;
+    {
+        const int64_t r = (int64_t)tile0 * 32;
+        int64_t lo64, hi64;
+        m6a_start_site_range(off_c, r, (int64_t)n_sites, a.bag_min, a.bag_max, &lo64, &hi64);
+        int lo = (int)lo64, hi = (int)hi64;
+        while (hi - lo > 1) {
+            const int mid = (int)(((int64_t)lo + hi) >> 1);
+            if (off_c[mid] <= r) lo = mid; else hi = mid;
+        }
+        s_base = lo;
+    }
+
 #ifdef M6A_AB_W3
     float w1[40], w3[16];
     float4 wq[2];
@@ -423,19 +441,8 @@
 #pragma unroll
     for (int i = 0; i < 16; i++) w3[i] = a.wfrag[(120 + i) * 64 + lane];
 
-    int s_base;
-    {
-        const int64_t r = (int64_t)tile0 * 32;
-        int lo = 0, hi = n_sites;
-        while (hi - lo > 1) {
-            const int mid = (int)(((int64_t)lo + hi) >> 1);
-            if (a.off[mid] <= r) lo = mid; else hi = mid;
-        }
-        s_base = lo;
-    }
     const int last_site = n_sites - 1;
 
-    const __attribute__((address_space(4))) int64_t *off_c = (const __attribute__((address_space(4))) int64_t *)a.off;
     auto link0 = [&](int base, int64_t (&o)[3]) {
 #pragma unroll
         for (int i = 0; i < 3; i++) {
@@ -502,6 +509,7 @@
     phase_shift_second_workgroup();
     BnPairs bnq;
     bn_pairs_load(bnq, bn_half);
+    m6a_clk_stamp(a.clk, 2);
     for (int tile = tile0; tile < tile1; ++tile) {
         const int tn = tile + 1 < tile1 ? tile + 1 : tile;
         float fn[8], evn;
@@ -638,27 +646,30 @@
     const int n_sites = (int)a.n_sites;
     const int last_lim = (int)(a.n_reads - 1 - (int64_t)(n_tiles - 1) * 32);
 
-    float w1x[20], w8[5], w2[80];
-#pragma unroll
-    for (int i = 0; i < 20; i++) w1x[i] = a.wfrag2[i * 64 + lane];
-#pragma unroll
-    for (int i = 0; i < 5; i++) w8[i] = a.wfrag2[(20 + i) * 64 + lane];
-#pragma unroll
-    for (int i = 0; i < 80; i++) w2[i] = a.wfrag[(40 + i) * 64 + lane];
-
+    const __attribute__((address_space(4))) int64_t *off_c = (const __attribute__((address_space(4))) int64_t *)a.off;
     int s_base;
     {
         const int64_t r = (int64_t)tile0 * 32;
-        int lo = 0, hi = n_sites;
+        int64_t lo64, hi64;
+        m6a_start_site_range(off_c, r, (int64_t)n_sites, a.bag_min, a.bag_max, &lo64, &hi64);
+        int lo = (int)lo64, hi = (int)hi64;
         while (hi - lo > 1) {
             const int mid = (int)(((int64_t)lo + hi) >> 1);
-            if (a.off[mid] <= r) lo = mid; else hi = mid;
+            if (off_c[mid] <= r) lo = mid; else hi = mid;
         }
         s_base = lo;
     }
+
+    float w1x[20], w8[5], w2[80];
+#pragma unroll
+    for (int i = 0; i < 20; i++) w1x[i] = a.wfrag2[i * 64 + lane];
+#pragma unroll
+    for (int i = 0; i < 5; i++) w8[i] = a.wfrag2[(20 + i) * 64 + lane];
+#pragma unroll
+    for (int i = 0; i < 80; i++) w2[i] = a.wfrag[(40 + i) * 64 + lane];
+
     const int last_site = n_sites - 1;
 
-    const __attribute__((address_space(4))) int64_t *off_c = (const __attribute__((address_space(4))) int64_t *)a.off;
     auto link0 = [&](int base, int64_t (&o)[3]) {
 #pragma unroll
         for (int i = 0; i < 3; i++) {
@@ -756,6 +767,7 @@
 
     BnPairs bnq;
     bn_pairs_load(bnq, bn_half);
+    m6a_clk_stamp(a.clk, 2);
     for (int tile = tile0; tile < tile1; ++tile) {
         const int tn = tile + 1 < tile1 ? tile + 1 : tile;
         float fn[5], evn;
@@ -1453,17 +1465,54 @@
     }
 }
 
-__global__ __launch_bounds__(256) void bag_verify_kernel(const unsigned long long *got, const uint32_t *hist, unsigned long long mn,
-                                                         unsigned long long mx, unsigned long long reads, unsigned long long hash, int *err)
-{
+__global__ __launch_bounds__(256) void bag_check_kernel(const int64_t *off, int64_t n_sites, unsigned long long *state, uint32_t *hist,
+                                                        unsigned long long mn_want, unsigned long long mx_want, unsigned long long reads,
+                                                        unsigned long long hash, int *err)
+{
+    __shared__ int64_t s_mn[4], s_mx[4];
+    __shared__ uint32_t s_hist[M6A_HIST_BINS];
     __shared__ unsigned long long s_part[256];
+    __shared__ int s_last;
+    for (int i = threadIdx.x; i < M6A_HIST_BINS; i += 256) s_hist[i] = 0;
+    __syncthreads();
+    int64_t mn = INT64_MAX, mx = 0;
+    for (int64_t s = (int64_t)blockIdx.x * blockDim.x + threadIdx.x; s < n_sites; s += (int64_t)gridDim.x * blockDim.x) {
+        const int64_t n = off[s + 1] - off[s];
+        mn = n < mn ? n : mn;
+        mx = n > mx ? n : mx;
+        atomicAdd(&s_hist[n < 0 ? 0 : n > M6A_RTAB_MAX_N ? M6A_RTAB_MAX_N + 1 : n], 1u);
+    }
+#pragma unroll
+    for (int m = 1; m < 64; m <<= 1) {
+        const int64_t omn = __shfl_xor(mn, m, 64), omx = __shfl_xor(mx, m, 64);
+        mn = omn < mn ? omn : mn;
+        mx = omx > mx ? omx : mx;
+    }
+    if ((threadIdx.x & 63) == 0) { s_mn[threadIdx.x >> 6] = mn; s_mx[threadIdx.x >> 6] = mx; }
+    __syncthreads();
+    for (int i = threadIdx.x; i < M6A_HIST_BINS; i += 256)
+        if (s_hist[i]) atomicAdd(&hist[i], s_hist[i]);
+    if (threadIdx.x == 0) {
+        for (int w = 1; w < 4; w++) { mn = s_mn[w] < mn ? s_mn[w] : mn; mx = s_mx[w] > mx ? s_mx[w] : mx; }
+        atomicMin(&state[0], (unsigned long long)mn);
+        atomicMax(&state[1], (unsigned long long)mx);
+    }
+    __threadfence();
+    __syncthreads();
+    if (threadIdx.x == 0) s_last = atomicAdd(&state[2], 1ull) == (unsigned long long)gridDim.x - 1;
+    __syncthreads();
+    if (!s_last) return;
+    __threadfence();
     unsigned long long h = 0;
-    for (int i = threadIdx.x; i < M6A_HIST_BINS; i += 256) h += (unsigned long long)hist[i] * m6a_bin_weight(i);
+    for (int i = threadIdx.x; i < M6A_HIST_BINS; i += 256)
+        h += (unsigned long long)atomicExch(&hist[i], 0u) * m6a_bin_weight(i);
     s_part[threadIdx.x] = h;
     __syncthreads();
     if (threadIdx.x == 0) {
         for (int i = 1; i < 256; i++) h += s_part[i];
-        if (got[0] != mn || got[1] != mx || got[2] != reads || h != hash) atomicExch(err, 3);
+        const unsigned long long got_mn = atomicExch(&state[0], ~0ull), got_mx = atomicExch(&state[1], 0ull);
+        atomicExch(&state[2], 0ull);
+        if (got_mn != mn_want || got_mx != mx_want || (unsigned long long)off[n_sites] != reads || h != hash) atomicExch(err, 3);
     }
 }
 
diff --git a/m6anet_amd/csrc/m6a_validate.hip b/m6anet_amd/csrc/m6a_validate.hip
--- a/m6anet_amd/csrc/m6a_validate.hip
+++ b/m6anet_amd/csrc/m6a_validate.hip
@@ -337,6 +337,8 @@
         if (!d_rp) { HIPCHK(c, c->rp_scratch.ensure((size_t)std::max<int64_t>(c->n_reads, 1) * 4)); d_rp = (float *)c->rp_scratch.p; }
         rc = launch_encode(c, X, km, off, S, c->n_reads, d_rp);
         if (rc) return rc;
+        rc = bag_check(c, off, S);
+        if (rc) return rc;
         return m6a_validate_pool(c, d_rp, off, S, T, K, seed, y, avg);
     }
     if (off[0] != 0) return fail(c, M6A_EINVAL, "off[0] must be 0");
diff --git a/m6anet_amd/engine.py b/m6anet_amd/engine.py
--- a/m6anet_amd/engine.py
+++ b/m6anet_amd/engine.py
@@ -224,6 +224,11 @@
         if n.value == 0:
             return None
         return {"ghz": g.value, "ghz_min": lo.value, "ghz_max": hi.value, "span_ms": span.value, "waves": n.value}
+
+    def profile_stamps(self, kind):
+        a = np.zeros(384, np.uint64)
+        self._chk(self._L.m6a_profile_stamps(self._h, kind, a.ctypes.data))
+        return a[:256].reshape(64, 4), a[256:].reshape(64, 2)
 
     @property
     def last_pool_variant(self):
```

Result: slower. 380.0 million (-2.5%).
